# aleph-zero-foundation/sha2-on-cq-halo2

Measured on AMD Instinct MI355X. Metric: sha256_cq_create_proof_k18: MSM Mscalar/s over proof-generation wall-clock (ms_per_step), higher is better.
Workload: dtype u256-montgomery

## Files before the change

include/cq_halo2.h:

```cpp
#ifndef CQ_HALO2_H
#define CQ_HALO2_H

#include <stddef.h>
#include <stdint.h>

#ifdef __cplusplus
extern "C" {
#endif

#define CQ_OK 0
#define CQ_ERR_ARG (-1)
#define CQ_ERR_HIP (-2)
#define CQ_ERR_NO_DEVICE (-3)
#define CQ_ERR_LOOKUP (-4)
#define CQ_ERR_INTERNAL (-5)
#define CQ_ERR_TRANSCRIPT (-6)

typedef struct cq_ctx cq_ctx;
typedef struct cq_domain cq_domain;
typedef struct cq_params cq_params;
typedef struct cq_table_config cq_table_config;
typedef struct cq_static_table cq_static_table;
typedef struct cq_g2_srs cq_g2_srs;
typedef struct cq_pk cq_pk;
// ... 29 lines not shown
                    const uint64_t omega[4]);

int cq_best_multiexp(cq_ctx* ctx, const uint64_t* coeffs, const uint64_t* bases, size_t len,
                     uint64_t out_jac[12]);
int cq_best_multiexp_dev(cq_ctx* ctx, const uint64_t* coeffs_dev, const uint64_t* bases_dev, size_t len,
                         uint64_t out_jac[12]);
int cq_msm_batch_dev(cq_ctx* ctx, const uint64_t* const* coeffs_dev, const uint64_t* bases_dev, size_t len,
                     size_t count, uint64_t* out_jac);
int cq_g1_sum(const uint64_t* jac_points, size_t count, uint64_t out_jac[12]);
int cq_g1_to_affine(const uint64_t jac[12], uint64_t out_affine[8]);
int cq_best_multiexp_g2(cq_ctx* ctx, const uint64_t* coeffs, const uint64_t* bases, size_t len, uint64_t out_jac[24]);
int cq_best_multiexp_g2_dev(cq_ctx* ctx, const uint64_t* coeffs_dev, const uint64_t* bases_dev, size_t len,
                            uint64_t out_jac[24]);
int cq_g2_sum(const uint64_t* jac_points, size_t count, uint64_t out_jac[24]);
int cq_g2_to_affine(const uint64_t jac[24], uint64_t out_affine[16]);
int cq_msm_precompute_dev(cq_ctx* ctx, const uint64_t* bases_dev, size_t n);
int cq_msm_forget_dev(cq_ctx* ctx, const uint64_t* bases_dev);
int cq_msm_set_precompute(cq_ctx* ctx, int on);
int cq_msm_set_window(cq_ctx* ctx, uint32_t bits);
int cq_msm_set_table_window(cq_ctx* ctx, uint32_t bits);
int cq_msm_table_width_dev(cq_ctx* ctx, const uint64_t* bases_dev, size_t n, uint32_t preferred_bits, uint32_t* bits);

int cq_msm_bucket_sums_dev(cq_ctx* ctx, const uint64_t* const* bases_dev, size_t arrays, int packed, const uint32_t* index_dev, size_t n,
                           size_t buckets, uint64_t* out_dev);

int cq_eval_polynomial(cq_ctx* ctx, const uint64_t* poly, size_t n, const uint64_t point[4], uint64_t out[4]);
int cq_eval_polynomial_dev(cq_ctx* ctx, const uint64_t* poly_dev, size_t n, const uint64_t point[4], uint64_t out[4]);
int cq_kate_division(cq_ctx* ctx, const uint64_t* a, size_t n, const uint64_t b[4], uint64_t* q);
int cq_kate_division_dev(cq_ctx* ctx, const uint64_t* a_dev, size_t n, const uint64_t b[4], uint64_t* q_dev);
int cq_batch_invert(cq_ctx* ctx, uint64_t* a, size_t n);
int cq_batch_invert_dev(cq_ctx* ctx, uint64_t* a_dev, size_t n);

typedef struct {
  const uint64_t* num;
  const uint32_t* den_rows;
  const uint64_t* den;
  size_t den_count;
} cq_assigned_column;
int cq_batch_invert_assigned_dev(cq_ctx* ctx, const cq_assigned_column* cols, size_t ncols, size_t n, uint64_t* const* out_dev);
int cq_batch_invert_assigned(cq_ctx* ctx, const cq_assigned_column* cols, size_t ncols, size_t n, uint64_t* const* out);

int cq_domain_create(cq_ctx* ctx, uint32_t j, uint32_t k, cq_domain** out);
void cq_domain_destroy(cq_domain* domain);
uint32_t cq_domain_k(const cq_domain* domain);
uint32_t cq_domain_extended_k(const cq_domain* domain);
int cq_domain_constants(const cq_domain* domain, uint64_t omega[4], uint64_t omega_inv[4],
                        uint64_t extended_omega[4], uint64_t ifft_divisor[4]);
int cq_lagrange_to_coeff(cq_domain* domain, uint64_t* a);
int cq_coeff_to_extended(cq_domain* domain, const uint64_t* a, uint64_t* out);
int cq_extended_to_coeff(cq_domain* domain, const uint64_t* a, uint64_t* out);
int cq_lagrange_to_coeff_dev(cq_domain* domain, const uint64_t* in_dev, uint64_t* out_dev, uint32_t batch);
int cq_coeff_to_extended_dev(cq_domain* domain, const uint64_t* in_dev, uint64_t* out_dev, uint32_t batch);
int cq_extended_to_coeff_dev(cq_domain* domain, const uint64_t* in_dev, uint64_t* out_dev);

int cq_params_create(cq_ctx* ctx, uint32_t k, const uint64_t* g, const uint64_t* g_lagrange, cq_params** out);
int cq_params_setup_from_toxic_waste(cq_ctx* ctx, uint32_t k, const uint64_t s[4], cq_params** out);
int cq_fixed_base_mul_dev(cq_ctx* ctx, const uint64_t* scalars_dev, size_t n, uint64_t* out_affine_dev);
int cq_params_read_raw(cq_ctx* ctx, const uint8_t* buf, size_t len, int checked, cq_params** out);
int cq_params_write_raw(cq_params* params, uint8_t* buf, size_t cap, size_t* written);
#define CQ_SERDE_PROCESSED 0
#define CQ_SERDE_RAW_BYTES 1
#define CQ_SERDE_RAW_BYTES_UNCHECKED 2
int cq_g1_decompress_dev(cq_ctx* ctx, const uint8_t* bytes_dev, size_t n, uint64_t* out_affine_dev, size_t* first_bad);
int cq_g1_compress_dev(cq_ctx* ctx, const uint64_t* affine_dev, size_t n, uint8_t* bytes_dev);
int cq_fr_from_repr_dev(cq_ctx* ctx, const uint8_t* bytes_dev, size_t n, uint64_t* out_dev, size_t* first_bad);
int cq_fr_to_repr_dev(cq_ctx* ctx, const uint64_t* in_dev, size_t n, uint8_t* bytes_dev);
int cq_params_read(cq_ctx* ctx, const uint8_t* buf, size_t len, int format, cq_params** out);
int cq_params_write(cq_params* params, int format, uint8_t* buf, size_t cap, size_t* written);
size_t cq_params_serialized_size(const cq_params* params, int format);
int cq_g2_decompress_dev(cq_ctx* ctx, const uint8_t* bytes_dev, size_t n, uint64_t* out_affine_dev, size_t* first_bad);
int cq_g2_compress_dev(cq_ctx* ctx, const uint64_t* affine_dev, size_t n, uint8_t* bytes_dev);
int cq_params_set_g2(cq_params* params, const uint64_t g2[16], const uint64_t s_g2[16]);
int cq_params_g2(const cq_params* params, uint64_t g2[16], uint64_t s_g2[16]);
int cq_params_read_full(cq_ctx* ctx, const uint8_t* buf, size_t len, int format, cq_params** out);
int cq_params_write_full(cq_params* params, int format, uint8_t* buf, size_t cap, size_t* written);
size_t cq_params_serialized_size_full(const cq_params* params, int format);
int cq_g_to_lagrange_dev(cq_ctx* ctx, const uint64_t* g_dev, uint32_t k, uint64_t* g_lagrange_dev);
int cq_g_to_lagrange_windowed_dev(cq_ctx* ctx, const uint64_t* g_dev, uint32_t k, uint64_t* g_lagrange_dev);
int cq_params_from_powers(cq_ctx* ctx, uint32_t k, const uint64_t* g, int g_on_device, cq_params** out);
int cq_params_downsize(cq_params* params, uint32_t k, cq_params** out);
void cq_params_destroy(cq_params* params);
const uint64_t* cq_params_g_dev(const cq_params* params);
const uint64_t* cq_params_g_lagrange_dev(const cq_params* params);
int cq_commit(cq_params* params, const uint64_t* poly, size_t len, uint64_t out_jac[12]);
int cq_commit_lagrange(cq_params* params, const uint64_t* poly, size_t len, uint64_t out_jac[12]);
int cq_commit_dev(cq_params* params, const uint64_t* poly_dev, size_t len, uint64_t out_jac[12]);
int cq_commit_lagrange_dev(cq_params* params, const uint64_t* poly_dev, size_t len, uint64_t out_jac[12]);

int cq_table_config_create(cq_ctx* ctx, size_t size, const uint64_t* g1_lagrange,
                           const uint64_t* g_lagrange_opening_at_0, cq_table_config** out);
int cq_table_config_setup_from_toxic_waste(cq_ctx* ctx, size_t size, const uint64_t s[4], cq_table_config** out);
int cq_table_config_from_srs(cq_ctx* ctx, size_t size, const uint64_t* srs_g1, size_t srs_len, int on_device,
                             cq_table_config** out);
void cq_table_config_destroy(cq_table_config* cfg);
int cq_table_config_download(cq_table_config* cfg, uint64_t* g1_lagrange, uint64_t* g_lagrange_opening_at_0);
int cq_static_table_create(cq_ctx* ctx, size_t size, const uint64_t* values, const uint64_t* qs_affine,
                           cq_static_table** out);
int cq_static_table_setup_from_toxic_waste(cq_ctx* ctx, size_t size, const uint64_t* values, const uint64_t s[4],
                                           cq_static_table** out);
int cq_static_table_new(cq_ctx* ctx, size_t size, const uint64_t* values, const uint64_t* srs_g1, cq_static_table** out);
int cq_static_table_new_fk(cq_ctx* ctx, size_t size, const uint64_t* values, const uint64_t* srs_g1, cq_static_table** out);
int cq_static_table_new_fk_dev(cq_ctx* ctx, size_t size, const uint64_t* values, const uint64_t* srs_g1_dev,
                               cq_static_table** out);
void cq_static_table_destroy(cq_static_table* table);
int cq_static_table_download_qs(cq_static_table* table, uint64_t* qs_affine);
int cq_g2_srs_create(cq_ctx* ctx, size_t count, const uint64_t* points, int checked, cq_g2_srs** out);
// ... 37 lines not shown
  const uint32_t* gate_program_lens;
  const uint32_t* gate_programs;
  uint32_t num_constants;
  const uint64_t* constants;
  uint32_t num_perm_columns;
  const uint32_t* perm_column_kinds;
  const uint32_t* perm_column_indices;
  const uint32_t* perm_mapping;
  const uint32_t* lookup_input_program_lens;
  const uint32_t* lookup_input_programs;
  uint32_t num_legacy_lookups;
  const uint32_t* legacy_lookup_widths;
  const uint32_t* legacy_program_lens;
  const uint32_t* legacy_programs;
  const uint8_t* advice_column_phases;
  uint32_t num_challenges;
  const uint8_t* challenge_phases;
} cq_plonk;

typedef struct {
  uint32_t k;
  uint32_t num_advice;
  uint32_t num_lookups;
  const uint32_t* lookup_widths;
  const uint32_t* lookup_columns;
  cq_static_table* const* lookup_tables;
  uint64_t vk_repr[4];
  const cq_plonk* plonk;
} cq_circuit;

void cq_permutation_assembly_init(uint32_t columns, uint32_t n, uint32_t* mapping, uint32_t* aux, uint32_t* sizes);
int cq_permutation_assembly_copy(uint32_t columns, uint32_t n, uint32_t* mapping, uint32_t* aux, uint32_t* sizes,
                                 uint32_t left_column, uint32_t left_row, uint32_t right_column, uint32_t right_row);
int cq_pk_create(cq_ctx* ctx, cq_params* params, const cq_circuit* circuit, cq_table_config* cfg,
                 const uint64_t* b0_g1_bound, int b0_on_device, cq_pk** out);
int cq_pk_read_raw(cq_ctx* ctx, cq_params* params, const cq_circuit* circuit, cq_table_config* cfg,
                   const uint64_t* b0_g1_bound, int b0_on_device, const uint8_t* buf, size_t len, uint32_t num_selectors,
                   int checked, cq_pk** out);
size_t cq_pk_raw_size(const cq_pk* pk, uint32_t num_selectors);
int cq_pk_write_raw(cq_pk* pk, const uint8_t* selector_bits, uint32_t num_selectors, uint8_t* buf, size_t cap, size_t* written);
int cq_pk_read(cq_ctx* ctx, cq_params* params, const cq_circuit* circuit, cq_table_config* cfg, const uint64_t* b0_g1_bound,
               int b0_on_device, const uint8_t* buf, size_t len, uint32_t num_selectors, int format, cq_pk** out);
size_t cq_pk_serialized_size(const cq_pk* pk, int format, uint32_t num_selectors);
int cq_pk_write(cq_pk* pk, int format, const uint8_t* selector_bits, uint32_t num_selectors, uint8_t* buf, size_t cap, size_t* written);
int cq_pk_set_sharding(cq_pk* pk, uint32_t rank, uint32_t world, cq_allgather_fn fn, void* user);
int cq_pk_set_column_sharding(cq_pk* pk, int on, cq_bcast_fn fn, void* user);
int cq_pk_set_resident_sharding(cq_pk* pk, int on, cq_exchange_fn fn, void* user);
#define CQ_OPENER_GWC 0
#define CQ_OPENER_SHPLONK 1
int cq_pk_set_opener(cq_pk* pk, int opener);
int cq_pk_set_rng_fill(cq_pk* pk, cq_rng_fill_fn fill);
void cq_pk_destroy(cq_pk* pk);
uint32_t cq_pk_usable_rows(const cq_pk* pk);
const uint64_t* cq_pk_b_row_bases_dev(const cq_pk* pk, int which);
size_t cq_pk_proof_size(const cq_pk* pk);
int cq_create_proof(cq_pk* pk, const uint64_t* const* advice_dev, cq_rng_next_u64 rng, void* rng_state,
                    uint8_t* proof, size_t proof_cap, size_t* proof_len);
int cq_create_proof_batch(cq_pk* pk, size_t count, const uint64_t* const* const* advice_dev, cq_rng_next_u64 rng,
                          void* const* rng_states, uint8_t* const* proofs, size_t proof_cap, size_t* proof_lens, uint32_t lanes);
int cq_create_proof_host(cq_pk* pk, const uint64_t* const* advice, cq_rng_next_u64 rng, void* rng_state,
                         uint8_t* proof, size_t proof_cap, size_t* proof_len);
int cq_create_proof_assigned(cq_pk* pk, const cq_assigned_column* cols, const uint64_t* const* instances,
                             const size_t* instance_lens, cq_rng_next_u64 rng, void* rng_state, uint8_t* proof,
                             size_t proof_cap, size_t* proof_len);
int cq_create_proof_instances(cq_pk* pk, const uint64_t* const* advice, int advice_on_device,
                              const uint64_t* const* instances, const size_t* instance_lens, cq_rng_next_u64 rng,
                              void* rng_state, uint8_t* proof, size_t proof_cap, size_t* proof_len);
typedef int (*cq_phase_fn)(void* user, uint32_t phase, const uint64_t* challenges, uint64_t* const* advice_dev);
int cq_create_proof_phases(cq_pk* pk, uint64_t* const* advice_dev, const uint64_t* const* instances,
                           const size_t* instance_lens, cq_phase_fn phase_fn, void* phase_user, cq_rng_next_u64 rng,
                           void* rng_state, uint8_t* proof, size_t proof_cap, size_t* proof_len);
#define CQ_FAIL_GATE 1u
#define CQ_FAIL_GATE_POISONED 2u
#define CQ_FAIL_LOOKUP 3u
#define CQ_FAIL_STATIC_LOOKUP 4u
#define CQ_FAIL_PERMUTATION 5u
typedef struct { uint32_t kind; uint32_t index; uint32_t row; uint32_t detail; } cq_witness_failure;
int cq_pk_check_witness(cq_pk* pk, const uint64_t* const* advice, int advice_on_device, const uint64_t* const* instances,
                        const size_t* instance_lens, const uint64_t* challenges, cq_witness_failure* failures, size_t cap,
                        size_t* total);
int cq_cq_round1_dev(cq_pk* pk, const uint64_t* const* advice_dev, const uint64_t* const* instance_dev, const uint64_t* challenges,
                     const uint64_t theta[4], uint64_t* f_dev, uint32_t* m_dev, uint64_t* commitments);
int cq_cq_round2_dev(cq_pk* pk, const uint64_t* f_dev, const uint32_t* m_dev, const uint64_t theta[4], const uint64_t beta[4],
                     uint64_t* b_coeff_dev, uint64_t* f_coeff_dev, uint64_t* commitments, uint64_t* a_at_zero);
int cq_quotient_dev(cq_pk* pk, const uint64_t* b_coeff_dev, const uint64_t* f_coeff_dev, const uint64_t y[4], const uint64_t beta[4],
                    const uint64_t* h_in_dev, int divide_by_vanishing, uint64_t* h_out_dev);
int cq_permute_expression_pair_dev(cq_ctx* ctx, uint32_t k, uint32_t usable, const uint64_t* input_dev, const uint64_t* table_dev,
                                   uint64_t* permuted_input_dev, uint64_t* permuted_table_dev);
int cq_permutation_commit_dev(cq_pk* pk, const uint64_t* const* advice_dev, const uint64_t* const* instance_dev, const uint64_t beta[4],
                              const uint64_t gamma[4], cq_rng_next_u64 rng, void* rng_state, uint64_t* z_coeff_dev,
                              uint64_t* commitments);
int cq_lookup_commit_product_dev(cq_pk* pk, const uint64_t* const* input_dev, const uint64_t* const* table_dev,
                                 const uint64_t* const* permuted_input_dev, const uint64_t* const* permuted_table_dev,
                                 const uint64_t beta[4], const uint64_t gamma[4], cq_rng_next_u64 rng, void* rng_state,
                                 uint64_t* z_coeff_dev, uint64_t* commitments);
int cq_evaluate_h_dev(cq_pk* pk, const uint64_t* const* advice_coeff_dev, const uint64_t* const* instance_coeff_dev,
                      const uint64_t* perm_z_coeff_dev, const uint64_t* const* permuted_input_coeff_dev,
                      const uint64_t* const* permuted_table_coeff_dev, const uint64_t* lookup_z_coeff_dev, const uint64_t* challenges,
                      const uint64_t beta[4], const uint64_t gamma[4], const uint64_t theta[4], const uint64_t y[4], uint64_t* h_out_dev);
typedef struct { const uint64_t* poly_dev; size_t len; uint64_t point[4]; } cq_open_query;
typedef int (*cq_squeeze_challenge_fn)(void* user, uint64_t* out );
typedef int (*cq_write_point_fn)(void* user, const uint64_t* affine );
typedef struct { cq_squeeze_challenge_fn squeeze_challenge; cq_write_point_fn write_point; void* user; } cq_open_transcript;
int cq_multiopen_dev(cq_pk* pk, const cq_open_query* queries, size_t count, const cq_open_transcript* transcript);
uint32_t cq_pk_permutation_sets(const cq_pk* pk);
uint32_t cq_pk_legacy_lookups(const cq_pk* pk);
// ... 128 lines not shown
```

include/cq_halo2_sys.rs:

```rust
#![allow(non_camel_case_types, dead_code)]
use core::ffi::{c_char, c_int, c_void};

pub const CQ_OK: i32 = 0;
pub const CQ_ERR_ARG: i32 = -1;
pub const CQ_ERR_HIP: i32 = -2;
pub const CQ_ERR_NO_DEVICE: i32 = -3;
pub const CQ_ERR_LOOKUP: i32 = -4;
pub const CQ_ERR_INTERNAL: i32 = -5;
pub const CQ_ERR_TRANSCRIPT: i32 = -6;
pub const CQ_RCCL_UNIQUE_ID_BYTES: usize = 128;
pub const CQ_SERDE_PROCESSED: i32 = 0;
pub const CQ_SERDE_RAW_BYTES: i32 = 1;
pub const CQ_SERDE_RAW_BYTES_UNCHECKED: i32 = 2;
pub const CQ_GATE_CONST: u32 = 0;
pub const CQ_GATE_ADVICE: u32 = 1;
pub const CQ_GATE_FIXED: u32 = 2;
pub const CQ_GATE_INSTANCE: u32 = 3;
pub const CQ_GATE_NEG: u32 = 4;
pub const CQ_GATE_ADD: u32 = 5;
pub const CQ_GATE_MUL: u32 = 6;
pub const CQ_GATE_SCALE: u32 = 7;
pub const CQ_GATE_CHALLENGE: u32 = 8;
pub const CQ_COL_ADVICE: u32 = 0;
pub const CQ_COL_FIXED: u32 = 1;
// ... 190 lines not shown
    pub fn cq_ctx_create(device: c_int, hip_stream: *mut c_void, out: *mut *mut CqCtx) -> c_int;
    pub fn cq_ctx_destroy(ctx: *mut CqCtx);
    pub fn cq_last_error(ctx: *const CqCtx) -> *const c_char;
    pub fn cq_ctx_sync(ctx: *mut CqCtx) -> c_int;
    pub fn cq_ctx_set_hip_graphs(ctx: *mut CqCtx, on: c_int) -> c_int;
    pub fn cq_rccl_unique_id(id: *mut u8 ) -> c_int;
    pub fn cq_ctx_comm_init_rccl(ctx: *mut CqCtx, rank: u32, world: u32, id: *const u8 ) -> c_int;
    pub fn cq_ctx_comm_destroy(ctx: *mut CqCtx) -> c_int;
    pub fn cq_ctx_comm_selftest(ctx: *mut CqCtx) -> c_int;
    pub fn cq_ctx_stream(ctx: *mut CqCtx) -> *mut c_void;
    pub fn cq_version() -> *const c_char;
    pub fn cq_dev_alloc(ctx: *mut CqCtx, bytes: usize, dptr: *mut *mut c_void) -> c_int;
    pub fn cq_dev_free(ctx: *mut CqCtx, dptr: *mut c_void) -> c_int;
    pub fn cq_dev_upload(ctx: *mut CqCtx, dst_dev: *mut c_void, src_host: *const c_void, bytes: usize) -> c_int;
    pub fn cq_dev_download(ctx: *mut CqCtx, dst_host: *mut c_void, src_dev: *const c_void, bytes: usize) -> c_int;
    pub fn cq_dev_memset(ctx: *mut CqCtx, dptr: *mut c_void, value: c_int, bytes: usize) -> c_int;
    pub fn cq_best_fft(ctx: *mut CqCtx, a: *mut u64, log_n: u32, omega: *const u64 ) -> c_int;
    pub fn cq_best_fft_dev(ctx: *mut CqCtx, in_dev: *const u64, out_dev: *mut u64, log_n: u32, omega: *const u64 ) -> c_int;
    pub fn cq_best_multiexp(ctx: *mut CqCtx, coeffs: *const u64, bases: *const u64, len: usize, out_jac: *mut u64 ) -> c_int;
    pub fn cq_best_multiexp_dev(ctx: *mut CqCtx, coeffs_dev: *const u64, bases_dev: *const u64, len: usize, out_jac: *mut u64 ) -> c_int;
    pub fn cq_msm_batch_dev(ctx: *mut CqCtx, coeffs_dev: *const *const u64, bases_dev: *const u64, len: usize, count: usize, out_jac: *mut u64) -> c_int;
    pub fn cq_g1_sum(jac_points: *const u64, count: usize, out_jac: *mut u64 ) -> c_int;
    pub fn cq_g1_to_affine(jac: *const u64 , out_affine: *mut u64 ) -> c_int;
    pub fn cq_best_multiexp_g2(ctx: *mut CqCtx, coeffs: *const u64, bases: *const u64, len: usize, out_jac: *mut u64 ) -> c_int;
    pub fn cq_best_multiexp_g2_dev(ctx: *mut CqCtx, coeffs_dev: *const u64, bases_dev: *const u64, len: usize, out_jac: *mut u64 ) -> c_int;
    pub fn cq_g2_sum(jac_points: *const u64, count: usize, out_jac: *mut u64 ) -> c_int;
    pub fn cq_g2_to_affine(jac: *const u64 , out_affine: *mut u64 ) -> c_int;
    pub fn cq_msm_precompute_dev(ctx: *mut CqCtx, bases_dev: *const u64, n: usize) -> c_int;
    pub fn cq_msm_forget_dev(ctx: *mut CqCtx, bases_dev: *const u64) -> c_int;
    pub fn cq_msm_set_precompute(ctx: *mut CqCtx, on: c_int) -> c_int;
    pub fn cq_msm_set_window(ctx: *mut CqCtx, bits: u32) -> c_int;
    pub fn cq_msm_set_table_window(ctx: *mut CqCtx, bits: u32) -> c_int;
    pub fn cq_msm_table_width_dev(ctx: *mut CqCtx, bases_dev: *const u64, n: usize, preferred_bits: u32, bits: *mut u32) -> c_int;
    pub fn cq_msm_bucket_sums_dev(ctx: *mut CqCtx, bases_dev: *const *const u64, arrays: usize, packed: c_int, index_dev: *const u32, n: usize, buckets: usize, out_dev: *mut u64) -> c_int;
    pub fn cq_eval_polynomial(ctx: *mut CqCtx, poly: *const u64, n: usize, point: *const u64 , out: *mut u64 ) -> c_int;
    pub fn cq_eval_polynomial_dev(ctx: *mut CqCtx, poly_dev: *const u64, n: usize, point: *const u64 , out: *mut u64 ) -> c_int;
    pub fn cq_kate_division(ctx: *mut CqCtx, a: *const u64, n: usize, b: *const u64 , q: *mut u64) -> c_int;
    pub fn cq_kate_division_dev(ctx: *mut CqCtx, a_dev: *const u64, n: usize, b: *const u64 , q_dev: *mut u64) -> c_int;
    pub fn cq_batch_invert(ctx: *mut CqCtx, a: *mut u64, n: usize) -> c_int;
    pub fn cq_batch_invert_dev(ctx: *mut CqCtx, a_dev: *mut u64, n: usize) -> c_int;
    pub fn cq_batch_invert_assigned_dev(ctx: *mut CqCtx, cols: *const CqAssignedColumn, ncols: usize, n: usize, out_dev: *const *mut u64) -> c_int;
    pub fn cq_batch_invert_assigned(ctx: *mut CqCtx, cols: *const CqAssignedColumn, ncols: usize, n: usize, out: *const *mut u64) -> c_int;
    pub fn cq_domain_create(ctx: *mut CqCtx, j: u32, k: u32, out: *mut *mut CqDomain) -> c_int;
    pub fn cq_domain_destroy(domain: *mut CqDomain);
    pub fn cq_domain_k(domain: *const CqDomain) -> u32;
    pub fn cq_domain_extended_k(domain: *const CqDomain) -> u32;
    pub fn cq_domain_constants(domain: *const CqDomain, omega: *mut u64 , omega_inv: *mut u64 , extended_omega: *mut u64 , ifft_divisor: *mut u64 ) -> c_int;
    pub fn cq_lagrange_to_coeff(domain: *mut CqDomain, a: *mut u64) -> c_int;
    pub fn cq_coeff_to_extended(domain: *mut CqDomain, a: *const u64, out: *mut u64) -> c_int;
    pub fn cq_extended_to_coeff(domain: *mut CqDomain, a: *const u64, out: *mut u64) -> c_int;
    pub fn cq_lagrange_to_coeff_dev(domain: *mut CqDomain, in_dev: *const u64, out_dev: *mut u64, batch: u32) -> c_int;
    pub fn cq_coeff_to_extended_dev(domain: *mut CqDomain, in_dev: *const u64, out_dev: *mut u64, batch: u32) -> c_int;
    pub fn cq_extended_to_coeff_dev(domain: *mut CqDomain, in_dev: *const u64, out_dev: *mut u64) -> c_int;
    pub fn cq_params_create(ctx: *mut CqCtx, k: u32, g: *const u64, g_lagrange: *const u64, out: *mut *mut CqParams) -> c_int;
    pub fn cq_params_setup_from_toxic_waste(ctx: *mut CqCtx, k: u32, s: *const u64 , out: *mut *mut CqParams) -> c_int;
    pub fn cq_fixed_base_mul_dev(ctx: *mut CqCtx, scalars_dev: *const u64, n: usize, out_affine_dev: *mut u64) -> c_int;
    pub fn cq_params_read_raw(ctx: *mut CqCtx, buf: *const u8, len: usize, checked: c_int, out: *mut *mut CqParams) -> c_int;
    pub fn cq_params_write_raw(params: *mut CqParams, buf: *mut u8, cap: usize, written: *mut usize) -> c_int;
    pub fn cq_g1_decompress_dev(ctx: *mut CqCtx, bytes_dev: *const u8, n: usize, out_affine_dev: *mut u64, first_bad: *mut usize) -> c_int;
    pub fn cq_g1_compress_dev(ctx: *mut CqCtx, affine_dev: *const u64, n: usize, bytes_dev: *mut u8) -> c_int;
    pub fn cq_fr_from_repr_dev(ctx: *mut CqCtx, bytes_dev: *const u8, n: usize, out_dev: *mut u64, first_bad: *mut usize) -> c_int;
    pub fn cq_fr_to_repr_dev(ctx: *mut CqCtx, in_dev: *const u64, n: usize, bytes_dev: *mut u8) -> c_int;
    pub fn cq_params_read(ctx: *mut CqCtx, buf: *const u8, len: usize, format: c_int, out: *mut *mut CqParams) -> c_int;
    pub fn cq_params_write(params: *mut CqParams, format: c_int, buf: *mut u8, cap: usize, written: *mut usize) -> c_int;
    pub fn cq_params_serialized_size(params: *const CqParams, format: c_int) -> usize;
    pub fn cq_g2_decompress_dev(ctx: *mut CqCtx, bytes_dev: *const u8, n: usize, out_affine_dev: *mut u64, first_bad: *mut usize) -> c_int;
    pub fn cq_g2_compress_dev(ctx: *mut CqCtx, affine_dev: *const u64, n: usize, bytes_dev: *mut u8) -> c_int;
    pub fn cq_params_set_g2(params: *mut CqParams, g2: *const u64 , s_g2: *const u64 ) -> c_int;
    pub fn cq_params_g2(params: *const CqParams, g2: *mut u64 , s_g2: *mut u64 ) -> c_int;
    pub fn cq_params_read_full(ctx: *mut CqCtx, buf: *const u8, len: usize, format: c_int, out: *mut *mut CqParams) -> c_int;
    pub fn cq_params_write_full(params: *mut CqParams, format: c_int, buf: *mut u8, cap: usize, written: *mut usize) -> c_int;
    pub fn cq_params_serialized_size_full(params: *const CqParams, format: c_int) -> usize;
    pub fn cq_g_to_lagrange_dev(ctx: *mut CqCtx, g_dev: *const u64, k: u32, g_lagrange_dev: *mut u64) -> c_int;
    pub fn cq_g_to_lagrange_windowed_dev(ctx: *mut CqCtx, g_dev: *const u64, k: u32, g_lagrange_dev: *mut u64) -> c_int;
    pub fn cq_params_from_powers(ctx: *mut CqCtx, k: u32, g: *const u64, g_on_device: c_int, out: *mut *mut CqParams) -> c_int;
    pub fn cq_params_downsize(params: *mut CqParams, k: u32, out: *mut *mut CqParams) -> c_int;
    pub fn cq_params_destroy(params: *mut CqParams);
    pub fn cq_params_g_dev(params: *const CqParams) -> *const u64;
    pub fn cq_params_g_lagrange_dev(params: *const CqParams) -> *const u64;
    pub fn cq_commit(params: *mut CqParams, poly: *const u64, len: usize, out_jac: *mut u64 ) -> c_int;
    pub fn cq_commit_lagrange(params: *mut CqParams, poly: *const u64, len: usize, out_jac: *mut u64 ) -> c_int;
    pub fn cq_commit_dev(params: *mut CqParams, poly_dev: *const u64, len: usize, out_jac: *mut u64 ) -> c_int;
    pub fn cq_commit_lagrange_dev(params: *mut CqParams, poly_dev: *const u64, len: usize, out_jac: *mut u64 ) -> c_int;
    pub fn cq_table_config_create(ctx: *mut CqCtx, size: usize, g1_lagrange: *const u64, g_lagrange_opening_at_0: *const u64, out: *mut *mut CqTableConfig) -> c_int;
    pub fn cq_table_config_setup_from_toxic_waste(ctx: *mut CqCtx, size: usize, s: *const u64 , out: *mut *mut CqTableConfig) -> c_int;
    pub fn cq_table_config_from_srs(ctx: *mut CqCtx, size: usize, srs_g1: *const u64, srs_len: usize, on_device: c_int, out: *mut *mut CqTableConfig) -> c_int;
    pub fn cq_table_config_destroy(cfg: *mut CqTableConfig);
    pub fn cq_table_config_download(cfg: *mut CqTableConfig, g1_lagrange: *mut u64, g_lagrange_opening_at_0: *mut u64) -> c_int;
    pub fn cq_static_table_create(ctx: *mut CqCtx, size: usize, values: *const u64, qs_affine: *const u64, out: *mut *mut CqStaticTable) -> c_int;
    pub fn cq_static_table_setup_from_toxic_waste(ctx: *mut CqCtx, size: usize, values: *const u64, s: *const u64 , out: *mut *mut CqStaticTable) -> c_int;
    pub fn cq_static_table_new(ctx: *mut CqCtx, size: usize, values: *const u64, srs_g1: *const u64, out: *mut *mut CqStaticTable) -> c_int;
    pub fn cq_static_table_new_fk(ctx: *mut CqCtx, size: usize, values: *const u64, srs_g1: *const u64, out: *mut *mut CqStaticTable) -> c_int;
    pub fn cq_static_table_new_fk_dev(ctx: *mut CqCtx, size: usize, values: *const u64, srs_g1_dev: *const u64, out: *mut *mut CqStaticTable) -> c_int;
    pub fn cq_static_table_destroy(table: *mut CqStaticTable);
    pub fn cq_static_table_download_qs(table: *mut CqStaticTable, qs_affine: *mut u64) -> c_int;
    pub fn cq_g2_srs_create(ctx: *mut CqCtx, count: usize, points: *const u64, checked: c_int, out: *mut *mut CqG2Srs) -> c_int;
    pub fn cq_g2_srs_setup_from_toxic_waste(ctx: *mut CqCtx, count: usize, s: *const u64 , out: *mut *mut CqG2Srs) -> c_int;
    pub fn cq_g2_srs_download(srs: *mut CqG2Srs, points: *mut u64) -> c_int;
    pub fn cq_g2_srs_len(srs: *const CqG2Srs) -> usize;
    pub fn cq_g2_srs_dev(srs: *const CqG2Srs) -> *const u64;
    pub fn cq_g2_srs_destroy(srs: *mut CqG2Srs);
    pub fn cq_g2_srs_read(ctx: *mut CqCtx, buf: *const u8, len: usize, format: c_int, out: *mut *mut CqG2Srs) -> c_int;
    pub fn cq_g2_srs_write(srs: *mut CqG2Srs, format: c_int, buf: *mut u8, cap: usize, written: *mut usize) -> c_int;
    pub fn cq_g2_srs_serialized_size(srs: *const CqG2Srs, format: c_int) -> usize;
    pub fn cq_static_table_commit(table: *mut CqStaticTable, srs_g2: *mut CqG2Srs, srs_g1_len: usize, circuit_n: usize, zv: *mut u64 , t: *mut u64 , x_b0_bound: *mut u64 ) -> c_int;
    pub fn cq_permutation_assembly_init(columns: u32, n: u32, mapping: *mut u32, aux: *mut u32, sizes: *mut u32);
    pub fn cq_permutation_assembly_copy(columns: u32, n: u32, mapping: *mut u32, aux: *mut u32, sizes: *mut u32, left_column: u32, left_row: u32, right_column: u32, right_row: u32) -> c_int;
    pub fn cq_pk_create(ctx: *mut CqCtx, params: *mut CqParams, circuit: *const CqCircuit, cfg: *mut CqTableConfig, b0_g1_bound: *const u64, b0_on_device: c_int, out: *mut *mut CqPk) -> c_int;
    pub fn cq_pk_read_raw(ctx: *mut CqCtx, params: *mut CqParams, circuit: *const CqCircuit, cfg: *mut CqTableConfig, b0_g1_bound: *const u64, b0_on_device: c_int, buf: *const u8, len: usize, num_selectors: u32, checked: c_int, out: *mut *mut CqPk) -> c_int;
    pub fn cq_pk_raw_size(pk: *const CqPk, num_selectors: u32) -> usize;
    pub fn cq_pk_write_raw(pk: *mut CqPk, selector_bits: *const u8, num_selectors: u32, buf: *mut u8, cap: usize, written: *mut usize) -> c_int;
    pub fn cq_pk_read(ctx: *mut CqCtx, params: *mut CqParams, circuit: *const CqCircuit, cfg: *mut CqTableConfig, b0_g1_bound: *const u64, b0_on_device: c_int, buf: *const u8, len: usize, num_selectors: u32, format: c_int, out: *mut *mut CqPk) -> c_int;
    pub fn cq_pk_serialized_size(pk: *const CqPk, format: c_int, num_selectors: u32) -> usize;
    pub fn cq_pk_write(pk: *mut CqPk, format: c_int, selector_bits: *const u8, num_selectors: u32, buf: *mut u8, cap: usize, written: *mut usize) -> c_int;
    pub fn cq_pk_set_sharding(pk: *mut CqPk, rank: u32, world: u32, fn_: CqAllgatherFn, user: *mut c_void) -> c_int;
    pub fn cq_pk_set_column_sharding(pk: *mut CqPk, on: c_int, fn_: CqBcastFn, user: *mut c_void) -> c_int;
    pub fn cq_pk_set_resident_sharding(pk: *mut CqPk, on: c_int, fn_: CqExchangeFn, user: *mut c_void) -> c_int;
    pub fn cq_pk_set_opener(pk: *mut CqPk, opener: c_int) -> c_int;
    pub fn cq_pk_set_rng_fill(pk: *mut CqPk, fill: CqRngFillFn) -> c_int;
    pub fn cq_pk_destroy(pk: *mut CqPk);
    pub fn cq_pk_usable_rows(pk: *const CqPk) -> u32;
    pub fn cq_pk_b_row_bases_dev(pk: *const CqPk, which: c_int) -> *const u64;
    pub fn cq_pk_proof_size(pk: *const CqPk) -> usize;
    pub fn cq_create_proof(pk: *mut CqPk, advice_dev: *const *const u64, rng: CqRngNextU64, rng_state: *mut c_void, proof: *mut u8, proof_cap: usize, proof_len: *mut usize) -> c_int;
    pub fn cq_create_proof_batch(pk: *mut CqPk, count: usize, advice_dev: *const *const *const u64, rng: CqRngNextU64, rng_states: *const *mut c_void, proofs: *const *mut u8, proof_cap: usize, proof_lens: *mut usize, lanes: u32) -> c_int;
    pub fn cq_create_proof_host(pk: *mut CqPk, advice: *const *const u64, rng: CqRngNextU64, rng_state: *mut c_void, proof: *mut u8, proof_cap: usize, proof_len: *mut usize) -> c_int;
    pub fn cq_create_proof_assigned(pk: *mut CqPk, cols: *const CqAssignedColumn, instances: *const *const u64, instance_lens: *const usize, rng: CqRngNextU64, rng_state: *mut c_void, proof: *mut u8, proof_cap: usize, proof_len: *mut usize) -> c_int;
    pub fn cq_create_proof_instances(pk: *mut CqPk, advice: *const *const u64, advice_on_device: c_int, instances: *const *const u64, instance_lens: *const usize, rng: CqRngNextU64, rng_state: *mut c_void, proof: *mut u8, proof_cap: usize, proof_len: *mut usize) -> c_int;
    pub fn cq_create_proof_phases(pk: *mut CqPk, advice_dev: *const *mut u64, instances: *const *const u64, instance_lens: *const usize, phase_fn: CqPhaseFn, phase_user: *mut c_void, rng: CqRngNextU64, rng_state: *mut c_void, proof: *mut u8, proof_cap: usize, proof_len: *mut usize) -> c_int;
    pub fn cq_pk_check_witness(pk: *mut CqPk, advice: *const *const u64, advice_on_device: c_int, instances: *const *const u64, instance_lens: *const usize, challenges: *const u64, failures: *mut CqWitnessFailure, cap: usize, total: *mut usize) -> c_int;
    pub fn cq_cq_round1_dev(pk: *mut CqPk, advice_dev: *const *const u64, instance_dev: *const *const u64, challenges: *const u64, theta: *const u64 , f_dev: *mut u64, m_dev: *mut u32, commitments: *mut u64) -> c_int;
    pub fn cq_cq_round2_dev(pk: *mut CqPk, f_dev: *const u64, m_dev: *const u32, theta: *const u64 , beta: *const u64 , b_coeff_dev: *mut u64, f_coeff_dev: *mut u64, commitments: *mut u64, a_at_zero: *mut u64) -> c_int;
    pub fn cq_quotient_dev(pk: *mut CqPk, b_coeff_dev: *const u64, f_coeff_dev: *const u64, y: *const u64 , beta: *const u64 , h_in_dev: *const u64, divide_by_vanishing: c_int, h_out_dev: *mut u64) -> c_int;
    pub fn cq_permute_expression_pair_dev(ctx: *mut CqCtx, k: u32, usable: u32, input_dev: *const u64, table_dev: *const u64, permuted_input_dev: *mut u64, permuted_table_dev: *mut u64) -> c_int;
    pub fn cq_permutation_commit_dev(pk: *mut CqPk, advice_dev: *const *const u64, instance_dev: *const *const u64, beta: *const u64 , gamma: *const u64 , rng: CqRngNextU64, rng_state: *mut c_void, z_coeff_dev: *mut u64, commitments: *mut u64) -> c_int;
    pub fn cq_lookup_commit_product_dev(pk: *mut CqPk, input_dev: *const *const u64, table_dev: *const *const u64, permuted_input_dev: *const *const u64, permuted_table_dev: *const *const u64, beta: *const u64 , gamma: *const u64 , rng: CqRngNextU64, rng_state: *mut c_void, z_coeff_dev: *mut u64, commitments: *mut u64) -> c_int;
    pub fn cq_evaluate_h_dev(pk: *mut CqPk, advice_coeff_dev: *const *const u64, instance_coeff_dev: *const *const u64, perm_z_coeff_dev: *const u64, permuted_input_coeff_dev: *const *const u64, permuted_table_coeff_dev: *const *const u64, lookup_z_coeff_dev: *const u64, challenges: *const u64, beta: *const u64 , gamma: *const u64 , theta: *const u64 , y: *const u64 , h_out_dev: *mut u64) -> c_int;
    pub fn cq_multiopen_dev(pk: *mut CqPk, queries: *const CqOpenQuery, count: usize, transcript: *const CqOpenTranscript) -> c_int;
    pub fn cq_pk_permutation_sets(pk: *const CqPk) -> u32;
    pub fn cq_pk_legacy_lookups(pk: *const CqPk) -> u32;
    pub fn cq_pk_vk_commitments(pk: *mut CqPk, fixed_commitments: *mut u64, permutation_commitments: *mut u64) -> c_int;
    pub fn cq_sha_witness_fill_dev(ctx: *mut CqCtx, words_dev: *const u32, nwords: usize, pairs: u32, n: usize, cols_dev: *const *mut u64) -> c_int;
    pub fn cq_sha_synthesis_table_dev(ctx: *mut CqCtx, kind: c_int, first_limb_len: u32, second_limb_len: u32, out_dev: *mut u64) -> c_int;
    pub fn cq_sha_decomposition_table_dev(ctx: *mut CqCtx, first_limb_len: u32, second_limb_len: u32, k_bits: u32, out_dev: *mut u64) -> c_int;
    pub fn cq_sha_spread_table_dev(ctx: *mut CqCtx, size: usize, dense_dev: *mut u64, spread_dev: *mut u64) -> c_int;
    pub fn cq_sha256_layout(cells: *mut u32, cap: usize, count: *mut usize) -> c_int;
    pub fn cq_sha256_synthesize_dev(ctx: *mut CqCtx, table_bits: u32, msg_words: *const u32, blocks: usize, n: usize, cols_dev: *const *mut u64, digest: *mut u32 ) -> c_int;
    pub fn cq_sha256_synthesize_segments_dev(ctx: *mut CqCtx, table_bits: u32, seg_blocks: *const u32, segments: usize, sources: *const u32, words_dev: *const u32, words_len: usize, n: usize, cols_dev: *const *mut u64, digests_dev: *mut u32) -> c_int;
    pub fn cq_sha256_synthesize_choices_dev(ctx: *mut CqCtx, table_bits: u32, seg_blocks: *const u32, segments: usize, sources: *const u32, choices: *const u32, n_choices: usize, words_dev: *const u32, words_len: usize, n: usize, cols_dev: *const *mut u64, digests_dev: *mut u32) -> c_int;
    pub fn cq_sha256_synthesize_states_dev(ctx: *mut CqCtx, table_bits: u32, seg_blocks: *const u32, segments: usize, sources: *const u32, choices: *const u32, n_choices: usize, init_sources: *const u32, words_dev: *const u32, words_len: usize, n: usize, cols_dev: *const *mut u64, digests_dev: *mut u32) -> c_int;
    pub fn cq_sha256_synthesize_xors_dev(ctx: *mut CqCtx, table_bits: u32, seg_blocks: *const u32, segments: usize, sources: *const u32, choices: *const u32, n_choices: usize, init_sources: *const u32, xors: *const u32, n_xors: usize, words_dev: *const u32, words_len: usize, n: usize, cols_dev: *const *mut u64, digests_dev: *mut u32) -> c_int;
    pub fn cq_sha256_synthesize_varlen_dev(ctx: *mut CqCtx, table_bits: u32, seg_max_blocks: *const u32, segments: usize, msg_bytes_dev: *const u8, msg_bytes_len: usize, msg_offsets: *const u64, msg_lens: *const u64, n: usize, cols_dev: *const *mut u64, digests_dev: *mut u32) -> c_int;
    pub fn cq_sha256_synthesize_varlen_from_dev(ctx: *mut CqCtx, table_bits: u32, seg_max_blocks: *const u32, segments: usize, msg_bytes_dev: *const u8, msg_bytes_len: usize, msg_offsets: *const u64, msg_lens: *const u64, init_states_dev: *const u32, base_lens: *const u64, n: usize, cols_dev: *const *mut u64, digests_dev: *mut u32) -> c_int;
    pub fn cq_sha512_layout(cells: *mut u32, cap: usize, count: *mut usize) -> c_int;
    pub fn cq_sha512_synthesize_dev(ctx: *mut CqCtx, table_bits: u32, seg_blocks: *const u32, segments: usize, seg_variant: *const u32, msg_words: *const u64, n: usize, cols_dev: *const *mut u64, digests_out: *mut u64) -> c_int;
    pub fn cq_xoshiro256ss_seed(seed: u64, state: *mut u64 );
    pub fn cq_xoshiro256ss_next_u64(state: *mut c_void) -> u64;
    pub fn cq_xoshiro256ss_fill(state: *mut u64 , dst: *mut u64, count: usize, threads: u32);
    pub fn cq_buffer_rng_next_u64(state: *mut c_void) -> u64;
    pub fn cq_opaque_rng_next_u64(state: *mut c_void) -> u64;
    pub fn cq_opaque_rng_fill(state: *mut c_void, dst: *mut u64, count: usize);
    pub fn cq_profile_enable(ctx: *mut CqCtx, on: c_int) -> c_int;
    pub fn cq_profile_read(ctx: *mut CqCtx, id: c_int, total_ms: *mut f64, calls: *mut u64) -> c_int;
    pub fn cq_bench_modmul_dev(ctx: *mut CqCtx, out_dev: *mut u64, lanes: u32, iters: u32, which: c_int) -> c_int;
}
```

sha2_on_cq_halo2_amd/csrc/capi_cq.hip:

```cpp
#include <algorithm>
#include <atomic>
#include <cstring>
#include <mutex>
#include <string>
#include <thread>
#include <vector>
#include "assigned_host.hpp"
#include "building.hpp"
#include "cq.hpp"
#include "xoshiro.hpp"
#include "ctx.hpp"
#include "g1fft.hpp"
#include "plonk.hpp"
#include "poly.hpp"
#include "prover.hpp"
#include "setup.hpp"
#include "msm.hpp"
#include "comm.hpp"
#include "serde.hpp"

using namespace cq;

static bool is_pow2(size_t x) { return x && !(x & (x - 1)); }
static uint32_t log2u(size_t x) {
// ... 132 lines not shown
  if ((rc = domain_lagrange_to_coeff(dom, t->values, coeffs, 1, size, size)) != CQ_OK) return rc;
  if ((rc = poly_eval(c, coeffs, (uint32_t)size, sf, &ts)) != CQ_OK) return rc;
  if ((rc = cq_qs_scalars(c, t->values, (uint32_t)size, ts, sf, dom->omega, dom->ifft_divisor, sc)) != CQ_OK) return rc;
  if ((rc = fixed_base_mul(c, sc, (uint32_t)size, t->qs)) != CQ_OK) return rc;
  return guard.finish(out);
}

void cq_static_table_destroy(cq_static_table* t) {
  if (!t) return;
  hipStreamSynchronize(t->ctx->stream);
  if (t->values) hipFree(t->values);
  if (t->qs) hipFree(t->qs);
  if (t->slots) hipFree(t->slots);
  delete t;
}

int cq_static_table_download_qs(cq_static_table* t, uint64_t* qs_affine) {
  if (!t || !qs_affine) return CQ_ERR_ARG;
  cq_ctx* c = t->ctx;
  CQ_HIP(c, hipMemcpyAsync(qs_affine, t->qs, t->N * sizeof(G1Affine), hipMemcpyDeviceToHost, c->stream));
  CQ_HIP(c, hipStreamSynchronize(c->stream));
  return CQ_OK;
}

int cq_pk_set_opener(cq_pk* pk, int opener) {
  if (!pk || (opener != CQ_OPENER_GWC && opener != CQ_OPENER_SHPLONK)) return CQ_ERR_ARG;
  pk->opener = opener;
  return CQ_OK;
}

int cq_pk_set_rng_fill(cq_pk* pk, cq_rng_fill_fn fill) {
  if (!pk) return CQ_ERR_ARG;
  pk->rng_fill = fill;
  return CQ_OK;
}

int cq_pk_set_column_sharding(cq_pk* pk, int on, cq_bcast_fn fn, void* user) {
  if (!pk) return CQ_ERR_ARG;
  pk->shard_columns = on != 0;
  pk->bcast = fn;
  pk->bcast_user = user;
  return CQ_OK;
}

int cq_pk_set_resident_sharding(cq_pk* pk, int on, cq_exchange_fn fn, void* user) {
  if (!pk) return CQ_ERR_ARG;
  pk->shard_resident = on != 0;
  pk->exchange = fn;
  pk->exchange_user = user;
  return CQ_OK;
}

uint32_t cq_pk_usable_rows(const cq_pk* pk) { return pk ? pk->u : 0; }
const uint64_t* cq_pk_b_row_bases_dev(const cq_pk* pk, int which) {
  return pk && (which == 0 || which == 1) ? (const uint64_t*)pk->b_row_bases[which] : nullptr;
}

size_t cq_pk_proof_size(const cq_pk* pk) {
  if (!pk) return 0;
  const size_t L = pk->lookups.size(), S = pk->perm_sets();
  const size_t PL = pk->legacy.size();
  const size_t openings = pk->opener == CQ_OPENER_SHPLONK ? 2 : pk->opening_rotations().size();
  const size_t points = pk->num_advice + 2 * L + 3 * PL + S + 5 * L + 1 + pk->domain->quotient_poly_degree + openings;
  const size_t scalars = pk->advice_queries.size() + pk->fixed_queries.size() + 1 + pk->perm_columns.size() + (S ? 3 * S - 1 : 0) + 3 * L + 5 * PL;
  return 32 * (points + scalars);
}

static int create_proof_any(cq_pk* pk, const uint64_t* const* advice_dev, const uint64_t* const* instances,
                            const size_t* instance_lens, cq_rng_next_u64 rng, void* rng_state, uint8_t* proof,
                            size_t proof_cap, size_t* proof_len, cq_phase_fn phase_fn = nullptr, void* phase_user = nullptr) {
  if (!pk || (!advice_dev && pk->num_advice) || !rng || !proof || !proof_len) return CQ_ERR_ARG;
  cq_ctx* c = pk->ctx;
  if (pk->num_instance && (!instances || !instance_lens)) return c->fail(CQ_ERR_ARG, "create_proof: instance columns missing");
  CQ_HIP(c, hipSetDevice(c->device));
  std::vector<uint8_t> out;
  if (pk->num_phases > 1 && !phase_fn) return c->fail(CQ_ERR_ARG, "create_proof: a multi-phase circuit needs cq_create_proof_phases");
  if (rng == cq_buffer_rng_next_u64) ((cq_buffer_rng*)rng_state)->overrun = 0;
  int rc = create_proof_dev(pk, advice_dev, instances, instance_lens, phase_fn, phase_user, rng, rng_state, out);
  const bool rank_local = rc == CQ_ERR_HIP || rc == CQ_ERR_INTERNAL || rc == CQ_ERR_NO_DEVICE;
  if (rank_local && pk->sharded() && !pk->allgather && c->rccl_comm && !pk->shard_single) {
    const std::string keep = c->err;
    cq::comm_rccl_abort(c);
    c->err = keep + " (sharded proof: this rank's RCCL communicator was aborted so that its peers do not hang)";
  }
  if (rng == cq_buffer_rng_next_u64 && ((cq_buffer_rng*)rng_state)->overrun && (rc == CQ_OK || rc == CQ_ERR_TRANSCRIPT))
    return c->fail(CQ_ERR_ARG, "create_proof: the pre-drawn RNG stream ran out (blinding would be zero)");
  if (rc != CQ_OK) return rc;
  if (out.size() > proof_cap) return c->fail(CQ_ERR_ARG, "proof buffer too small");
  memcpy(proof, out.data(), out.size());
  *proof_len = out.size();
  return CQ_OK;
}

int cq_create_proof(cq_pk* pk, const uint64_t* const* advice_dev, cq_rng_next_u64 rng, void* rng_state, uint8_t* proof,
                    size_t proof_cap, size_t* proof_len) {
  return create_proof_any(pk, advice_dev, nullptr, nullptr, rng, rng_state, proof, proof_cap, proof_len);
}

static int create_proof_host_any(cq_pk* pk, const uint64_t* const* advice, const uint64_t* const* instances,
                                 const size_t* instance_lens, cq_rng_next_u64 rng, void* rng_state, uint8_t* proof,
                                 size_t proof_cap, size_t* proof_len) {
  if (!pk || (!advice && pk->num_advice)) return CQ_ERR_ARG;
  cq_ctx* c = pk->ctx;
  CQ_HIP(c, hipSetDevice(c->device));
  const size_t n = (size_t)1 << pk->k;
  void* stage;
// ... 334 lines not shown
```

sha2_on_cq_halo2_amd/csrc/capi_poly.hip:

```cpp
#include <cstring>
#include <string>
#include <vector>
#include "assigned_host.hpp"
#include "ctx.hpp"
#include "poly.hpp"

using namespace cq;

namespace {
struct HostStage {
  cq_ctx* c;
  void* din = nullptr;
  void* dout = nullptr;
  int rc = CQ_OK;
  HostStage(cq_ctx* c_, size_t in_bytes, size_t out_bytes) : c(c_) {
    if ((rc = c->ensure_scratch(Scratch::EntryA, in_bytes ? in_bytes : 32, &din)) != CQ_OK) return;
    rc = c->ensure_scratch(Scratch::EntryB, out_bytes ? out_bytes : 32, &dout);
  }
};

int assigned_offsets(cq_ctx* c, const cq_assigned_column* cols, size_t ncols, size_t n, std::vector<uint32_t>& off) {
  if (n > 0x7fffffffull) return c->fail(CQ_ERR_ARG, "batch_invert_assigned: n too large");
  off.assign(ncols + 1, 0);
  for (size_t a = 0; a < ncols; a++) {
    const cq_assigned_column& col = cols[a];
    if ((n && !col.num) || (col.den_count && (!col.den_rows || !col.den)))
      return c->fail(CQ_ERR_ARG, "batch_invert_assigned: column " + std::to_string(a) + ": null array");
    if (col.den_count > n)
      return c->fail(CQ_ERR_ARG, "batch_invert_assigned: column " + std::to_string(a) + ", entry " + std::to_string(n) +
                                     ": more entries than rows");
    if ((uint64_t)off[a] + col.den_count > 0x7fffffffull) return c->fail(CQ_ERR_ARG, "batch_invert_assigned: too many rational cells");
    off[a + 1] = off[a] + (uint32_t)col.den_count;
  }
  return CQ_OK;
}
inline size_t round32(size_t b) { return (b + 31) & ~(size_t)31; }
}

extern "C" {

int cq_domain_create(cq_ctx* c, uint32_t j, uint32_t k, cq_domain** out) {
  if (!c || !out || j < 1) return CQ_ERR_ARG;
  CQ_HIP(c, hipSetDevice(c->device));
  return domain_create(c, j, k, out);
}
void cq_domain_destroy(cq_domain* d) { domain_destroy(d); }
uint32_t cq_domain_k(const cq_domain* d) { return d ? d->k : 0; }
uint32_t cq_domain_extended_k(const cq_domain* d) { return d ? d->extended_k : 0; }

int cq_domain_constants(const cq_domain* d, uint64_t omega[4], uint64_t omega_inv[4], uint64_t extended_omega[4],
                        uint64_t ifft_divisor[4]) {
  if (!d) return CQ_ERR_ARG;
  if (omega) d->omega.to_limbs64(omega);
  if (omega_inv) d->omega_inv.to_limbs64(omega_inv);
  if (extended_omega) d->extended_omega.to_limbs64(extended_omega);
  if (ifft_divisor) d->ifft_divisor.to_limbs64(ifft_divisor);
  return CQ_OK;
}

int cq_lagrange_to_coeff_dev(cq_domain* d, const uint64_t* in_dev, uint64_t* out_dev, uint32_t batch) {
  if (!d || !in_dev || !out_dev || !batch) return CQ_ERR_ARG;
  CQ_HIP(d->ctx, hipSetDevice(d->ctx->device));
  return domain_lagrange_to_coeff(d, (const Fr*)in_dev, (Fr*)out_dev, batch, d->n(), d->n());
}
int cq_coeff_to_extended_dev(cq_domain* d, const uint64_t* in_dev, uint64_t* out_dev, uint32_t batch) {
  if (!d || !in_dev || !out_dev || !batch) return CQ_ERR_ARG;
  if ((const void*)in_dev == (const void*)out_dev) return d->ctx->fail(CQ_ERR_ARG, "coeff_to_extended: in == out");
  CQ_HIP(d->ctx, hipSetDevice(d->ctx->device));
  return domain_coeff_to_extended(d, (const Fr*)in_dev, (Fr*)out_dev, batch, d->n(), d->ext());
}
int cq_extended_to_coeff_dev(cq_domain* d, const uint64_t* in_dev, uint64_t* out_dev) {
  if (!d || !in_dev || !out_dev) return CQ_ERR_ARG;
  CQ_HIP(d->ctx, hipSetDevice(d->ctx->device));
  return domain_extended_to_coeff(d, (const Fr*)in_dev, (Fr*)out_dev);
}

int cq_lagrange_to_coeff(cq_domain* d, uint64_t* a) {
  if (!d || !a) return CQ_ERR_ARG;
  cq_ctx* c = d->ctx;
  CQ_HIP(c, hipSetDevice(c->device));
  const size_t bytes = d->n() * sizeof(Fr);
  HostStage st(c, bytes, bytes);
  if (st.rc != CQ_OK) return st.rc;
  CQ_HIP(c, hipMemcpyAsync(st.din, a, bytes, hipMemcpyHostToDevice, c->stream));
  int rc = domain_lagrange_to_coeff(d, (const Fr*)st.din, (Fr*)st.dout, 1, d->n(), d->n());
  if (rc != CQ_OK) return rc;
  CQ_HIP(c, hipMemcpyAsync(a, st.dout, bytes, hipMemcpyDeviceToHost, c->stream));
  CQ_HIP(c, hipStreamSynchronize(c->stream));
  return CQ_OK;
}
int cq_coeff_to_extended(cq_domain* d, const uint64_t* a, uint64_t* out) {
  if (!d || !a || !out) return CQ_ERR_ARG;
  cq_ctx* c = d->ctx;
  CQ_HIP(c, hipSetDevice(c->device));
  HostStage st(c, d->n() * sizeof(Fr), d->ext() * sizeof(Fr));
  if (st.rc != CQ_OK) return st.rc;
  CQ_HIP(c, hipMemcpyAsync(st.din, a, d->n() * sizeof(Fr), hipMemcpyHostToDevice, c->stream));
  int rc = domain_coeff_to_extended(d, (const Fr*)st.din, (Fr*)st.dout, 1, d->n(), d->ext());
  if (rc != CQ_OK) return rc;
  CQ_HIP(c, hipMemcpyAsync(out, st.dout, d->ext() * sizeof(Fr), hipMemcpyDeviceToHost, c->stream));
  CQ_HIP(c, hipStreamSynchronize(c->stream));
  return CQ_OK;
}
int cq_extended_to_coeff(cq_domain* d, const uint64_t* a, uint64_t* out) {
  if (!d || !a || !out) return CQ_ERR_ARG;
  cq_ctx* c = d->ctx;
  CQ_HIP(c, hipSetDevice(c->device));
  const size_t out_bytes = d->n() * d->quotient_poly_degree * sizeof(Fr);
  HostStage st(c, d->ext() * sizeof(Fr), out_bytes);
  if (st.rc != CQ_OK) return st.rc;
  CQ_HIP(c, hipMemcpyAsync(st.din, a, d->ext() * sizeof(Fr), hipMemcpyHostToDevice, c->stream));
  int rc = domain_extended_to_coeff(d, (const Fr*)st.din, (Fr*)st.dout);
  if (rc != CQ_OK) return rc;
  if (out_bytes) CQ_HIP(c, hipMemcpyAsync(out, st.dout, out_bytes, hipMemcpyDeviceToHost, c->stream));
  CQ_HIP(c, hipStreamSynchronize(c->stream));
  return CQ_OK;
}

int cq_eval_polynomial_dev(cq_ctx* c, const uint64_t* poly_dev, size_t n, const uint64_t point[4], uint64_t out[4]) {
  if (!c || !point || !out || (n && !poly_dev) || n > 0x7fffffffull) return CQ_ERR_ARG;
  CQ_HIP(c, hipSetDevice(c->device));
  Fr r;
  int rc = poly_eval(c, (const Fr*)poly_dev, (uint32_t)n, Fr::from_limbs64(point), &r);
  if (rc != CQ_OK) return rc;
  r.to_limbs64(out);
  return CQ_OK;
}
int cq_eval_polynomial(cq_ctx* c, const uint64_t* poly, size_t n, const uint64_t point[4], uint64_t out[4]) {
  if (!c || !point || !out || (n && !poly) || n > 0x7fffffffull) return CQ_ERR_ARG;
// ... 122 lines not shown
```

sha2_on_cq_halo2_amd/csrc/cq.hpp:

```cpp
#pragma once
#include <hip/hip_runtime.h>
#include <vector>
#include "../../include/cq_halo2.h"
#include "curve.hpp"
#include "pk.hpp"
#include "poly.hpp"

struct cq_ctx;
struct cq_params;

namespace cq {

constexpr uint32_t CQ_MAX_WIDTH = 8;

struct CqRound1Args {
  const Fr* cols[CQ_MAX_WIDTH];
  const Fr* values[CQ_MAX_WIDTH];
  const uint32_t* slots[CQ_MAX_WIDTH];
  uint32_t nslots[CQ_MAX_WIDTH];
  uint32_t width;
};
constexpr uint32_t CQ_ROUND1_BATCH = 8;
struct CqRound1Batch {
  CqRound1Args a[CQ_ROUND1_BATCH];
// ... 52 lines not shown
int g1_validate(cq_ctx* c, const G1Affine* pts, uint32_t n, uint32_t* bad_dev);
int fr_validate(cq_ctx* c, const Fr* v, size_t n, uint32_t* bad_dev);

}

namespace cq {
inline void shard_range(size_t n, uint32_t rank, uint32_t world, size_t& lo, size_t& hi) {
  const size_t base = n / world, rem = n % world;
  lo = rank * base + (rank < rem ? rank : rem);
  hi = lo + base + (rank < rem ? 1 : 0);
}
}

struct cq_params {
  cq_ctx* ctx;
  uint32_t k;
  size_t n;
  cq::G1Affine* g;
  cq::G1Affine* g_lagrange;
  uint32_t key_users = 0;
  bool owner_released = false;
  bool has_g2 = false;
  uint64_t g2[16] = {}, s_g2[16] = {};
};

struct cq_table_config {
  cq_ctx* ctx;
  uint32_t log_n;
  size_t N;
  cq::G1Affine* g1_lagrange = nullptr;
  cq::G1Affine* g_lagrange_opening_at_0 = nullptr;
  uint32_t key_users = 0;
  bool owner_released = false;
};

struct cq_static_table {
  cq_ctx* ctx;
  size_t N;
  cq::Fr* values = nullptr;
  cq::G1Affine* qs = nullptr;
  uint32_t* slots = nullptr;
  uint32_t nslots = 0;
};

struct cq_pk : cq_pk_desc {
  cq_ctx* ctx;
  cq_params* params;
  cq_domain* domain = nullptr;
  cq_table_config* table_cfg;
  cq::G1Affine* b0_g1_bound = nullptr;
  bool own_b0 = false;
  cq::G1Affine* b_row_bases[2] = {nullptr, nullptr};
  cq::Fr* l_active_row = nullptr;
  cq::Fr* fixed_values = nullptr;
  cq::Fr* fixed_polys = nullptr;
  cq::Fr* fixed_cosets = nullptr;
  cq::Fr* l0 = nullptr;
  cq::Fr* l_last = nullptr;
  uint32_t* gate_prog = nullptr;
  cq::Fr* constants = nullptr;
  uint32_t* lookup_prog = nullptr;
  uint32_t* legacy_prog = nullptr;
  cq::Fr* perm_values = nullptr;
  cq::Fr* perm_polys = nullptr;
  cq::Fr* perm_cosets = nullptr;
  cq::Fr* omega_powers = nullptr;
  cq::Fr* ext_pow_lo = nullptr;
  cq::Fr* ext_pow_hi = nullptr;
  int opener = CQ_OPENER_GWC;
  cq_rng_fill_fn rng_fill = nullptr;
  cq::Fr vk_repr;
  std::vector<cq::G1Affine*> qs_concat;
  uint32_t shard_rank = 0, shard_world = 1;
  bool shard_single = false;
  bool sharded() const { return shard_world > 1 || shard_single; }
  cq_allgather_fn allgather = nullptr;
  void* allgather_user = nullptr;
  bool shard_columns = true;
  cq_bcast_fn bcast = nullptr;
  void* bcast_user = nullptr;
  bool shard_resident = false;
  cq_exchange_fn exchange = nullptr;
  void* exchange_user = nullptr;
  uint32_t table_c = 0;
  struct TableRef { const void* bases; size_t n; uint32_t c; };
  std::vector<TableRef> held_tables, shard_tables;
  bool dropped_params_tables = false, dropped_cfg_tables = false;
  bool counted_users = false;
};
```

sha2_on_cq_halo2_amd/csrc/domain.hip:

```cpp
#include "ctx.hpp"
#include "poly.hpp"

namespace cq {

int domain_create(cq_ctx* c, uint32_t j, uint32_t k, cq_domain** out) {
  if (j < 2 && j != 1) return c->fail(CQ_ERR_ARG, "domain: j must be >= 1");
  if (k > FR_S) return c->fail(CQ_ERR_ARG, "domain: k too large");
  cq_domain* d = new cq_domain();
  d->ctx = c;
  d->j = j;
  d->k = k;
  d->quotient_poly_degree = j - 1;
  const uint64_t n = 1ull << k;
  uint32_t ek = k;
  while ((1ull << ek) < n * d->quotient_poly_degree) ek++;
  if (ek > FR_S) {
    delete d;
    return c->fail(CQ_ERR_ARG, "domain: extended_k exceeds the field's 2-adicity");
  }
  d->extended_k = ek;
  Fr w = fr_from_raw(FR_ROOT_OF_UNITY_RAW);
  for (uint32_t i = ek; i < FR_S; i++) w = w.sqr();
  d->extended_omega = w;
  for (uint32_t i = k; i < ek; i++) w = w.sqr();
  d->omega = w;
  d->omega_inv = d->omega.inv();
  d->extended_omega_inv = d->extended_omega.inv();
  d->g_coset = fr_from_raw(FR_ZETA_RAW);
  d->g_coset_inv = d->g_coset.sqr();
  const Fr orig = d->g_coset.pow_u64(n);
  const Fr step = d->extended_omega.pow_u64(n);
  Fr cur = orig;
  const size_t tl = (size_t)1 << (ek - k);
  for (size_t i = 0; i < tl; i++) {
    d->t_evaluations.push_back((cur - Fr::one()).inv());
    cur = cur * step;
  }
  d->ifft_divisor = Fr::from_u64(n).inv();
  d->extended_ifft_divisor = Fr::from_u64(1ull << ek).inv();
  d->barycentric_weight = d->ifft_divisor;
  if (hipMalloc(&d->t_evaluations_dev, tl * sizeof(Fr)) != hipSuccess ||
      hipMemcpy(d->t_evaluations_dev, d->t_evaluations.data(), tl * sizeof(Fr), hipMemcpyHostToDevice) != hipSuccess) {
    delete d;
    return c->fail(CQ_ERR_HIP, "domain: t_evaluations upload failed");
  }
  *out = d;
  return CQ_OK;
}

void domain_destroy(cq_domain* d) {
  if (!d) return;
  hipStreamSynchronize(d->ctx->stream);
  if (d->t_evaluations_dev) hipFree(d->t_evaluations_dev);
  delete d;
}

static int run(cq_ctx* c, uint32_t log_n, const Fr& omega, const Fr* in, Fr* out, NttIo& io) {
  int rc = CQ_OK;
  const NttTables* tb = c->tables_for(log_n, omega, &rc);
  if (!tb) return rc;
  const size_t n = (size_t)1 << log_n;
  const bool aux = c->aux_stream && c->stream == c->aux_stream;
  void* scr;
  if ((rc = c->ensure_scratch(aux ? Scratch::NttAux : Scratch::Ntt, (size_t)2 * io.batch * n * sizeof(Fr), &scr)) != CQ_OK) return rc;
  io.prof = c;
  io.critical = !aux;
  if (ntt_run(*tb, in, out, (Fr*)scr, io, c->stream) != 0) return c->fail(CQ_ERR_HIP, "ntt launch failed");
  return CQ_OK;
}

int domain_fft(cq_ctx* c, const Fr* in, Fr* out, uint32_t log_n, const Fr& omega, uint32_t batch, size_t in_stride,
               size_t out_stride) {
  NttIo io;
  io.batch = batch;
  io.in_stride = in_stride;
  io.out_stride = out_stride;
  io.in_len = io.out_len = 1u << log_n;
  return run(c, log_n, omega, in, out, io);
}

int domain_lagrange_to_coeff(cq_domain* d, const Fr* in, Fr* out, uint32_t batch, size_t in_stride, size_t out_stride) {
  NttIo io;
  io.batch = batch;
  io.in_stride = in_stride;
  io.out_stride = out_stride;
  io.in_len = io.out_len = (uint32_t)d->n();
  io.out_mul = true;
  io.out_mul_v[0] = d->ifft_divisor;
  return run(d->ctx, d->k, d->omega_inv, in, out, io);
}

int domain_coeff_to_extended(cq_domain* d, const Fr* in, Fr* out, uint32_t batch, size_t in_stride, size_t out_stride) {
  NttIo io;
  io.batch = batch;
  io.in_stride = in_stride;
  io.out_stride = out_stride;
  io.in_len = (uint32_t)d->n();
  io.out_len = (uint32_t)d->ext();
  io.in_coset = true;
  io.in_coset_mul[0] = d->g_coset;
  io.in_coset_mul[1] = d->g_coset_inv;
  return run(d->ctx, d->extended_k, d->extended_omega, in, out, io);
}

int domain_extended_to_coeff(cq_domain* d, const Fr* in, Fr* out) {
  NttIo io;
  io.batch = 1;
  io.in_stride = d->ext();
  io.out_stride = d->n() * d->quotient_poly_degree;
  io.in_len = (uint32_t)d->ext();
  io.out_len = (uint32_t)(d->n() * d->quotient_poly_degree);
  io.out_mul = true;
  io.out_coset = true;
  io.out_mul_v[0] = d->extended_ifft_divisor;
  io.out_mul_v[1] = d->extended_ifft_divisor * d->g_coset_inv;
  io.out_mul_v[2] = d->extended_ifft_divisor * d->g_coset;
  return run(d->ctx, d->extended_k, d->extended_omega_inv, in, out, io);
}

}
```

sha2_on_cq_halo2_amd/csrc/ntt.hip:

```cpp
#include <cstdlib>
#include "ntt.hpp"
#include "ctx.hpp"

namespace cq {

__global__ void fr_powers_kernel(Fr* out, Fr base, uint64_t step, uint32_t count) {
  uint32_t j = blockIdx.x * blockDim.x + threadIdx.x;
  if (j >= count) return;
  out[j] = base.pow_u64((uint64_t)j * step);
}

static __device__ __forceinline__ Fr29 lds_load29(const uint32_t* sm, uint32_t E, uint32_t i) {
  Fr29 r;
  CQ_UNROLL for (int l = 0; l < 9; l++) r.a[l] = sm[l * E + i];
  return r;
}
static __device__ __forceinline__ void lds_store29(uint32_t* sm, uint32_t E, uint32_t i, const Fr29& r) {
  CQ_UNROLL for (int l = 0; l < 9; l++) sm[l * E + i] = r.a[l];
}
static __device__ __forceinline__ Fr29 g_load29(const Fr* p) {
  const uint4* q = reinterpret_cast<const uint4*>(p);
  const uint4 a = q[0], b = q[1];
  const uint32_t w[8] = {a.x, a.y, a.z, a.w, b.x, b.y, b.z, b.w};
  return Fr29::unpack(w);
}
static __device__ __forceinline__ void g_store29(Fr* p, const Fr29& x, bool canonical) {
  uint32_t w[8];
  x.pack(w);
  if (canonical) Fr::cond_sub_p(w, 0);
  uint4* q = reinterpret_cast<uint4*>(p);
  q[0] = make_uint4(w[0], w[1], w[2], w[3]);
  q[1] = make_uint4(w[4], w[5], w[6], w[7]);
}
static __device__ __forceinline__ Fr29 const29(const uint32_t* c) {
  Fr29 r;
  CQ_UNROLL for (int l = 0; l < 9; l++) r.a[l] = c[l];
  return r;
}
static __device__ __forceinline__ Fr29 canon29(const Fr29& x) {
  uint32_t w[8];
  x.pack(w);
  Fr::cond_sub_p(w, 0);
  return Fr29::unpack(w);
}
static __device__ __forceinline__ Fr29 sub_level(const Fr29& u, const Fr29& v, uint32_t rnd) {
  switch (rnd) {
    case 0: return Fr29::sub<2>(u, v);
    case 1: return Fr29::sub<4>(u, v);
    case 2: return Fr29::sub<8>(u, v);
    case 3: return Fr29::sub<16>(u, v);
    case 4: return Fr29::sub<32>(u, v);
    default: return Fr29::sub<64>(u, v);
  }
}

__global__ void ntt_table_to29_kernel(Fr* t, uint32_t count) {
  const uint32_t j = blockIdx.x * blockDim.x + threadIdx.x;
  if (j >= count) return;
  g_store29(t + j, Fr29::mul(g_load29(t + j), const29(CONSTS29<FrP>.from256)), true);
}

#ifdef CQ_NTT_TRACE
__device__ uint64_t g_ntt_trace[4 * 65536];
__device__ uint32_t g_ntt_trace_n;
static __device__ __forceinline__ uint32_t ntt_trace_begin() {
  uint32_t slot = 0;
  if (threadIdx.x == 0) {
    slot = atomicAdd(&g_ntt_trace_n, 1u) & 65535u;
    uint32_t hw, xcc;
    asm volatile("s_getreg_b32 %0, hwreg(HW_REG_HW_ID)" : "=s"(hw));
    asm volatile("s_getreg_b32 %0, hwreg(HW_REG_XCC_ID)" : "=s"(xcc));
    g_ntt_trace[4 * slot] = wall_clock64();
    g_ntt_trace[4 * slot + 2] = ((uint64_t)xcc << 32) | hw;
    g_ntt_trace[4 * slot + 3] = ((uint64_t)blockIdx.y << 32) | blockIdx.x;
  }
  return slot;
}
static __device__ __forceinline__ void ntt_trace_end(uint32_t slot) {
  __syncthreads();
  if (threadIdx.x == 0) g_ntt_trace[4 * slot + 1] = wall_clock64();
}
extern "C" int cq_debug_ntt_trace(uint64_t* out, uint32_t cap) {
  uint32_t n = 0;
  if (hipDeviceSynchronize() != hipSuccess) return -1;
  if (hipMemcpyFromSymbol(&n, HIP_SYMBOL(g_ntt_trace_n), 4) != hipSuccess) return -1;
  if (n > cap) n = cap;
  if (n > 65536) n = 65536;
  if (n && hipMemcpyFromSymbol(out, HIP_SYMBOL(g_ntt_trace), (size_t)n * 32) != hipSuccess) return -1;
  const uint32_t z = 0;
  if (hipMemcpyToSymbol(HIP_SYMBOL(g_ntt_trace_n), &z, 4) != hipSuccess) return -1;
  return (int)n;
}
#endif

static_assert(NTT_MAX_DEG <= 6, "sub_level: B_r = 2^(r+1) <= 64");
static __device__ __forceinline__ uint32_t bitrev(uint32_t x, uint32_t bits) {
  return bits ? (__brev(x) >> (32 - bits)) : 0;
}

template <uint32_t DEG, uint32_t LOG_T>
__global__ __launch_bounds__(NTT_THREADS) void ntt_pass_kernel(NttPassArgs a) {
  extern __shared__ uint32_t smem29[];
#ifdef CQ_NTT_TRACE
  const uint32_t trace_slot = ntt_trace_begin();
#endif
  if (a.flags & NTT_CRITICAL) CQ_CRITICAL_WAVES();
  constexpr bool DYN = DEG == 0;
  const uint32_t deg = DYN ? a.deg : DEG, log_t = DYN ? a.log_t : LOG_T;
  const uint32_t D = 1u << deg;
  const uint32_t T = 1u << log_t;
  const uint32_t E = D * T;
  uint32_t* const tw29 = smem29 + 9 * E;
  uint32_t* const cl29 = tw29 + 9 * (D / 2 + 1);
  uint32_t* const cs29 = cl29 + 27;
  const uint32_t n = 1u << a.log_n;
  const uint32_t t = n >> deg;
  const uint32_t p = 1u << a.lgp;
  const uint32_t tile = blockIdx.x;
  const uint32_t batch = blockIdx.y;
  const Fr* in = a.in + (size_t)batch * a.in_stride;
  Fr* out = a.out + (size_t)batch * a.out_stride;
  const uint32_t index0 = tile * T;
  const bool first = a.lgp == 0, last = a.next_deg == 0;
  constexpr bool SWZ = !DYN && LOG_T == 4;
  auto at = [&](uint32_t row, uint32_t c) { return SWZ ? (((row ^ (((row >> 2) ^ (row >> 4)) & 3u)) << 4) + c) : row * T + c; };

  const bool load_mul = first && (a.flags & NTT_IN_COSET);
  if (load_mul && threadIdx.x < 3) {
    Fr29 cl = const29(CONSTS29<FrP>.from256);
    if (threadIdx.x) cl = Fr29::mul(Fr29::unpack(a.in_coset[threadIdx.x - 1].v.l), const29(CONSTS29<FrP>.c271));
    CQ_UNROLL for (int l = 0; l < 9; l++) cl29[threadIdx.x * 9 + l] = cl.a[l];
  }
  if (last && threadIdx.x >= 64 && threadIdx.x < 67) {
    const uint32_t m = threadIdx.x - 64;
    const Fr one = Fr::one();
    const uint32_t* src = (a.flags & NTT_OUT_MUL) ? ((a.flags & NTT_OUT_COSET) ? a.out_mul[m].v.l : a.out_mul[0].v.l) : one.v.l;
    const Fr29 cm = Fr29::unpack(src);
    CQ_UNROLL for (int l = 0; l < 9; l++) cs29[m * 9 + l] = cm.a[l];
  }
  if (load_mul) __syncthreads();
  const uint32_t half = D >> 1;
  for (uint32_t j = threadIdx.x; j < half; j += NTT_THREADS) {
    const Fr29 w = g_load29(a.pq + ((size_t)j << a.pq_shift));
    CQ_UNROLL for (int l = 0; l < 9; l++) tw29[l * half + j] = w.a[l];
  }
  for (uint32_t e = threadIdx.x; e < E; e += NTT_THREADS) {
    const uint32_t c = e & (T - 1);
    const uint32_t i = e >> log_t;
    const uint32_t g = index0 + c + i * t;
    Fr29 x = Fr29::zero();
    if (g < a.in_len) {
      x = g_load29(in + g);
      if (load_mul) x = Fr29::mul(x, lds_load29(cl29 + (g % 3) * 9, 1, 0));
    }
    lds_store29(smem29, E, at(i, c), x);
  }
  __syncthreads();

  constexpr uint32_t R4 = DEG / 2, LEVELS = DEG;
  Fr29::static_for<0, (int)R4>([&](auto ST) {
    constexpr uint32_t st = (uint32_t) decltype(ST)::value;
    constexpr uint32_t rnd = 2 * st;
    const uint32_t bit = half >> rnd;
    const uint32_t hb = bit >> 1;
    for (uint32_t w = threadIdx.x; w < (half >> 1) * T; w += NTT_THREADS) {
      const uint32_t c = w & (T - 1);
      const uint32_t wg = w >> log_t;
      const uint32_t dj = wg >> rnd;
      const uint32_t r0 = (((wg & ((1u << rnd) - 1u)) * bit) << 1) + dj;
      const uint32_t o0 = at(r0, c), o1 = at(r0 + hb, c), o2 = at(r0 + bit, c), o3 = at(r0 + bit + hb, c);
      const Fr29 x0 = lds_load29(smem29, E, o0), x1 = lds_load29(smem29, E, o1);
      const Fr29 x2 = lds_load29(smem29, E, o2), x3 = lds_load29(smem29, E, o3);
      const Fr29 s02 = x0 + x2, s13 = x1 + x3;
      Fr29 d02 = sub_level(x0, x2, rnd);
      Fr29 d13 = sub_level(x1, x3, rnd);
      if (dj) Fr29::mul_pair(d02, lds_load29(tw29, half, dj << rnd), d13, lds_load29(tw29, half, (dj + hb) << rnd), d02, d13);
      else d13 = Fr29::mul(d13, lds_load29(tw29, half, (dj + hb) << rnd));
      Fr29 y0 = s02 + s13;
      y0.normalise();
      Fr29 y1 = sub_level(s02, s13, rnd + 1);
      Fr29 y2 = d02 + d13;
      y2.normalise();
      Fr29 y3 = sub_level(d02, d13, rnd + 1);
      if (dj) {
        const Fr29 w2 = lds_load29(tw29, half, dj << (rnd + 1));
        Fr29::mul_pair(y1, w2, y3, w2, y1, y3);
      }
      lds_store29(smem29, E, o0, y0);
      lds_store29(smem29, E, o1, y1);
      lds_store29(smem29, E, o2, y2);
      lds_store29(smem29, E, o3, y3);
    }
    __syncthreads();
  });
#pragma unroll
  for (uint32_t rnd = 2 * R4; rnd < (DYN ? 6u : LEVELS); rnd++) {
    if (DYN && rnd >= deg) break;
    const uint32_t bit = half >> rnd;
    const uint32_t lg_rest = rnd;
    for (uint32_t w = threadIdx.x; w < half * T; w += NTT_THREADS) {
      const uint32_t c = w & (T - 1);
      const uint32_t wb = w >> log_t;
      const uint32_t di = wb >> lg_rest;
      const uint32_t b = ((wb & ((1u << lg_rest) - 1u)) * bit) | di;
      const uint32_t i0 = (b << 1) - di;
      const uint32_t i1 = i0 + bit;
// ... 61 lines not shown

int NttTables::build(uint32_t log_n_, const Fr& omega_, hipStream_t stream) {
  log_n = log_n_;
  omega = omega_;
  tw_l = (log_n + 1) / 2;
  const uint32_t lo_cnt = 1u << tw_l;
  const uint32_t hi_cnt = 1u << (log_n - tw_l);
  pq_log = log_n < NTT_MAX_DEG ? log_n : NTT_MAX_DEG;
  const uint32_t pq_cnt = pq_log ? (1u << (pq_log - 1)) : 1;
  if (hipMalloc(&tw_lo, sizeof(Fr) * lo_cnt) != hipSuccess) return -1;
  if (hipMalloc(&tw_hi, sizeof(Fr) * hi_cnt) != hipSuccess) return -1;
  if (hipMalloc(&pq, sizeof(Fr) * pq_cnt) != hipSuccess) return -1;
  fr_powers_kernel<<<(lo_cnt + 255) / 256, 256, 0, stream>>>(tw_lo, omega, 1, lo_cnt);
  fr_powers_kernel<<<(hi_cnt + 255) / 256, 256, 0, stream>>>(tw_hi, omega, (uint64_t)lo_cnt, hi_cnt);
  if (log_n >= 8 && log_n <= 24 && !getenv("CQ_NTT_NO_FULL_TABLE") && hipMalloc(&tw_full, sizeof(Fr) << log_n) == hipSuccess)
    fr_powers_kernel<<<((1u << log_n) + 255) / 256, 256, 0, stream>>>(tw_full, omega, 1, 1u << log_n);
  else
    (void)hipGetLastError();
  fr_powers_kernel<<<(pq_cnt + 255) / 256, 256, 0, stream>>>(pq, omega, (uint64_t)1 << (log_n - pq_log), pq_cnt);
  ntt_table_to29_kernel<<<(lo_cnt + 255) / 256, 256, 0, stream>>>(tw_lo, lo_cnt);
  ntt_table_to29_kernel<<<(hi_cnt + 255) / 256, 256, 0, stream>>>(tw_hi, hi_cnt);
  if (tw_full) ntt_table_to29_kernel<<<((1u << log_n) + 255) / 256, 256, 0, stream>>>(tw_full, 1u << log_n);
  ntt_table_to29_kernel<<<(pq_cnt + 255) / 256, 256, 0, stream>>>(pq, pq_cnt);
  return hipGetLastError() == hipSuccess ? 0 : -1;
}

int ntt_run(const NttTables& tb, const Fr* in, Fr* out, Fr* scratch, const NttIo& io, hipStream_t stream) {
  const uint32_t log_n = tb.log_n;
  const uint32_t n = 1u << log_n;
  const uint32_t npass = log_n == 0 ? 1 : (log_n + NTT_MAX_DEG - 1) / NTT_MAX_DEG;
  uint32_t degs[8];
  uint32_t rem = log_n;
  for (uint32_t i = 0; i < npass; i++) {
    uint32_t d = (rem + (npass - i) - 1) / (npass - i);
    degs[i] = d;
    rem -= d;
  }
  if (NTT_MAX_DEG == 6 && log_n >= 12) {
    for (uint32_t c5 = 0; c5 <= npass; c5++) {
      bool found = false;
      for (uint32_t a6 = 0; a6 + c5 <= npass; a6++) {
        const uint32_t b4 = npass - c5 - a6;
        if (6 * a6 + 5 * c5 + 4 * b4 != log_n) continue;
        uint32_t i = 0;
        for (uint32_t q = 0; q < a6; q++) degs[i++] = 6;
        for (uint32_t q = 0; q < c5; q++) degs[i++] = 5;
        for (uint32_t q = 0; q < b4; q++) degs[i++] = 4;
        found = true;
        break;
      }
      if (found) break;
    }
  }
  Fr* sbuf[2] = {scratch, scratch + (size_t)io.batch * n};
  const Fr* src = in;
  uint32_t lgp = 0;
  for (uint32_t ps = 0; ps < npass; ps++) {
    const bool last = (ps + 1 == npass);
    Fr* dst = last ? out : sbuf[ps & 1];
    NttPassArgs a;
    a.in = src;
    a.out = dst;
    a.in_stride = (ps == 0) ? io.in_stride : (size_t)n;
    a.out_stride = last ? io.out_stride : (size_t)n;
    a.log_n = log_n;
    a.lgp = lgp;
    a.deg = degs[ps];
    a.next_deg = last ? 0 : degs[ps + 1];
    const uint32_t t = n >> degs[ps];
    uint32_t log_t = 0;
    while ((1u << (log_t + 1)) <= t && ((1u << (log_t + 1)) << degs[ps]) <= NTT_TILE_ELEMS) log_t++;
    a.log_t = log_t;
    a.tw_lo = tb.tw_lo;
    a.tw_hi = tb.tw_hi;
    a.tw_full = tb.tw_full;
    a.tw_l = tb.tw_l;
    a.pq = tb.pq;
    a.pq_shift = tb.pq_log - degs[ps];
    a.flags = io.critical ? NTT_CRITICAL : 0;
    a.in_len = n;
    a.out_len = n;
    if (ps == 0) {
      a.in_len = io.in_len;
      if (io.in_coset) {
        a.flags |= NTT_IN_COSET;
        a.in_coset[0] = io.in_coset_mul[0];
        a.in_coset[1] = io.in_coset_mul[1];
      }
    }
    if (last) {
      a.out_len = io.out_len;
      const Fr fix = io.in_coset ? Fr::one() : Fr::from_u64(32);
      if (io.out_mul || !io.in_coset) {
        a.flags |= NTT_OUT_MUL;
        a.out_mul[0] = (io.out_mul ? io.out_mul_v[0] : Fr::one()) * fix;
        if (io.out_mul && io.out_coset) {
          a.flags |= NTT_OUT_COSET;
          a.out_mul[1] = io.out_mul_v[1] * fix;
          a.out_mul[2] = io.out_mul_v[2] * fix;
        }
      }
    }
    const uint32_t T = 1u << log_t;
    dim3 grid(t / T, io.batch);
    const size_t lds = ((size_t)(T << degs[ps]) + ((size_t)1 << degs[ps]) / 2 + 1) * 36 + 54 * 4;
    hipEvent_t pe = io.prof ? io.prof->prof_begin(CQ_PROF_NTT_PASS) : nullptr;
    constexpr uint32_t LT = NTT_TILE_ELEMS == 512 ? 9 : NTT_TILE_ELEMS == 2048 ? 11 : 10;
    static_assert(NTT_TILE_ELEMS == (1u << LT), "NTT_TILE_ELEMS: 512, 1024 or 2048");
    if (degs[ps] == 6 && log_t == LT - 6) ntt_pass_kernel<6, LT - 6><<<grid, NTT_THREADS, lds, stream>>>(a);
    else if (degs[ps] == 5 && log_t == LT - 5) ntt_pass_kernel<5, LT - 5><<<grid, NTT_THREADS, lds, stream>>>(a);
    else if (degs[ps] == 4 && log_t == LT - 4) ntt_pass_kernel<4, LT - 4><<<grid, NTT_THREADS, lds, stream>>>(a);
    else ntt_pass_kernel<0, 0><<<grid, NTT_THREADS, lds, stream>>>(a);
    if (io.prof) io.prof->prof_end(pe);
    src = dst;
    lgp += degs[ps];
  }
  return hipGetLastError() == hipSuccess ? 0 : -1;
}

}
```

sha2_on_cq_halo2_amd/csrc/ntt.hpp:

```cpp
#pragma once
#include <hip/hip_runtime.h>
#include "field.hpp"
#include "field29.hpp"

struct cq_ctx;

namespace cq {

#ifndef CQ_NTT_THREADS
#define CQ_NTT_THREADS 256
#endif
constexpr uint32_t NTT_THREADS = CQ_NTT_THREADS;
#ifndef CQ_NTT_MAX_DEG
#define CQ_NTT_MAX_DEG 6
#endif
#ifndef CQ_NTT_TILE_ELEMS
#define CQ_NTT_TILE_ELEMS 1024
#endif
constexpr uint32_t NTT_MAX_DEG = CQ_NTT_MAX_DEG;
constexpr uint32_t NTT_TILE_ELEMS = CQ_NTT_TILE_ELEMS;

enum : uint32_t { NTT_IN_COSET = 1, NTT_OUT_MUL = 2, NTT_OUT_COSET = 4, NTT_CRITICAL = 8 };

struct NttPassArgs {
  const Fr* in;
  Fr* out;
  size_t in_stride, out_stride;
  uint32_t log_n, lgp, deg, log_t;
  uint32_t next_deg;
  const Fr* tw_lo;
  const Fr* tw_hi;
  const Fr* tw_full;
  uint32_t tw_l;
  const Fr* pq;
  uint32_t pq_shift;
  uint32_t flags;
  uint32_t in_len;
  uint32_t out_len;
  Fr in_coset[2];
  Fr out_mul[3];
};

struct NttTables {
  uint32_t log_n = 0;
  Fr omega;
  Fr* tw_lo = nullptr;
  Fr* tw_hi = nullptr;
  Fr* tw_full = nullptr;
  Fr* pq = nullptr;
  uint32_t tw_l = 0, pq_log = 0;
  NttTables() = default;
  NttTables(const NttTables&) = delete;
  NttTables& operator=(const NttTables&) = delete;
  ~NttTables();
  int build(uint32_t log_n, const Fr& omega, hipStream_t stream);
};

struct NttIo {
  uint32_t batch = 1;
  size_t in_stride = 0, out_stride = 0;
  uint32_t in_len = 0, out_len = 0;
  bool in_coset = false;
  Fr in_coset_mul[2];
  bool out_mul = false, out_coset = false;
  Fr out_mul_v[3];
  cq_ctx* prof = nullptr;
  bool critical = false;
};

int ntt_run(const NttTables& tb, const Fr* in, Fr* out, Fr* scratch, const NttIo& io, hipStream_t stream);

}
```

sha2_on_cq_halo2_amd/csrc/pk.hip:

```cpp
#include <algorithm>
#include <cstring>
#include <string>
#include <vector>
#include "building.hpp"
#include "cq.hpp"
#include "ctx.hpp"
#include "g1fft.hpp"
#include "msm.hpp"
#include "plonk.hpp"
#include "poly.hpp"
#include "serde.hpp"

using namespace cq;

size_t cq::static_table_rows(const cq_static_table* t) { return t->N; }

namespace {
void put_be32(uint8_t*& o, uint32_t v) {
  o[0] = (uint8_t)(v >> 24); o[1] = (uint8_t)(v >> 16); o[2] = (uint8_t)(v >> 8); o[3] = (uint8_t)v;
  o += 4;
}
int unit_coset(cq_pk* pk, size_t row, Fr* tmp, Fr* dst) {
  cq_ctx* c = pk->ctx;
  const size_t n = (size_t)1 << pk->k, ext = pk->domain->ext();
// ... 246 lines not shown
  if (b0_g1_bound && b0_on_device) {
    pk->b0_g1_bound = (G1Affine*)b0_g1_bound;
  } else if (b0_g1_bound) {
    if ((rc = c->dev_alloc(&pk->b0_g1_bound, n - 1, "b0 bound")) != CQ_OK) return rc;
    pk->own_b0 = true;
    CQ_HIP(c, hipMemcpyAsync(pk->b0_g1_bound, b0_g1_bound, (n - 1) * sizeof(G1Affine), hipMemcpyHostToDevice, c->stream));
  }
  for (auto& lk : pk->lookups) {
    G1Affine* cat = nullptr;
    const size_t N = cfg->N;
    if ((rc = c->dev_alloc(&cat, lk.tables.size() * N, "qs")) != CQ_OK) return rc;
    pk->qs_concat.push_back(cat);
    for (size_t j = 0; j < lk.tables.size(); j++)
      CQ_HIP(c, hipMemcpyAsync(cat + j * N, lk.tables[j]->qs, N * sizeof(G1Affine), hipMemcpyDeviceToDevice, c->stream));
  }
  if ((rc = pk_small_tables(pk)) != CQ_OK) return rc;
  CQ_HIP(c, hipStreamSynchronize(c->stream));
  if (!pk->lookups.empty() && pk->b0_g1_bound && cfg->N + 1 <= ((size_t)1 << (MSM_TABLE_C - 1)) && n >= 2) {
    const G1Affine* src[2] = {pk->params->g, pk->b0_g1_bound};
    for (int q = 0; q < 2; q++) {
      if ((rc = c->dev_alloc(&pk->b_row_bases[q], n, "b row bases")) != CQ_OK) return rc;
      if ((rc = g1_to_lagrange_shifted(c, src[q], (uint32_t)(n - 1), 1, pk->k, pk->b_row_bases[q])) != CQ_OK) return rc;
      if (msm_bases29(c, pk->b_row_bases[q], (uint32_t)n, pk->b_row_bases[q]) != 0) return c->fail(CQ_ERR_HIP, "b row bases");
    }
    CQ_HIP(c, hipStreamSynchronize(c->stream));
  }
  return CQ_OK;
}

static int pk_create_impl(cq_ctx* c, cq_params* params, const cq_circuit* cs, cq_table_config* cfg, const uint64_t* b0_g1_bound,
                          int b0_on_device, PkStreamReader* in, cq_pk** out) {
  if (!c || !params || !cs || !out) return CQ_ERR_ARG;
  *out = nullptr;
  cq_pk_desc desc;
  std::string why;
  int rc = pk_describe(cs, params->k, cfg ? &cfg->N : nullptr, b0_g1_bound != nullptr, in != nullptr,
                       PkLimits{CQ_MAX_LOOKUPS, CQ_MAX_WIDTH, PERM_MAX_COLUMNS, PERM_MAX_CHUNK}, &desc, &why);
  if (rc != CQ_OK) return c->fail(rc, why);
  CQ_HIP(c, hipSetDevice(c->device));
  cq_pk* pk = new cq_pk();
  Building<cq_pk> guard(pk, cq_pk_destroy, c);
  static_cast<cq_pk_desc&>(*pk) = std::move(desc);
  pk->ctx = c;
  pk->params = params;
  pk->table_cfg = cfg;
  pk->vk_repr = Fr::from_limbs64(cs->vk_repr);
  params->key_users++;
  if (cfg) cfg->key_users++;
  pk->counted_users = true;
  if ((rc = pk_upload_programs(pk, cs->plonk)) != CQ_OK) return rc;
  if ((rc = domain_create(c, pk->cs_degree, pk->k, &pk->domain)) != CQ_OK) return rc;
  if ((rc = pk_alloc_polys(pk)) != CQ_OK) return rc;
  if ((rc = in ? pk_read_polys(pk, *in) : pk_keygen_polys(pk, cs->plonk)) != CQ_OK) return rc;
  if ((rc = pk_attach_bases(pk, b0_g1_bound, b0_on_device)) != CQ_OK) return rc;
  *out = guard.release();
  return CQ_OK;
}

extern "C" {

int cq_pk_create(cq_ctx* c, cq_params* params, const cq_circuit* cs, cq_table_config* cfg, const uint64_t* b0_g1_bound,
                 int b0_on_device, cq_pk** out) {
  return pk_create_impl(c, params, cs, cfg, b0_g1_bound, b0_on_device, nullptr, out);
}

int cq_pk_read_raw(cq_ctx* c, cq_params* params, const cq_circuit* cs, cq_table_config* cfg, const uint64_t* b0_g1_bound,
                   int b0_on_device, const uint8_t* buf, size_t len, uint32_t num_selectors, int checked, cq_pk** out) {
  if (!buf) return CQ_ERR_ARG;
  PkStreamReader in{buf, len, num_selectors, checked != 0, false};
  return pk_create_impl(c, params, cs, cfg, b0_g1_bound, b0_on_device, &in, out);
}

int cq_pk_read(cq_ctx* c, cq_params* params, const cq_circuit* cs, cq_table_config* cfg, const uint64_t* b0_g1_bound, int b0_on_device,
               const uint8_t* buf, size_t len, uint32_t num_selectors, int format, cq_pk** out) {
  if (!buf) return CQ_ERR_ARG;
  if (format != CQ_SERDE_PROCESSED && format != CQ_SERDE_RAW_BYTES && format != CQ_SERDE_RAW_BYTES_UNCHECKED)
    return c ? c->fail(CQ_ERR_ARG, "pk: unknown serde format") : CQ_ERR_ARG;
  PkStreamReader in{buf, len, num_selectors, format == CQ_SERDE_RAW_BYTES, format == CQ_SERDE_PROCESSED};
  return pk_create_impl(c, params, cs, cfg, b0_g1_bound, b0_on_device, &in, out);
}

static size_t pk_stream_size(const cq_pk* pk, uint32_t num_selectors, size_t point_bytes) {
  if (!pk) return 0;
  const size_t n = (size_t)1 << pk->k, ext = pk->domain->ext(), F = pk->num_fixed, PC = pk->perm_columns.size();
  const size_t poly_n = 4 + n * sizeof(Fr), poly_e = 4 + ext * sizeof(Fr);
  return 8 + (F + PC) * point_bytes + (size_t)num_selectors * ((n + 7) / 8) + 3 * poly_e + 3 * 4 + F * (2 * poly_n + poly_e) + 3 * 4 +
         PC * (2 * poly_n + poly_e);
}
size_t cq_pk_raw_size(const cq_pk* pk, uint32_t num_selectors) { return pk_stream_size(pk, num_selectors, sizeof(G1Affine)); }
size_t cq_pk_serialized_size(const cq_pk* pk, int format, uint32_t num_selectors) {
  if (format == CQ_SERDE_PROCESSED) return pk_stream_size(pk, num_selectors, 32);
  if (format == CQ_SERDE_RAW_BYTES || format == CQ_SERDE_RAW_BYTES_UNCHECKED) return pk_stream_size(pk, num_selectors, sizeof(G1Affine));
  return 0;
}

static int pk_write_impl(cq_pk* pk, bool processed, const uint8_t* selector_bits, uint32_t num_selectors, uint8_t* buf, size_t cap,
                         size_t* written) {
  if (!pk || !buf || !written || (num_selectors && !selector_bits)) return CQ_ERR_ARG;
  cq_ctx* c = pk->ctx;
  CQ_HIP(c, hipSetDevice(c->device));
  const size_t n = (size_t)1 << pk->k, ext = pk->domain->ext(), F = pk->num_fixed, PC = pk->perm_columns.size();
  const size_t total = pk_stream_size(pk, num_selectors, processed ? 32 : sizeof(G1Affine));
  if (cap < total) return c->fail(CQ_ERR_ARG, "pk: output buffer too small");
  uint8_t* o = buf;
  put_be32(o, pk->k);
  put_be32(o, (uint32_t)F);
// ... 101 lines not shown
    pk->dropped_cfg_tables = true;
  }
  struct Use { const G1Affine* b; size_t len; };
  std::vector<Use> uses{{pk->params->g_lagrange, n}, {pk->params->g, n}, {pk->params->g, n - 1}};
  if (has_cfg) {
    uses.push_back({pk->table_cfg->g1_lagrange, N});
    uses.push_back({pk->table_cfg->g_lagrange_opening_at_0, N});
  }
  if (pk->b0_g1_bound) uses.push_back({pk->b0_g1_bound, n - 1});
  std::vector<std::pair<const G1Affine*, const G1Affine*>> iv;
  for (auto& u : uses) {
    size_t lo, hi;
    shard_range(u.len, pk->shard_rank, pk->shard_world, lo, hi);
    if (hi > lo) iv.push_back({u.b + lo, u.b + hi});
  }
  std::sort(iv.begin(), iv.end());
  std::vector<std::pair<const G1Affine*, const G1Affine*>> merged;
  for (auto& x : iv) {
    if (!merged.empty() && x.first <= merged.back().second) merged.back().second = std::max(merged.back().second, x.second);
    else merged.push_back(x);
  }
  for (auto& m : merged) {
    bool held = false;
    const size_t len = (size_t)(m.second - m.first);
    if ((rc = msm_register_tables(c, m.first, len, pk->table_c, &held)) != CQ_OK) return rc;
    if (held) pk->shard_tables.push_back({m.first, len, pk->table_c});
  }
  return CQ_OK;
}

int cq_pk_set_sharding(cq_pk* pk, uint32_t rank, uint32_t world, cq_allgather_fn fn, void* user) {
  if (!pk || world == 0 || rank >= world) return CQ_ERR_ARG;
  cq_ctx* c = pk->ctx;
  if (world > 1 && !fn && (!c->rccl_comm || c->rccl_world != world || c->rccl_rank != rank))
    return c->fail(CQ_ERR_ARG, "set_sharding: no all-gather callback and no matching RCCL communicator on the context");
  CQ_HIP(c, hipSetDevice(c->device));
  CQ_HIP(c, hipStreamSynchronize(c->stream));
  pk->shard_rank = rank;
  pk->shard_world = world;
  pk->shard_single = world == 1 && !fn && c->rccl_comm && c->rccl_world == 1;
  pk->allgather = world > 1 ? fn : nullptr;
  pk->allgather_user = user;
  int rc = pk_shard_tables(pk);
  if (rc != CQ_OK) return rc;
  CQ_HIP(c, hipStreamSynchronize(c->stream));
  return CQ_OK;
}

void cq_pk_destroy(cq_pk* pk) {
  if (!pk) return;
  hipStreamSynchronize(pk->ctx->stream);
  if (pk->domain) domain_destroy(pk->domain);
  if (pk->l_active_row) hipFree(pk->l_active_row);
  for (void* p : {(void*)pk->fixed_values, (void*)pk->fixed_polys, (void*)pk->fixed_cosets, (void*)pk->l0, (void*)pk->l_last,
                  (void*)pk->gate_prog, (void*)pk->constants, (void*)pk->lookup_prog, (void*)pk->legacy_prog, (void*)pk->perm_values, (void*)pk->perm_polys, (void*)pk->perm_cosets,
                  (void*)pk->omega_powers, (void*)pk->ext_pow_lo, (void*)pk->ext_pow_hi})
    if (p) hipFree(p);
  if (pk->shard_world > 1 || pk->dropped_params_tables || pk->dropped_cfg_tables) {
    pk->shard_world = 1;
    (void)pk_shard_tables(pk);
  }
  for (auto& t : pk->held_tables) msm_release_table(pk->ctx, t.bases, t.n, t.c);
  for (int q = 0; q < 2; q++)
    if (pk->b_row_bases[q]) hipFree(pk->b_row_bases[q]);
  if (pk->own_b0 && pk->b0_g1_bound) {
    msm_unregister_tables(pk->ctx, pk->b0_g1_bound);
    hipFree(pk->b0_g1_bound);
  }
  for (auto p : pk->qs_concat) {
    msm_unregister_tables(pk->ctx, p);
    hipFree(p);
  }
  if (pk->counted_users) {
    cq_params* params = pk->params;
    cq_table_config* cfg = pk->table_cfg;
    if (--params->key_users == 0 && params->owner_released) cq_params_destroy(params);
    if (cfg && --cfg->key_users == 0 && cfg->owner_released) cq_table_config_destroy(cfg);
  }
  delete pk;
}

}
```

sha2_on_cq_halo2_amd/csrc/pk.hpp:

```cpp
#pragma once
#include <algorithm>
#include <cstdint>
#include <string>
#include <utility>
#include <vector>
#include "../../include/cq_halo2.h"

namespace cq {
size_t static_table_rows(const cq_static_table* t);
bool gate_program_check(const uint32_t* lens, const uint32_t* words, uint32_t num_polys, uint32_t num_constants,
                        uint32_t num_advice, uint32_t num_fixed, uint32_t num_instance, uint32_t num_challenges,
                        const char** why, size_t* total_words);
}

struct cq_lookup_desc {
  std::vector<uint32_t> cols;
  std::vector<int64_t> prog;
  std::vector<cq_static_table*> tables;
};

struct cq_pk_desc {
  uint32_t k = 0, num_advice = 0, bf = 0, u = 0;
  std::vector<cq_lookup_desc> lookups;
  std::vector<std::pair<uint32_t, int32_t>> advice_queries;
  uint32_t num_fixed = 0, num_instance = 0, cs_degree = 3;
  std::vector<std::pair<uint32_t, int32_t>> fixed_queries;
  uint32_t num_gate_polys = 0;
  bool lookup_exprs = false;
  struct LegacyLookup { uint32_t width; size_t in_off, tab_off; };
  std::vector<LegacyLookup> legacy;
  std::vector<std::pair<uint32_t, uint32_t>> perm_columns;
  std::vector<uint8_t> advice_phase;
  std::vector<uint8_t> challenge_phase;
  uint32_t num_phases = 1;
  bool general() const { return num_gate_polys || !perm_columns.empty() || !legacy.empty(); }
  size_t perm_sets() const {
    const size_t chunk = cs_degree - 2;
    return (perm_columns.size() + chunk - 1) / chunk;
  }
  int32_t point_rotation(int32_t rot) const {
    const int64_t n = (int64_t)1 << k, r = (((int64_t)rot % n) + n) % n;
    return (int32_t)(r >= (n + 1) / 2 ? r - n : r);
  }
  std::vector<int32_t> opening_rotations() const {
    std::vector<int32_t> rots{0};
    auto seen = [&](int32_t rot) {
      const int32_t r = point_rotation(rot);
      if (std::find(rots.begin(), rots.end(), r) == rots.end()) rots.push_back(r);
    };
    for (auto& q : advice_queries) seen(q.second);
    for (auto& q : fixed_queries) seen(q.second);
    if (perm_sets() || !legacy.empty()) seen(1);
    if (!legacy.empty()) seen(-1);
    if (perm_sets() > 1) seen(-(int32_t)(bf + 1));
    return rots;
  }
};

namespace cq {

struct PkLimits {
  uint32_t lookups, width, perm_columns, perm_chunk;
};

inline std::vector<uint32_t> pack_programs(const uint32_t* lens, const uint32_t* words, size_t count, std::vector<size_t>* offsets = nullptr) {
  std::vector<uint32_t> blob;
  for (size_t i = 0; i < count; i++) {
    if (offsets) offsets->push_back(blob.size());
    blob.push_back(lens[i]);
    blob.insert(blob.end(), words, words + lens[i]);
    words += lens[i];
// ... 146 lines not shown
```

sha2_on_cq_halo2_amd/csrc/poly.hip:

```cpp
#include "poly.hpp"
#include "field29.hpp"
#include <algorithm>
#include <cstring>
#include "ctx.hpp"

namespace cq {

static __device__ __forceinline__ Fr ld(const Fr* p) {
  const uint4* q = reinterpret_cast<const uint4*>(p);
  uint4 a = q[0], b = q[1];
  Fr r;
  r.v.l[0] = a.x; r.v.l[1] = a.y; r.v.l[2] = a.z; r.v.l[3] = a.w;
  r.v.l[4] = b.x; r.v.l[5] = b.y; r.v.l[6] = b.z; r.v.l[7] = b.w;
  return r;
}
static __device__ __forceinline__ void ld8w(const Fr* p, uint32_t* w) {
  const uint4* q = reinterpret_cast<const uint4*>(p);
  const uint4 a = q[0], b = q[1];
  w[0] = a.x; w[1] = a.y; w[2] = a.z; w[3] = a.w;
  w[4] = b.x; w[5] = b.y; w[6] = b.z; w[7] = b.w;
}
static __device__ __forceinline__ void st(Fr* p, const Fr& r) {
  uint4* q = reinterpret_cast<uint4*>(p);
  q[0] = make_uint4(r.v.l[0], r.v.l[1], r.v.l[2], r.v.l[3]);
// ... 229 lines not shown
    __syncthreads();
    Fr29::mul_pair(below, inc, suf, above, inc, suf);
  }
  bi_put29(lo, hi, t, inc);
  bi_put29(lo2, hi2, t, suf);
  __syncthreads();
  Fr29 exc = t ? bi_get29(lo, hi, t - 1) : Fr29::one();
  const Fr29 total = bi_get29(lo, hi, 255);
  const Fr29 after = t < 255 ? bi_get29(lo2, hi2, t + 1) : Fr29::one();
  __syncthreads();
  if (t == 0) {
    Fr tc;
    total.pack(tc.v.l);
    Fr::cond_sub_p(tc.v.l, 0);
    bi_put(lo, hi, 0, tc.inv_safegcd_var());
  }
  if constexpr (IO::kNumerator) exc = IO::scaled_for_numerator(exc);
  const Fr29 exc_b = Fr29::mul(exc, total_a);
  __syncthreads();
  const Fr29 total_inv = bi_get29(lo, hi, 0);
  Fr29 r = Fr29::mul(total_inv, after);
  auto prefix = [&](int k) {
    uint32_t w[8] = {0, 0, 0, 0, 0, 0, 0, 0};
    if (nz[k]) ld8w(io.slot(base + k * 256 + t), w);
    return Fr29::unpack(w);
  };
  auto emit = [&](int k, const Fr29& out) {
    if constexpr (!IO::kNumerator) io.emit(base + k * 256 + t, nz[k], out);
  };
  Fr29::static_for<0, H>([&](auto K) {
    constexpr int k1 = BI_PER_LANE - 1 - 2 * decltype(K)::value, k0 = k1 - 1;
    Fr29 b1, b0, o1, o0;
    Fr29::mul_pair(k1 >= H ? exc_b : exc, prefix(k1), k0 >= H ? exc_b : exc, prefix(k0), b1, b0);
    Fr29::mul_pair(b1, r, r, elem(k1), o1, r);
    Fr29::mul_pair(b0, r, r, elem(k0), o0, r);
    if constexpr (IO::kNumerator) {
      const auto c1 = io.cell(base + k1 * 256 + t, n), c0 = io.cell(base + k0 * 256 + t, n);
      IO::times_numerators(c1, o1, c0, o0);
      c1.emit(nz[k1], o1);
      c0.emit(nz[k0], o0);
    } else {
      emit(k1, o1);
      emit(k0, o0);
    }
  });
}
template <int BI_PER_LANE>
__global__ __launch_bounds__(256) void batch_invert_kernel(Fr* __restrict__ a, uint32_t n) {
  CQ_CRITICAL_WAVES();
  batch_invert_block<BI_PER_LANE>(BiInPlace{a}, n);
}

#include "assigned_kernels.hpp"

__global__ __launch_bounds__(256) void lincomb_kernel(LincombArgs args, uint32_t n, Fr* __restrict__ out) {
  __shared__ uint32_t cf[LINCOMB_MAX][9];
  for (uint32_t j = threadIdx.x; j < args.count; j += blockDim.x) {
    const Fr29 c = Fr29::unpack(args.coeff[j].v.l);
    CQ_UNROLL for (int l = 0; l < 9; l++) cf[j][l] = c.a[l];
  }
  __syncthreads();
  const uint32_t i = blockIdx.x * blockDim.x + threadIdx.x;
  if (i >= n) return;
  Fr29 acc = Fr29::zero();
  uint64_t col[18];
  for (uint32_t j0 = 0; j0 < args.count; j0 += 6) {
    CQ_UNROLL for (int k = 0; k < 18; k++) col[k] = 0;
    const uint32_t j1 = min(args.count, j0 + 6);
    for (uint32_t j = j0; j < j1; j++) {
      if (i >= args.len[j]) continue;
      uint32_t w[8];
      ld8w(args.p[j] + i, w);
      Fr29 c;
      CQ_UNROLL for (int l = 0; l < 9; l++) c.a[l] = cf[j][l];
      Fr29::mac(col, Fr29::unpack(w), c);
    }
    acc = acc + Fr29::redc(col);
    acc.normalise();
  }
  uint32_t w[8];
  acc.to_canonical_words(w);
  Fr r;
  CQ_UNROLL for (int k = 0; k < 8; k++) r.v.l[k] = w[k];
  if (i == 0) r = r - args.sub_const;
  st(out + i, r);
}

__global__ __launch_bounds__(256) void from_u512_kernel(const uint64_t* __restrict__ words, uint32_t n, Fr* __restrict__ out) {
  CQ_CRITICAL_WAVES();
  const uint32_t i = blockIdx.x * blockDim.x + threadIdx.x;
  if (i >= n) return;
  uint64_t w[8];
  for (int k = 0; k < 8; k++) w[k] = words[(size_t)i * 8 + k];
  st(out + i, Fr::from_u512(w));
}

__global__ __launch_bounds__(256) void cq_b_denominators_kernel(const Fr* __restrict__ f, uint32_t n, uint32_t u, Fr beta,
                                                                Fr* __restrict__ out) {
  const uint32_t i = blockIdx.x * blockDim.x + threadIdx.x;
  if (i >= n) return;
  st(out + i, i < u ? ld(f + i) + beta : beta);
}

struct CqQuotientConsts {
  Fr y261;
  Fr beta_32;
  Fr one_1024;
  Fr c_1024;
  Fr scale261;
};
__global__ __launch_bounds__(256) void cq_quotient_kernel(CqQuotientArgs args, CqQuotientConsts k, uint32_t ext, Fr* h) {
  const uint32_t i = blockIdx.x * blockDim.x + threadIdx.x;
  if (i >= ext) return;
  uint32_t w8[8];
  auto load29 = [&](const Fr* p) {
    ld8w(p, w8);
    return Fr29::unpack(w8);
  };
  const Fr29 la = load29(args.l_active + i);
  const Fr29 y = Fr29::unpack(k.y261.v.l), beta = Fr29::unpack(k.beta_32.v.l), one = Fr29::unpack(k.one_1024.v.l);
  Fr29 acc = Fr29::zero();
  if (args.h_in) acc = Fr29::mul(load29(args.h_in + i), Fr29::unpack(k.c_1024.v.l));
  for (uint32_t l = 0; l < args.count; l++) {
    const Fr29 b = load29(args.b[l] + i), f = load29(args.f[l] + i);
    Fr29 w = Fr29::mul(f, la) + beta;
    w.normalise();
    uint64_t col[18];
    CQ_UNROLL for (int q = 0; q < 18; q++) col[q] = 0;
    Fr29::mac(col, acc, y);
    Fr29::mac(col, b, w);
    acc = Fr29::sub<2>(Fr29::redc(col), one);
  }
  acc = Fr29::mul(acc, Fr29::unpack(k.scale261.v.l));
  if (args.t_len) acc = Fr29::mul(acc, load29(args.t_evals + (i & (args.t_len - 1))));
  acc.pack(w8);
  Fr::cond_sub_p(w8, 0);
  Fr r;
  CQ_UNROLL for (int q = 0; q < 8; q++) r.v.l[q] = w8[q];
  st(h + i, r);
}

__global__ void fill_usable_rows_kernel(Fr* out, uint32_t n, uint32_t u) {
  const uint32_t i = blockIdx.x * blockDim.x + threadIdx.x;
  if (i >= n) return;
  st(out + i, i < u ? Fr::one() : Fr::zero());
}

__global__ __launch_bounds__(256) void advice_fill_kernel(AdviceFillArgs a, const Fr* __restrict__ tails, uint32_t n, uint32_t u) {
  const uint32_t col = blockIdx.y;
  const uint32_t h = blockIdx.x * blockDim.x + threadIdx.x;
  if (h >= 2 * n) return;
  const uint32_t i = h >> 1;
  const uint4* src = i < u ? reinterpret_cast<const uint4*>(a.src[col]) + h
                           : reinterpret_cast<const uint4*>(tails + (size_t)col * (n - u)) + (h - 2 * u);
  reinterpret_cast<uint4*>(a.dst[col])[h] = *src;
}
__global__ void gather_scalars_kernel(GatherArgs a, Fr* out) {
  CQ_CRITICAL_WAVES();
  const uint32_t i = threadIdx.x;
  if (i < a.count) st(out + i, ld(a.src[i]));
}

static inline uint32_t blocks_for(uint32_t n) { return (n + 255) / 256; }

int poly_eval_batch(cq_ctx* c, const Fr* const* p, const uint32_t* len, uint32_t count, const Fr& z, Fr* out_host) {
  if (count == 0) return CQ_OK;
  if (count > EVAL_MAX_BATCH) return c->fail(CQ_ERR_ARG, "eval: batch too large");
  EvalBatchArgs args;
  uint32_t maxlen = 0;
  for (uint32_t i = 0; i < count; i++) {
    args.p[i] = p[i];
    args.len[i] = len[i];
    args.cur_len[i] = len[i];
    maxlen = std::max(maxlen, len[i]);
  }
  if (maxlen == 0) {
    for (uint32_t i = 0; i < count; i++) out_host[i] = Fr::zero();
    return CQ_OK;
  }
  const uint32_t nb0 = (maxlen + EVAL_TILE - 1) / EVAL_TILE;
  void* scr;
  int rc;
  if ((rc = c->ensure_scratch(Scratch::PolyTmp, ((size_t)count * (nb0 + 8) * 2) * sizeof(Fr), &scr)) != CQ_OK) return rc;
  Fr* buf[2] = {(Fr*)scr, (Fr*)scr + (size_t)count * (nb0 + 8)};
  const uint32_t stride = nb0 + 8;
  Fr x = z;
  const Fr* level_in = nullptr;
// ... 96 lines not shown
  if (per == 4) batch_invert_kernel<4><<<(n + 256 * 4 - 1) / (256 * 4), 256, 0, c->stream>>>(a, n);
  else if (per == 8) batch_invert_kernel<8><<<(n + 256 * 8 - 1) / (256 * 8), 256, 0, c->stream>>>(a, n);
  else batch_invert_kernel<16><<<(n + 256 * 16 - 1) / (256 * 16), 256, 0, c->stream>>>(a, n);
  return hipGetLastError() == hipSuccess ? CQ_OK : c->fail(CQ_ERR_HIP, "batch_invert launch failed");
}

int poly_validate_assigned(cq_ctx* c, const uint32_t* off, uint32_t ncols, const uint32_t* rows_dev, uint32_t nrows, uint32_t* verdict_dev) {
  if (hipMemsetAsync(verdict_dev, 0xff, sizeof(uint32_t), c->stream) != hipSuccess) return c->fail(CQ_ERR_HIP, "assigned: verdict reset failed");
  for (uint32_t c0 = 0; c0 < ncols; c0 += ASSIGNED_MAX_COLS) {
    AssignedCols cols{};
    cols.count = std::min(ASSIGNED_MAX_COLS, ncols - c0);
    for (uint32_t j = 0; j <= cols.count; j++) cols.off[j] = off[c0 + j] - off[c0];
    const uint32_t total = cols.off[cols.count];
    if (total) assigned_validate_kernel<<<blocks_for(total), 256, 0, c->stream>>>(cols, rows_dev + off[c0], nrows, off[c0], verdict_dev);
  }
  return hipGetLastError() == hipSuccess ? CQ_OK : c->fail(CQ_ERR_HIP, "assigned validate launch failed");
}

int poly_resolve_assigned(cq_ctx* c, const Fr* const* num, Fr* const* out, const uint32_t* off, uint32_t ncols, const uint32_t* rows_dev,
                          const Fr* den_dev, uint32_t nrows, Fr* work_dev, const uint32_t* verdict_dev) {
  for (uint32_t c0 = 0; c0 < ncols; c0 += ASSIGNED_MAX_COLS) {
    AssignedCols cols{};
    cols.count = std::min(ASSIGNED_MAX_COLS, ncols - c0);
    bool copies = false;
    for (uint32_t j = 0; j < cols.count; j++) {
      cols.num[j] = num[c0 + j];
      cols.out[j] = out[c0 + j];
      copies |= cols.out[j] != cols.num[j];
    }
    for (uint32_t j = 0; j <= cols.count; j++) cols.off[j] = off[c0 + j] - off[c0];
    const uint32_t total = cols.off[cols.count];
    const uint32_t* rows = rows_dev + off[c0];
    const Fr* den = den_dev + off[c0];
    Fr* work = work_dev + off[c0];
    if (copies && nrows) assigned_copy_kernel<<<dim3(blocks_for(2 * nrows), cols.count), 256, 0, c->stream>>>(cols, nrows, verdict_dev);
    if (!total) continue;
    const int per = batch_invert_per_lane(total);
    const uint32_t blocks = (total + 256 * per - 1) / (256 * per);
    if (per == 4) assigned_resolve_kernel<4><<<blocks, 256, 0, c->stream>>>(cols, rows, den, work, nrows, verdict_dev);
    else if (per == 8) assigned_resolve_kernel<8><<<blocks, 256, 0, c->stream>>>(cols, rows, den, work, nrows, verdict_dev);
    else assigned_resolve_kernel<16><<<blocks, 256, 0, c->stream>>>(cols, rows, den, work, nrows, verdict_dev);
  }
  return hipGetLastError() == hipSuccess ? CQ_OK : c->fail(CQ_ERR_HIP, "assigned resolve launch failed");
}

int poly_lincomb(cq_ctx* c, const LincombArgs& args_in, uint32_t n, Fr* out) {
  if (!n) return CQ_OK;
  LincombArgs args = args_in;
  for (uint32_t j = 0; j < args.count; j++) args.coeff[j] = fr_to_r261(args_in.coeff[j]);
  lincomb_kernel<<<blocks_for(n), 256, 0, c->stream>>>(args, n, out);
  return hipGetLastError() == hipSuccess ? CQ_OK : c->fail(CQ_ERR_HIP, "lincomb launch failed");
}

int poly_from_u512(cq_ctx* c, const uint64_t* words_dev, uint32_t n, Fr* out) {
  if (!n) return CQ_OK;
  from_u512_kernel<<<blocks_for(n), 256, 0, c->stream>>>(words_dev, n, out);
  return hipGetLastError() == hipSuccess ? CQ_OK : c->fail(CQ_ERR_HIP, "from_u512 launch failed");
}

int poly_cq_b_denominators(cq_ctx* c, const Fr* f, uint32_t n, uint32_t u, const Fr& beta, Fr* out) {
  cq_b_denominators_kernel<<<blocks_for(n), 256, 0, c->stream>>>(f, n, u, beta, out);
  return hipGetLastError() == hipSuccess ? CQ_OK : c->fail(CQ_ERR_HIP, "cq_b launch failed");
}

int poly_cq_quotient(cq_ctx* c, const CqQuotientArgs& args, uint32_t ext, Fr* h) {
  CqQuotientConsts k;
  const Fr inv32 = Fr::from_u64(32).inv(), inv1024 = inv32 * inv32;
  k.y261 = fr_to_r261(args.y);
  k.beta_32 = args.beta * inv32;
  k.one_1024 = inv1024;
  k.c_1024 = fr_to_r261(inv1024);
  k.scale261 = fr_to_r261((args.has_scale ? args.scale : Fr::one()) * Fr::from_u64(args.t_len ? 32768 : 1024));
  cq_quotient_kernel<<<blocks_for(ext), 256, 0, c->stream>>>(args, k, ext, h);
  return hipGetLastError() == hipSuccess ? CQ_OK : c->fail(CQ_ERR_HIP, "cq_quotient launch failed");
}

int poly_fill_usable_rows(cq_ctx* c, Fr* out, uint32_t n, uint32_t u) {
  fill_usable_rows_kernel<<<blocks_for(n), 256, 0, c->stream>>>(out, n, u);
  return hipGetLastError() == hipSuccess ? CQ_OK : c->fail(CQ_ERR_HIP, "fill launch failed");
}

int poly_advice_fill(cq_ctx* c, const AdviceFillArgs& a, const Fr* tails_dev, uint32_t n, uint32_t u) {
  if (!a.count) return CQ_OK;
  advice_fill_kernel<<<dim3(blocks_for(2 * n), a.count), 256, 0, c->stream>>>(a, tails_dev, n, u);
  return hipGetLastError() == hipSuccess ? CQ_OK : c->fail(CQ_ERR_HIP, "advice fill launch failed");
}

int poly_gather_scalars(cq_ctx* c, const GatherArgs& a, Fr* out_dev) {
  if (!a.count) return CQ_OK;
  gather_scalars_kernel<<<1, GATHER_MAX, 0, c->stream>>>(a, out_dev);
  return hipGetLastError() == hipSuccess ? CQ_OK : c->fail(CQ_ERR_HIP, "gather launch failed");
}

}
```

sha2_on_cq_halo2_amd/csrc/poly.hpp:

```cpp
#pragma once
#include <hip/hip_runtime.h>
#include <vector>
#include "field.hpp"
#include "ntt.hpp"

struct cq_ctx;

namespace cq {

constexpr uint32_t POLY_CHUNK = 16;
constexpr uint32_t LINCOMB_MAX = 40;
constexpr uint32_t CQ_MAX_LOOKUPS = 16;

struct LincombArgs {
  const Fr* p[LINCOMB_MAX];
  uint32_t len[LINCOMB_MAX];
  Fr coeff[LINCOMB_MAX];
  uint32_t count;
  Fr sub_const;
};
inline Fr fr_to_r261(const Fr& x) { return Fr::from_u64(32) * x; }

#ifndef CQ_EVAL_TILE
#define CQ_EVAL_TILE 4096
#endif
constexpr uint32_t EVAL_TILE = CQ_EVAL_TILE;
constexpr uint32_t EVAL_MAX_BATCH = 40;
struct EvalBatchArgs {
  const Fr* p[EVAL_MAX_BATCH];
  uint32_t len[EVAL_MAX_BATCH];
  uint32_t cur_len[EVAL_MAX_BATCH];
};
struct EvalPowers {
  Fr sq[8];
  Fr x256;
};

struct CqQuotientArgs {
  const Fr* b[CQ_MAX_LOOKUPS];
  const Fr* f[CQ_MAX_LOOKUPS];
  uint32_t count;
  const Fr* h_in;
  const Fr* l_active;
  const Fr* t_evals;
  uint32_t t_len;
  Fr y, beta;
  Fr scale;
  uint32_t has_scale = 0;
};

int poly_eval(cq_ctx* c, const Fr* a_dev, uint32_t n, const Fr& z, Fr* out_host);
int poly_eval_batch(cq_ctx* c, const Fr* const* p_dev, const uint32_t* len, uint32_t count, const Fr& z, Fr* out_host);
int poly_kate_division(cq_ctx* c, const Fr* a_dev, uint32_t n, const Fr& z, Fr* q_dev);
int poly_batch_invert(cq_ctx* c, Fr* a_dev, uint32_t n);
constexpr uint32_t ASSIGNED_MAX_COLS = 32;
struct AssignedCols {
  const Fr* num[ASSIGNED_MAX_COLS];
  Fr* out[ASSIGNED_MAX_COLS];
  uint32_t off[ASSIGNED_MAX_COLS + 1];
  uint32_t count;
};
int poly_validate_assigned(cq_ctx* c, const uint32_t* off, uint32_t ncols, const uint32_t* rows_dev, uint32_t nrows, uint32_t* verdict_dev);
int poly_resolve_assigned(cq_ctx* c, const Fr* const* num_dev, Fr* const* out_dev, const uint32_t* off, uint32_t ncols,
                          const uint32_t* rows_dev, const Fr* den_dev, uint32_t nrows, Fr* work_dev, const uint32_t* verdict_dev);
int poly_lincomb(cq_ctx* c, const LincombArgs& args, uint32_t n, Fr* out_dev);
int poly_from_u512(cq_ctx* c, const uint64_t* words_dev, uint32_t n, Fr* out_dev);
int poly_cq_b_denominators(cq_ctx* c, const Fr* f, uint32_t n, uint32_t u, const Fr& beta, Fr* out);
int poly_cq_quotient(cq_ctx* c, const CqQuotientArgs& args, uint32_t ext, Fr* h);
int poly_fill_usable_rows(cq_ctx* c, Fr* out, uint32_t n, uint32_t u);
constexpr uint32_t ADVICE_FILL_MAX = 32;
struct AdviceFillArgs {
  const Fr* src[ADVICE_FILL_MAX];
  Fr* dst[ADVICE_FILL_MAX];
  uint32_t count;
};
int poly_advice_fill(cq_ctx* c, const AdviceFillArgs& a, const Fr* tails_dev, uint32_t n, uint32_t u);
constexpr uint32_t GATHER_MAX = 64;
struct GatherArgs {
  const Fr* src[GATHER_MAX];
  uint32_t count;
};
int poly_gather_scalars(cq_ctx* c, const GatherArgs& a, Fr* out_dev);

}

struct cq_domain {
  cq_ctx* ctx;
  uint32_t j, k, extended_k, quotient_poly_degree;
  cq::Fr omega, omega_inv, extended_omega, extended_omega_inv, g_coset, g_coset_inv, ifft_divisor,
      extended_ifft_divisor, barycentric_weight;
  std::vector<cq::Fr> t_evaluations;
  cq::Fr* t_evaluations_dev = nullptr;
  size_t n() const { return (size_t)1 << k; }
  size_t ext() const { return (size_t)1 << extended_k; }
};

namespace cq {
int domain_create(cq_ctx* c, uint32_t j, uint32_t k, cq_domain** out);
void domain_destroy(cq_domain* d);
int domain_lagrange_to_coeff(cq_domain* d, const Fr* in, Fr* out, uint32_t batch, size_t in_stride, size_t out_stride);
int domain_coeff_to_extended(cq_domain* d, const Fr* in, Fr* out, uint32_t batch, size_t in_stride, size_t out_stride);
int domain_extended_to_coeff(cq_domain* d, const Fr* in, Fr* out );
int domain_fft(cq_ctx* c, const Fr* in, Fr* out, uint32_t log_n, const Fr& omega, uint32_t batch, size_t in_stride,
               size_t out_stride);
}
```

sha2_on_cq_halo2_amd/csrc/prover_lookup.hip:

```cpp
#include "prover_run.hpp"

namespace cq {
namespace prover {

GateEvalArgs ProofRun::lagrange_eval_args(const uint32_t* prog, uint32_t num_polys, const Fr& fold) const {
  GateEvalArgs ga;
  ga.prog = prog;
  ga.num_polys = num_polys;
  ga.constants = pk->constants;
  ga.challenges = B.challenges;
  ga.advice = B.adv;
  ga.fixed = pk->fixed_values;
  ga.instance = B.inst_lag;
  ga.stride = n;
  ga.size = (uint32_t)n;
  ga.rot_scale = 1;
  ga.y = fold;
  return ga;
}
int ProofRun::lagrange_compress(const uint32_t* prog, uint32_t width, const Fr& chal, Fr* dst) {
  return gate_eval(c, lagrange_eval_args(prog, width, chal), dst);
}

int ProofRun::count_multiplicities() {
// ... 96 lines not shown
    for (uint32_t j = 0; j < CQ_MAX_WIDTH; j++) fb.theta_pow[j] = theta_pow[j];
    for (uint32_t q = 0; q < fb.count; q++) {
      const size_t l = l0 + q;
      const uint32_t w = (uint32_t)pk->lookups[l].cols.size();
      fb.width[q] = w;
      for (uint32_t j = 0; j < w; j++) fb.src[q][j] = lk_input[l][j];
      fb.out[q] = owns_lookup(l) ? B.f_lag + l * n : nullptr;
    }
    CQ_TRY(cq_fold_inputs(c, fb, (uint32_t)n));
  }
  if (L || PL) {
    std::vector<const Fr*> sc;
    std::vector<const G1Affine*> bs;
    std::vector<size_t> ln;
    for (size_t l = 0; l < PL; l++)
      for (int which = 2; which <= 3; which++) { sc.push_back(plk_buf(l, which)); bs.push_back(pk->params->g_lagrange); ln.push_back(n); }
    std::vector<int> f_linear(L, 0);
    std::vector<G1Jac> f_host(L);
    for (size_t l = 0; l < L; l++) {
      f_linear[l] = 1;
      for (int64_t pj : pk->lookups[l].prog) f_linear[l] &= pj < 0;
    }
    std::vector<size_t> f_slot(L, 0);
    for (size_t l = 0; l < L; l++)
      if (!f_linear[l]) { f_slot[l] = sc.size(); sc.push_back(B.f_lag + l * n); bs.push_back(pk->params->g_lagrange); ln.push_back(n); }
    const size_t m_first = sc.size();
    if (!early_m)
      for (size_t l = 0; l < L; l++) { sc.push_back(B.m_fr + l * N); bs.push_back(pk->table_cfg->g1_lagrange); ln.push_back(N); }
    std::vector<G1Affine> cm;
    Commit r1;
    const uint64_t seq = c->msm_tail_seq;
    if (!sc.empty()) CQ_TRY(r1.begin(pk, sc, bs, ln));
    if (L && !early_m) CQ_TRY(fork_bucket_sums(seq));
    std::vector<size_t> f_lin;
    for (size_t l = 0; l < L; l++)
      if (f_linear[l]) f_lin.push_back(l);
    struct PoolJoin {
      HostPool& pool;
      HostPool::Ticket t;
      ~PoolJoin() { pool.wait(t); }
    } f_job{c->pool(), nullptr};
    f_job.t = c->pool().submit(f_lin.size(), [&](size_t i) {
      const size_t l = f_lin[i];
      const auto& lcols = pk->lookups[l].cols;
      G1Jac acc = jac_from_affine(advice_commitments[lcols[0]]);
      for (size_t j = 1; j < lcols.size(); j++) acc = jac_add(host_scalar_mul(acc, theta), jac_from_affine(advice_commitments[lcols[j]]));
      f_host[l] = acc;
    });
    {
      AuxFork fork(c);
      CQ_TRY(fork.begin(seq));
      if (resident) {
        CQ_TRY(resident_round1_transforms());
      } else {
        if (L) {
          CQ_TRY(lagrange_to_coeff_cols(B.f_lag, B.f_coeff, L));
          CQ_TRY(coeff_to_extended_cols(B.f_coeff, B.cosets + L * ext, L));
        }
        if (general && I) CQ_TRY(coeff_to_extended_cols(B.inst_coeff, B.inst_cosets, I));
        if (A && S == 0 && !adv_is_coeff) {
          CQ_TRY(lagrange_to_coeff_cols(B.adv, B.adv, A));
          adv_is_coeff = true;
        }
      }
      CQ_TRY(fork.end());
    }
    if (!sc.empty()) CQ_TRY(r1.end(cm));
    c->pool().wait(f_job.t);
    for (size_t q = 0; q < 2 * PL; q++)
      if (!tr.write_point(cm[q])) return c->fail(CQ_ERR_TRANSCRIPT, "permuted lookup commitment is the identity");
    for (size_t l = 0; l < L; l++) {
      const G1Affine f_cm = f_linear[l] ? jac_to_affine(f_host[l]) : cm[f_slot[l]];
      if (!tr.write_point(f_cm)) return c->fail(CQ_ERR_TRANSCRIPT, "f commitment is the identity");
      if (!tr.write_point(early_m ? m_commitments[l] : cm[m_first + l])) return c->fail(CQ_ERR_TRANSCRIPT, "m commitment is the identity");
    }
  }
  return CQ_OK;
}

int ProofRun::legacy_commit_product() {
  for (size_t l = 0; l < PL; l++)
    CQ_TRY(lookup_product(c, plk_buf(l, 0), plk_buf(l, 1), plk_buf(l, 2), plk_buf(l, 3), beta, gamma, plkz_tails.data() + l * bf, (uint32_t)n, bf,
                          plk_buf(l, 4)));
  return CQ_OK;
}

int ProofRun::cq_round2() {
  bool random_late = false;
  CQ_TRY(round2_prepare());
  CQ_TRY(round2_random_late(random_late));
  return round2_commit(random_late);
}
int ProofRun::round2_prepare() {
  for (size_t l0 = 0; l0 < L; l0 += CQ_FOLD_BATCH) {
    CqFoldBatch fb;
    fb.count = (uint32_t)std::min<size_t>(CQ_FOLD_BATCH, L - l0);
    for (uint32_t j = 0; j < CQ_MAX_WIDTH; j++) fb.theta_pow[j] = theta_pow[j];
    for (uint32_t q = 0; q < fb.count; q++) {
      const size_t l = l0 + q;
      const cq_lookup_desc& lk = pk->lookups[l];
      fb.width[q] = (uint32_t)lk.cols.size();
      for (uint32_t j = 0; j < fb.width[q]; j++) fb.src[q][j] = lk.tables[j]->values;
      fb.out[q] = nullptr;
      fb.f[q] = owns_lookup(l) ? B.f_lag + l * n : nullptr;
      fb.b[q] = B.bpoly + l * n;
      fb.m[q] = B.m_counts + l * N;
// ... 38 lines not shown
}
int ProofRun::round2_random_late(bool& random_late) {
  const char* force = getenv("CQ_RANDOM_LATE");
  const auto t0 = std::chrono::steady_clock::now();
  while (!drawer.done.load()) {
    if (force && force[0] == '1') break;
    const double waited = std::chrono::duration<double, std::micro>(std::chrono::steady_clock::now() - t0).count();
    if (!(force && force[0] == '0') && waited > 100.0 && drawer.remaining_us() > 700.0) break;
    std::this_thread::yield();
  }
  CQ_TRY(shard_any(pk, (force && force[0] == '1') || !drawer.done.load(), random_late));
  return CQ_OK;
}
int ProofRun::round2_commit(bool random_late) {
  if (!random_late) CQ_TRY(finish_random_poly());
  std::vector<G1Affine> r2;
  {
    std::vector<const Fr*> sc;
    std::vector<const G1Affine*> bs;
    std::vector<size_t> ln;
    std::vector<size_t> at;
    for (size_t l = 0; b_by_rows && l < L; l++)
      for (size_t q = 0; q < 2; q++) { sc.push_back(B.b_values + l * (N + 1)); bs.push_back(B.b_sums + (2 * l + q) * (N + 1)); ln.push_back(N + 1); }
    for (size_t st = 0; st < S; st++) { at.push_back(sc.size()); sc.push_back(B.z + st * n); bs.push_back(pk->params->g_lagrange); ln.push_back(n); }
    for (size_t l = 0; l < PL; l++) { at.push_back(sc.size()); sc.push_back(plk_buf(l, 4)); bs.push_back(pk->params->g_lagrange); ln.push_back(n); }
    size_t woff = 0;
    for (size_t l = 0; l < L; l++) {
      const uint32_t w = (uint32_t)pk->lookups[l].cols.size();
      at.push_back(sc.size()); sc.push_back(B.a_val + l * N); bs.push_back(pk->table_cfg->g1_lagrange); ln.push_back(N);
      at.push_back(sc.size()); sc.push_back(B.a_scaled + woff * N); bs.push_back(pk->qs_concat[l]); ln.push_back((size_t)w * N);
      at.push_back(sc.size()); sc.push_back(B.a_val + l * N); bs.push_back(pk->table_cfg->g_lagrange_opening_at_0); ln.push_back(N);
      if (b_by_rows) {
        at.push_back(2 * l);
        at.push_back(2 * l + 1);
      } else {
        at.push_back(sc.size()); sc.push_back(B.bpoly + l * n + 1); bs.push_back(pk->params->g); ln.push_back(n - 1);
        at.push_back(sc.size()); sc.push_back(B.bpoly + l * n + 1); bs.push_back(pk->b0_g1_bound); ln.push_back(n - 1);
      }
      woff += w;
    }
    if (!random_late) { at.push_back(sc.size()); sc.push_back(B.random_poly); bs.push_back(pk->params->g); ln.push_back(n); }
    Commit r2cm;
    const uint64_t seq = c->msm_tail_seq;
    if (sums_pending) {
      CQ_HIP(c, hipStreamWaitEvent(s, c->b_sums_done, 0));
      sums_pending = false;
    }
    CQ_TRY(r2cm.begin(pk, sc, bs, ln));
    {
      AuxFork fork(c);
      CQ_TRY(fork.begin(seq));
      if (A && !adv_is_coeff) CQ_TRY(lagrange_to_coeff_cols(B.adv, B.adv, A));
      if (resident) CQ_TRY(resident_b_to_coset());
      else if (L) CQ_TRY(coeff_to_extended_cols(B.bpoly, B.cosets, L));
      if (general && A) CQ_TRY(coeff_to_extended_cols(B.adv, B.adv_cosets, A));
      CQ_TRY(fork.end());
    }
    if (random_late) CQ_TRY(finish_random_poly());
    mark("round 2 queued");
    {
      std::vector<G1Affine> in_launch_order;
      CQ_TRY(r2cm.end(in_launch_order));
      for (size_t i : at) r2.push_back(in_launch_order[i]);
    }
    mark("round 2 commitments on the host");
    if (random_late) {
      std::vector<G1Affine> rc;
      CQ_TRY(commit_batch(pk, {B.random_poly}, {pk->params->g}, n, rc));
      r2.push_back(rc[0]);
    }
  }
  for (size_t st = 0; st < S; st++)
    if (!tr.write_point(r2[st])) return c->fail(CQ_ERR_TRANSCRIPT, "permutation product commitment is the identity");
  if (S) CQ_TRY(lagrange_to_coeff_cols(B.z, B.z, S));
  for (size_t l = 0; l < PL; l++) {
    if (!tr.write_point(r2[S + l])) return c->fail(CQ_ERR_TRANSCRIPT, "lookup product commitment is the identity");
    CQ_TRY(domain_lagrange_to_coeff(dom, plk_buf(l, 2), plk_buf(l, 2), 3, n, n));
  }
  for (size_t l = 0; l < L; l++) {
    for (size_t q = 0; q < 5; q++)
      if (!tr.write_point(r2[S + PL + 5 * l + q])) return c->fail(CQ_ERR_TRANSCRIPT, "a CQ round-2 commitment is the identity");
  }
  random_cm = r2[S + PL + 5 * L];
  if (L) {
    if (resident) CQ_TRY(resident_sum_b_at_zero());
    const Fr n_table_inv = Fr::from_u64(N).inv();
    for (size_t l = 0; l < L; l++)
      a_at_zero[l] = (small_fr[l] * Fr::from_u64(n) - Fr::from_u64(bf + 1) * beta_inv) * n_table_inv;
  }
  return CQ_OK;
}

}
}
```

sha2_on_cq_halo2_amd/csrc/prover_quotient.hip:

```cpp
#include "prover_run.hpp"

namespace cq {
namespace prover {

int perm_products(const cq_pk* pk, const Fr* const* cols, const Fr& beta, const Fr& gamma, const Fr* z_tails, Fr* mv, Fr* z) {
  cq_ctx* c = pk->ctx;
  const hipStream_t s = c->stream;
  const size_t n = (size_t)1 << pk->k, S = pk->perm_sets(), PC = pk->perm_columns.size(), chunk_len = pk->cs_degree - 2;
  const uint32_t bf = pk->bf, u = pk->u;
  const Fr delta = fr_from_raw(FR_DELTA_RAW);
  std::vector<PermProductArgs> pa(S);
  Fr deltaomega = Fr::one();
  for (size_t st = 0; st < S; st++) {
    PermProductArgs& a = pa[st];
    a.count = (uint32_t)std::min(chunk_len, PC - st * chunk_len);
    a.beta = beta;
    a.gamma = gamma;
    a.omega_powers = pk->omega_powers;
    for (uint32_t j = 0; j < a.count; j++) {
      const size_t ci = st * chunk_len + j;
      a.col[j] = cols[ci];
      a.sigma[j] = pk->perm_values + ci * n;
      a.delta_beta[j] = deltaomega * beta;
      deltaomega = deltaomega * delta;
// ... 93 lines not shown
    }
    LookupHArgs la;
    la.a = co;
    la.s = co + ext;
    la.z = co + 2 * ext;
    la.cin = co + 3 * ext;
    la.ctab = co + 4 * ext;
    la.l0 = pk->l0;
    la.l_last = pk->l_last;
    la.l_active = pk->l_active_row;
    la.beta = t.beta;
    la.gamma = t.gamma;
    la.y = t.y;
    la.ext = (uint32_t)ext;
    la.rot_scale = rot_scale;
    CQ_TRY(lookup_h_terms(c, la, h_ext));
  }
  return CQ_OK;
}

int ProofRun::permutation_commit() {
  if (!S) return CQ_OK;
  std::vector<const Fr*> cols(PC);
  for (size_t ci = 0; ci < PC; ci++) {
    const auto& col = pk->perm_columns[ci];
    cols[ci] = col.first == CQ_COL_ADVICE ? B.adv + (size_t)col.second * n
             : col.first == CQ_COL_FIXED  ? pk->fixed_values + (size_t)col.second * n
                                          : B.inst_lag + (size_t)col.second * n;
  }
  return perm_products(pk, cols.data(), beta, gamma, z_tails.data(), B.mv, B.z);
}

int ProofRun::evaluate_h() {
  if (general) {
    if (I && !(L || PL)) CQ_TRY(coeff_to_extended_cols(B.inst_coeff, B.inst_cosets, I));
    if (S) CQ_TRY(coeff_to_extended_cols(B.z, B.z_cosets, S));
    std::vector<const Fr*> plk_polys(PL);
    for (size_t l = 0; l < PL; l++) plk_polys[l] = plk_buf(l, 2);
    HTermsArgs ht;
    ht.adv_cosets = B.adv_cosets;
    ht.inst_cosets = B.inst_cosets;
    ht.z_cosets = B.z_cosets;
    ht.challenges = B.challenges;
    ht.plk_polys = plk_polys.data();
    ht.plk_cosets = B.plk_cosets;
    ht.beta = beta;
    ht.gamma = gamma;
    ht.theta = theta;
    ht.y = y;
    CQ_TRY(h_terms(pk, ht, B.h_ext));
  }
  CqQuotientArgs qa;
  qa.h_in = general ? B.h_ext : nullptr;
  qa.l_active = pk->l_active_row;
  qa.t_evals = dom->t_evaluations_dev;
  qa.t_len = (uint32_t)dom->t_evaluations.size();
  qa.y = y;
  qa.beta = beta;
  if (resident) return resident_quotient(qa);
  qa.count = (uint32_t)L;
  for (size_t l = 0; l < L; l++) {
    qa.b[l] = B.cosets + l * ext;
    qa.f[l] = B.cosets + (L + l) * ext;
  }
  return poly_cq_quotient(c, qa, (uint32_t)ext, B.h_ext);
}

int ProofRun::construct_h() {
  if (resident) CQ_TRY(resident_collect_h());
  else CQ_TRY(domain_extended_to_coeff(dom, B.h_ext, B.h_coeff));
  for (size_t i = 0; i < pieces; i++) (void)rng.fr();
  {
    std::vector<const Fr*> sc(pieces);
    std::vector<const G1Affine*> bs(pieces, pk->params->g);
    for (size_t i = 0; i < pieces; i++) sc[i] = B.h_coeff + i * n;
    std::vector<G1Affine> o;
    CQ_TRY(commit_batch(pk, sc, bs, n, o));
    for (auto& p : o)
      if (!tr.write_point(p)) return c->fail(CQ_ERR_TRANSCRIPT, "h piece commitment is the identity");
  }
  return CQ_OK;
}

}
}
```

sha2_on_cq_halo2_amd/csrc/prover_run.hpp:

```cpp
#pragma once
#include <algorithm>
#include <array>
#include <atomic>
#include <chrono>
#include <cstdio>
#include <cstdlib>
#include <cstring>
#include <functional>
#include <thread>
#include <vector>
#include "blake2b.hpp"
#include "comm.hpp"
#include "cq.hpp"
#include "ctx.hpp"
#include "msm.hpp"
#include "plonk.hpp"
#include "prover.hpp"
#include "glv.hpp"
#include "xoshiro.hpp"

namespace cq {
namespace prover {

struct Transcript {
// ... 166 lines not shown

struct OpenTranscript {
  std::function<int(Fr&)> squeeze;
  std::function<int(const G1Affine&, const char* what)> write_point;
};
struct OpenJob {
  const cq_pk* pk;
  const std::vector<Query>* qs;
  const std::vector<Fr>* points;
  const std::vector<size_t>* q_h;
  Fr xn;
  Fr *gwc_batch, *gwc_wit;
  Fr* shplonk;
  OpenTranscript tr;
  std::function<int(size_t g, const std::vector<Term>& terms, const Fr& eval_batch, Fr* batch, Fr* wit)> witness;
};
int open_gwc_queries(OpenJob& j);
int open_shplonk_queries(OpenJob& j);

struct RandomPolyDrawer {
  std::thread th;
  bool running = false;
  std::atomic<bool> done{false};
  std::atomic<uint32_t> chunks_done{0};
  uint32_t chunks_total = 1;
  std::chrono::steady_clock::time_point t_start;
  hipError_t err = hipSuccess;
  double remaining_us() const {
    if (done.load()) return 0.0;
    const double el = std::chrono::duration<double, std::micro>(std::chrono::steady_clock::now() - t_start).count();
    const uint32_t d = chunks_done.load();
    return d ? el * (double)(chunks_total - d + 1) / d : 1e9;
  }
  void start(cq_ctx* c, Rng* rng, uint64_t* pin, uint64_t* dev, size_t words);
  int join();
  ~RandomPolyDrawer() {
    if (running) th.join();
  }
};

struct ProofRun {
  cq_pk* const pk;
  cq_ctx* const c = pk->ctx;
  cq_domain* const dom = pk->domain;
  const hipStream_t s = c->stream;
  const uint32_t k = pk->k;
  const size_t n = (size_t)1 << k, ext = dom->ext();
  const uint32_t bf = pk->bf, u = pk->u;
  const size_t L = pk->lookups.size(), A = pk->num_advice, I = pk->num_instance;
  const size_t N = pk->table_cfg ? pk->table_cfg->N : 0;
  const size_t S = pk->perm_sets(), PC = pk->perm_columns.size(), chunk_len = pk->cs_degree - 2;
  const size_t PL = pk->legacy.size(), NC = pk->challenge_phase.size(), pieces = dom->quotient_poly_degree;
  const bool general = pk->general();
  const bool early_m = L > 0 && pk->num_phases == 1 && pk->challenge_phase.empty();
  const bool early_adv = early_advice_polys(pk);
  const bool b_by_rows = L > 0 && !pk->sharded() && pk->b_row_bases[0] != nullptr &&
                         msm_bucket_sums_fit((uint32_t)n, (uint32_t)std::min<size_t>(2 * L, MSM_MAX_BATCH));
  const bool sums_side = b_by_rows && side_switch();
  bool sums_pending = false;
  static bool side_switch() {
    const char* e = getenv("CQ_BUCKET_SUMS_SIDE");
    return !(e && e[0] == '0');
  }

  bool resident = false;
  const uint32_t SW = pk->shard_world, me = pk->shard_rank;
  size_t lk_lo = 0, lk_hi = L, adv_lo = 0, adv_hi = A;
  size_t lk_cnt = L;
  const size_t res_slice_max = (n + pk->shard_world - 1) / pk->shard_world + 1;
  const size_t res_stage_elems = (size_t)pk->shard_world * res_slice_max * (pk->cs_degree > 2 ? pk->cs_degree - 1 : 1) + res_slice_max + 64;
  void* res_stage_v = nullptr;

  Rng rng;
  Transcript tr;
  Buffers B;
  void *pin = nullptr, *small_v = nullptr;
  volatile uint32_t* herr = nullptr;
  Fr* small_fr = nullptr;
  const std::chrono::steady_clock::time_point t_start = std::chrono::steady_clock::now();

  std::vector<Fr> z_tails = std::vector<Fr>(S * bf), plk_tails = std::vector<Fr>(PL * 2 * (bf + 1)), plkz_tails = std::vector<Fr>(PL * bf);
  std::vector<std::array<const Fr*, CQ_MAX_WIDTH>> lk_input = std::vector<std::array<const Fr*, CQ_MAX_WIDTH>>(L);
  std::vector<G1Affine> m_commitments = std::vector<G1Affine>(L, G1Affine::identity());
  std::vector<G1Affine> advice_commitments = std::vector<G1Affine>(A, G1Affine::identity());
  std::vector<Fr> user_challenges = std::vector<Fr>(NC, Fr::zero());
  Fr* adv_poly = nullptr;
  bool adv_is_coeff = false;
  Fr theta, beta, gamma, beta_inv, y, x, xn;
  Fr theta_pow[CQ_MAX_WIDTH];
  std::vector<Fr> a_at_zero = std::vector<Fr>(L);
  G1Affine random_cm = G1Affine::identity();
  std::vector<Query> qs;
  std::vector<size_t> q_h;
  std::vector<int32_t> rots;
  std::vector<Fr> points;
  std::vector<int> qowner;
  size_t my_lo = 0, my_hi = n;
  RandomPolyDrawer drawer;

  ProofRun(cq_pk* pk_, cq_rng_next_u64 rng_next, void* rng_state);
  ~ProofRun();

  void mark(const char* what) const {
    if (host_trace_enabled()) fprintf(stderr, "[cq host] %8.1f us  %s\n", std::chrono::duration<double, std::micro>(std::chrono::steady_clock::now() - t_start).count(), what);
  }
  uint32_t phase_of(size_t a) const { return pk->advice_phase.empty() ? 0u : pk->advice_phase[a]; }
// ... 54 lines not shown
```

sha2_on_cq_halo2_amd/params.py:

```python
from __future__ import annotations

import numpy as np

from ._lib import CqError
from ._marshal import SERDE_PROCESSED, _fr, _g1, _g2, _limbs4, _written
from .context import Context, DevBuf, _Handle, _host_or_device_points


class ParamsKZG(_Handle):

    _destroy = "cq_params_destroy"

    def _open_k(self, k: int, ctx: Context, create, *args) -> "ParamsKZG":
        self.k, self.n = k, 1 << k
        return self._open(ctx, create, *args)

    def __init__(self, ctx: Context, k: int, g: np.ndarray, g_lagrange: np.ndarray):
        g = _g1(g)
        g_lagrange = _g1(g_lagrange)
        assert g.shape[0] == 1 << k and g_lagrange.shape[0] == 1 << k
        self._open_k(k, ctx, ctx.lib.cq_params_create, ctx.h, k, g.ctypes.data, g_lagrange.ctypes.data)

    @classmethod
    def setup_from_toxic_waste(cls, ctx: Context, k: int, s: np.ndarray) -> "ParamsKZG":
# ... 212 lines not shown


class EvaluationDomain(_Handle):

    _destroy = "cq_domain_destroy"

    def __init__(self, ctx: Context, j: int, k: int):
        self._open(ctx, ctx.lib.cq_domain_create, ctx.h, j, k)
        self.j = j
        self.k = k
        self.extended_k = ctx.lib.cq_domain_extended_k(self.h)
        self.n = 1 << k

    @property
    def extended_len(self) -> int:
        return 1 << self.extended_k

    def constants(self):
        arrs = [np.zeros(4, dtype=np.uint64) for _ in range(4)]
        self.ctx._chk(self.ctx.lib.cq_domain_constants(self.h, *[a.ctypes.data for a in arrs]))
        return dict(zip(("omega", "omega_inv", "extended_omega", "ifft_divisor"), arrs))

    def lagrange_to_coeff(self, a: np.ndarray) -> np.ndarray:
        a = _fr(a).copy()
        if a.shape[0] != self.n:
            raise CqError(-1, "lagrange_to_coeff: wrong length")
        self.ctx._chk(self.ctx.lib.cq_lagrange_to_coeff(self.h, a.ctypes.data))
        return a

    def coeff_to_extended(self, a: np.ndarray) -> np.ndarray:
        a = _fr(a)
        if a.shape[0] != self.n:
            raise CqError(-1, "coeff_to_extended: wrong length")
        out = np.zeros((self.extended_len, 4), dtype=np.uint64)
        self.ctx._chk(self.ctx.lib.cq_coeff_to_extended(self.h, a.ctypes.data, out.ctypes.data))
        return out

    def extended_to_coeff(self, a: np.ndarray) -> np.ndarray:
        a = _fr(a)
        if a.shape[0] != self.extended_len:
            raise CqError(-1, "extended_to_coeff: wrong length")
        out = np.zeros((self.n * (self.j - 1), 4), dtype=np.uint64)
        self.ctx._chk(self.ctx.lib.cq_extended_to_coeff(self.h, a.ctypes.data, out.ctypes.data))
        return out

    def lagrange_to_coeff_dev(self, src: DevBuf, dst: DevBuf, batch: int = 1):
        self.ctx._chk(self.ctx.lib.cq_lagrange_to_coeff_dev(self.h, src.ptr, dst.ptr, batch))

    def coeff_to_extended_dev(self, src: DevBuf, dst: DevBuf, batch: int = 1):
        self.ctx._chk(self.ctx.lib.cq_coeff_to_extended_dev(self.h, src.ptr, dst.ptr, batch))

    def extended_to_coeff_dev(self, src: DevBuf, dst: DevBuf):
        self.ctx._chk(self.ctx.lib.cq_extended_to_coeff_dev(self.h, src.ptr, dst.ptr))
```

sha2_on_cq_halo2_amd/proving_key.py:

```python
from __future__ import annotations

import ctypes as C
from typing import NamedTuple

import numpy as np

from ._lib import CqError
from ._marshal import (FAIL_GATE, FAIL_GATE_POISONED, FAIL_LOOKUP, FAIL_PERMUTATION, FAIL_STATIC_LOOKUP, SERDE_PROCESSED,
                       _ALLGATHER_T, _BCAST_T, _EXCHANGE_T, _OPENERS, _PHASE_T, _SQUEEZE_T, _WRITE_POINT_T, _BufferRng, _CqCircuit,
                       _CqOpenQuery, _CqOpenTranscript, _CqPlonk, _ProofBuffer, _assigned_structs, _fr, _g1, _instance_columns,
                       _limbs4, _ptr_array, _struct_of, _written, fr_from_mont, fr_to_mont)
from .context import Context, DevBuf, _Handle
from .params import ParamsKZG, TableConfig


def _lower_plonk(cs, fixed, mapping, keep: list, from_raw: bool = False) -> _CqPlonk:
    pl = _CqPlonk()
    n_fixed = cs.num_fixed_columns
    fixed = [_fr(f) for f in (fixed or [])]
    pl.num_fixed, pl.num_instance = n_fixed, cs.num_instance_columns
    if not from_raw:
        assert len(fixed) == n_fixed, "one value column per fixed column (pk.fixed_values)"
        fptrs = _ptr_array([f.ctypes.data for f in fixed], False)
        keep += [fixed, fptrs]
# ... 114 lines not shown
            self._b0 = b0
            b0_ptr, on_dev = b0.ctypes.data, 0
        shape = (ctx.h, params.h, C.byref(cs_), table_cfg.h if table_cfg is not None else None, b0_ptr, on_dev)
        if raw is None:
            self._open(ctx, ctx.lib.cq_pk_create, *shape)
        else:
            rb = np.frombuffer(raw, dtype=np.uint8)
            if format is not None:
                if checked is not None:
                    raise CqError(-1, "ProvingKey: give `format` or `checked`, not both")
                self._open(ctx, ctx.lib.cq_pk_read, *shape, rb.ctypes.data, rb.shape[0], num_selectors, format)
            else:
                checked = True if checked is None else checked
                self._open(ctx, ctx.lib.cq_pk_read_raw, *shape, rb.ctypes.data, rb.shape[0], num_selectors, 1 if checked else 0)
        self.num_advice = num_advice
        self._num_lookups = len(lookups)
        self._table_size = table_cfg.size if table_cfg is not None else 0
        self.usable_rows = ctx.lib.cq_pk_usable_rows(self.h)
        self.proof_size = ctx.lib.cq_pk_proof_size(self.h)

    @classmethod
    def read(cls, ctx: Context, params: ParamsKZG, k: int, num_advice: int, lookups, table_cfg, b0_g1_bound, vk_repr, data: bytes,
             format: int = SERDE_PROCESSED, cs=None, num_selectors: int = 0) -> "ProvingKey":
        return cls(ctx, params, k, num_advice, lookups, table_cfg, b0_g1_bound, vk_repr, cs=cs, raw=data, num_selectors=num_selectors,
                   format=format)

    def _write(self, size: int, fn, *fmt, selector_bits: bytes, num_selectors: int) -> bytes:
        sel = np.frombuffer(selector_bits, dtype=np.uint8) if num_selectors else None
        return _written(size, lambda buf, size, w: self.ctx._chk(fn(self.h, *fmt, sel.ctypes.data if sel is not None else None,
                                                                    num_selectors, buf, size, w)))

    def write(self, format: int = SERDE_PROCESSED, selector_bits: bytes = b"", num_selectors: int = 0) -> bytes:
        return self._write(self.serialized_size(format, num_selectors), self.ctx.lib.cq_pk_write, format, selector_bits=selector_bits,
                           num_selectors=num_selectors)

    def to_bytes(self, selector_bits: bytes = b"", num_selectors: int = 0) -> bytes:
        return self._write(self.ctx.lib.cq_pk_raw_size(self.h, num_selectors), self.ctx.lib.cq_pk_write_raw, selector_bits=selector_bits,
                           num_selectors=num_selectors)

    def serialized_size(self, format: int = SERDE_PROCESSED, num_selectors: int = 0) -> int:
        return self.ctx.lib.cq_pk_serialized_size(self.h, format, num_selectors)

    def vk_commitments(self):
        nf = self.cs.num_fixed_columns if self.cs is not None else 0
        npc = len(self.cs.permutation_columns) if self.cs is not None else 0
        f = np.zeros((max(nf, 1), 8), dtype=np.uint64)
        p = np.zeros((max(npc, 1), 8), dtype=np.uint64)
        self.ctx._chk(self.ctx.lib.cq_pk_vk_commitments(self.h, f.ctypes.data, p.ctypes.data))
        return f[:nf], p[:npc]

    def b_row_bases(self, which):
        return self.ctx.lib.cq_pk_b_row_bases_dev(self.h, which)

    def set_opener(self, name: str):
        self.ctx._chk(self.ctx.lib.cq_pk_set_opener(self.h, _OPENERS[name]))
        self.proof_size = self.ctx.lib.cq_pk_proof_size(self.h)

    def set_rng_fill(self, name):
        fn = C.cast(self.ctx.lib.cq_opaque_rng_fill, C.c_void_p) if name == "opaque" else None
        self.ctx._chk(self.ctx.lib.cq_pk_set_rng_fill(self.h, fn))

    def _rng(self, rng_words=None, seed=None, opaque=False):
        lib = self.ctx.lib
        if rng_words is not None:
            w = np.ascontiguousarray(rng_words, dtype=np.uint64)
            st = _BufferRng(w.ctypes.data_as(C.POINTER(C.c_uint64)), 0, w.shape[0], 0)
            self._rng_keep = (w, st)
            return C.cast(lib.cq_buffer_rng_next_u64, C.c_void_p), C.cast(C.byref(st), C.c_void_p)
        st = (C.c_uint64 * 4)()
        lib.cq_xoshiro256ss_seed(seed, st)
        self._rng_keep = st
        return C.cast(lib.cq_opaque_rng_next_u64 if opaque else lib.cq_xoshiro256ss_next_u64, C.c_void_p), C.cast(st, C.c_void_p)

    def _run(self, fn, ptrs, rng_fn, rng_state, instances=None, on_device=False) -> bytes:
        arr, out = _ptr_array(ptrs, False), _ProofBuffer(self.proof_size)
        if instances is None:
            self.ctx._chk(fn(self.h, arr, rng_fn, rng_state, *out.args))
        else:
            iptr, ilen, keep = _instance_columns(instances)
            self.ctx._chk(self.ctx.lib.cq_create_proof_instances(self.h, arr, 1 if on_device else 0, iptr, ilen, rng_fn, rng_state,
                                                                 *out.args))
            del keep
        return out.bytes()

    def create_proof(self, advice, rng_words=None, seed=None, instances=None) -> bytes:
        cols = [np.ascontiguousarray(a, dtype=np.uint64) for a in advice]
        assert len(cols) == self.num_advice and all(c.shape == (1 << self.k, 4) for c in cols)
        fn, st = self._rng(rng_words, seed)
        return self._run(self.ctx.lib.cq_create_proof_host, [c.ctypes.data for c in cols], fn, st, instances)

    def create_proof_dev(self, advice_ptrs, rng_words=None, seed=None, instances=None, opaque_rng=False) -> bytes:
        fn, st = self._rng(rng_words, seed, opaque_rng)
        return self._run(self.ctx.lib.cq_create_proof, list(advice_ptrs), fn, st, instances, on_device=True)

    def create_proof_assigned(self, columns, rng_words=None, seed=None, instances=None) -> bytes:
        columns = list(columns)
        assert len(columns) == self.num_advice and all(c.n == 1 << self.k for c in columns)
        fn, st = self._rng(rng_words, seed)
        iptr, ilen, keep = _instance_columns(instances)
        out = _ProofBuffer(self.proof_size)
        self.ctx._chk(self.ctx.lib.cq_create_proof_assigned(self.h, _assigned_structs(columns), iptr, ilen, fn, st, *out.args))
        del keep
        return out.bytes()

    def create_proof_phases(self, advice_bufs, phase_fn, rng_words=None, seed=None, instances=None) -> bytes:
        fn, st = self._rng(rng_words, seed)
# ... 245 lines not shown
```

Before: 1439.

## Compute quotient over coset-major layout with size-n NTTs instead of extended NTT

For non-general circuits with a 2n extended domain, polynomials are moved to the extended evaluation domain as two size-n coset NTTs, with per-coset twiddle scaling applied at load time. The quotient comes back via a batched size-n inverse NTT plus a coset-solve kernel that recombines the halves. Lookup inputs are folded in coefficient form by a new fold kernel, so each lookup needs one transform instead of per-column ones. This should cut extended-NTT cost and transforms, at the price of extra twiddle loads, a new coset-major l_active buffer and more complex NTT indexing.

```diff
diff --git a/include/cq_halo2.h b/include/cq_halo2.h
--- a/include/cq_halo2.h
+++ b/include/cq_halo2.h
@@ -105,6 +105,10 @@
 int cq_lagrange_to_coeff_dev(cq_domain* domain, const uint64_t* in_dev, uint64_t* out_dev, uint32_t batch);
 int cq_coeff_to_extended_dev(cq_domain* domain, const uint64_t* in_dev, uint64_t* out_dev, uint32_t batch);
 int cq_extended_to_coeff_dev(cq_domain* domain, const uint64_t* in_dev, uint64_t* out_dev);
+int cq_coeff_to_cosets_dev(cq_domain* domain, const uint64_t* in_dev, uint64_t* out_dev, uint32_t batch);
+int cq_cosets_to_coeff_dev(cq_domain* domain, const uint64_t* in_dev, uint64_t* out_dev);
+int cq_fold_columns_dev(cq_ctx* ctx, const uint64_t* const* cols_dev, uint32_t width, const uint64_t theta[4], size_t n,
+                        uint64_t* out_dev);
 
 int cq_params_create(cq_ctx* ctx, uint32_t k, const uint64_t* g, const uint64_t* g_lagrange, cq_params** out);
 int cq_params_setup_from_toxic_waste(cq_ctx* ctx, uint32_t k, const uint64_t s[4], cq_params** out);
@@ -248,6 +252,7 @@
 int cq_pk_set_rng_fill(cq_pk* pk, cq_rng_fill_fn fill);
 void cq_pk_destroy(cq_pk* pk);
 uint32_t cq_pk_usable_rows(const cq_pk* pk);
+int cq_pk_coset_quotient(const cq_pk* pk);
 const uint64_t* cq_pk_b_row_bases_dev(const cq_pk* pk, int which);
 size_t cq_pk_proof_size(const cq_pk* pk);
 int cq_create_proof(cq_pk* pk, const uint64_t* const* advice_dev, cq_rng_next_u64 rng, void* rng_state,
diff --git a/include/cq_halo2_sys.rs b/include/cq_halo2_sys.rs
--- a/include/cq_halo2_sys.rs
+++ b/include/cq_halo2_sys.rs
@@ -266,6 +266,9 @@
     pub fn cq_lagrange_to_coeff_dev(domain: *mut CqDomain, in_dev: *const u64, out_dev: *mut u64, batch: u32) -> c_int;
     pub fn cq_coeff_to_extended_dev(domain: *mut CqDomain, in_dev: *const u64, out_dev: *mut u64, batch: u32) -> c_int;
     pub fn cq_extended_to_coeff_dev(domain: *mut CqDomain, in_dev: *const u64, out_dev: *mut u64) -> c_int;
+    pub fn cq_coeff_to_cosets_dev(domain: *mut CqDomain, in_dev: *const u64, out_dev: *mut u64, batch: u32) -> c_int;
+    pub fn cq_cosets_to_coeff_dev(domain: *mut CqDomain, in_dev: *const u64, out_dev: *mut u64) -> c_int;
+    pub fn cq_fold_columns_dev(ctx: *mut CqCtx, cols_dev: *const *const u64, width: u32, theta: *const u64 , n: usize, out_dev: *mut u64) -> c_int;
     pub fn cq_params_create(ctx: *mut CqCtx, k: u32, g: *const u64, g_lagrange: *const u64, out: *mut *mut CqParams) -> c_int;
     pub fn cq_params_setup_from_toxic_waste(ctx: *mut CqCtx, k: u32, s: *const u64 , out: *mut *mut CqParams) -> c_int;
     pub fn cq_fixed_base_mul_dev(ctx: *mut CqCtx, scalars_dev: *const u64, n: usize, out_affine_dev: *mut u64) -> c_int;
@@ -334,6 +337,7 @@
     pub fn cq_pk_set_rng_fill(pk: *mut CqPk, fill: CqRngFillFn) -> c_int;
     pub fn cq_pk_destroy(pk: *mut CqPk);
     pub fn cq_pk_usable_rows(pk: *const CqPk) -> u32;
+    pub fn cq_pk_coset_quotient(pk: *const CqPk) -> c_int;
     pub fn cq_pk_b_row_bases_dev(pk: *const CqPk, which: c_int) -> *const u64;
     pub fn cq_pk_proof_size(pk: *const CqPk) -> usize;
     pub fn cq_create_proof(pk: *mut CqPk, advice_dev: *const *const u64, rng: CqRngNextU64, rng_state: *mut c_void, proof: *mut u8, proof_cap: usize, proof_len: *mut usize) -> c_int;
diff --git a/sha2_on_cq_halo2_amd/csrc/capi_cq.hip b/sha2_on_cq_halo2_amd/csrc/capi_cq.hip
--- a/sha2_on_cq_halo2_amd/csrc/capi_cq.hip
+++ b/sha2_on_cq_halo2_amd/csrc/capi_cq.hip
@@ -208,6 +208,7 @@
 }
 
 uint32_t cq_pk_usable_rows(const cq_pk* pk) { return pk ? pk->u : 0; }
+int cq_pk_coset_quotient(const cq_pk* pk) { return pk && pk->coset_quotient() ? 1 : 0; }
 const uint64_t* cq_pk_b_row_bases_dev(const cq_pk* pk, int which) {
   return pk && (which == 0 || which == 1) ? (const uint64_t*)pk->b_row_bases[which] : nullptr;
 }
diff --git a/sha2_on_cq_halo2_amd/csrc/capi_poly.hip b/sha2_on_cq_halo2_amd/csrc/capi_poly.hip
--- a/sha2_on_cq_halo2_amd/csrc/capi_poly.hip
+++ b/sha2_on_cq_halo2_amd/csrc/capi_poly.hip
@@ -75,6 +75,34 @@
   return domain_extended_to_coeff(d, (const Fr*)in_dev, (Fr*)out_dev);
 }
 
+int cq_coeff_to_cosets_dev(cq_domain* d, const uint64_t* in_dev, uint64_t* out_dev, uint32_t batch) {
+  if (!d || !in_dev || !out_dev || !batch) return CQ_ERR_ARG;
+  if ((const void*)in_dev == (const void*)out_dev) return d->ctx->fail(CQ_ERR_ARG, "coeff_to_cosets: in == out");
+  CQ_HIP(d->ctx, hipSetDevice(d->ctx->device));
+  return domain_coeff_to_cosets(d, (const Fr*)in_dev, (Fr*)out_dev, batch, d->n(), d->ext());
+}
+int cq_cosets_to_coeff_dev(cq_domain* d, const uint64_t* in_dev, uint64_t* out_dev) {
+  if (!d || !in_dev || !out_dev) return CQ_ERR_ARG;
+  CQ_HIP(d->ctx, hipSetDevice(d->ctx->device));
+  return domain_cosets_to_coeff(d, (const Fr*)in_dev, (Fr*)out_dev);
+}
+int cq_fold_columns_dev(cq_ctx* c, const uint64_t* const* cols_dev, uint32_t width, const uint64_t theta[4], size_t n, uint64_t* out_dev) {
+  if (!c || !cols_dev || !theta || !out_dev || !width || width > FOLD_MAX_WIDTH || n > 0x7fffffffull) return CQ_ERR_ARG;
+  CQ_HIP(c, hipSetDevice(c->device));
+  FoldCoeffArgs fa;
+  fa.count = 1;
+  fa.width[0] = width;
+  fa.out[0] = (Fr*)out_dev;
+  for (uint32_t j = 0; j < width; j++) {
+    if (!cols_dev[j]) return CQ_ERR_ARG;
+    fa.src[0][j] = (const Fr*)cols_dev[j];
+  }
+  const Fr th = Fr::from_limbs64(theta);
+  fa.theta_pow261[0] = Fr::one();
+  for (uint32_t j = 1; j < FOLD_MAX_WIDTH; j++) fa.theta_pow261[j] = fa.theta_pow261[j - 1] * th;
+  return poly_fold_coeff(c, fa, (uint32_t)n);
+}
+
 int cq_lagrange_to_coeff(cq_domain* d, uint64_t* a) {
   if (!d || !a) return CQ_ERR_ARG;
   cq_ctx* c = d->ctx;
diff --git a/sha2_on_cq_halo2_amd/csrc/coset_kernels.hpp b/sha2_on_cq_halo2_amd/csrc/coset_kernels.hpp
--- /dev/null
+++ b/sha2_on_cq_halo2_amd/csrc/coset_kernels.hpp
@@ -0,0 +1,62 @@
+#pragma once
+
+__global__ __launch_bounds__(256) void fold_coeff_kernel(FoldCoeffArgs args, uint32_t n) {
+  const uint32_t l = blockIdx.y, i = blockIdx.x * blockDim.x + threadIdx.x;
+  if (i >= n) return;
+  const uint32_t w = args.width[l];
+  if (!w) return;
+  Fr29 acc = Fr29::zero();
+  uint64_t col[18];
+  for (uint32_t j0 = 0; j0 < w; j0 += 6) {
+    CQ_UNROLL for (int k = 0; k < 18; k++) col[k] = 0;
+    const uint32_t j1 = min(w, j0 + 6);
+    for (uint32_t j = j0; j < j1; j++) {
+      uint32_t v[8];
+      ld8w(args.src[l][j] + i, v);
+      Fr29::mac(col, Fr29::unpack(v), Fr29::unpack(args.theta_pow261[w - 1 - j].v.l));
+    }
+    acc = acc + Fr29::redc(col);
+    acc.normalise();
+  }
+  uint32_t v[8];
+  acc.to_canonical_words(v);
+  Fr r;
+  CQ_UNROLL for (int k = 0; k < 8; k++) r.v.l[k] = v[k];
+  st(args.out[l] + i, r);
+}
+
+__global__ __launch_bounds__(256) void coset_solve_kernel(Fr* io, const Fr* tw_full, const Fr* tw_lo, const Fr* tw_hi, uint32_t tw_l,
+                                                          CosetSolveConsts k, uint32_t n) {
+  CQ_CRITICAL_WAVES();
+  const uint32_t i = blockIdx.x * blockDim.x + threadIdx.x;
+  if (i >= n) return;
+  const Fr u0 = ld(io + i);
+  Fr u1 = ld(io + n + i);
+  if (i) {
+    uint32_t v[8], t[8];
+    if (tw_full) {
+      ld8w(tw_full + i, t);
+    } else {
+      ld8w(tw_lo + (i & ((1u << tw_l) - 1)), t);
+      if (i >> tw_l) {
+        ld8w(tw_hi + (i >> tw_l), v);
+        Fr29::mul(Fr29::unpack(t), Fr29::unpack(v)).pack(t);
+        Fr::cond_sub_p(t, 0);
+      }
+    }
+    Fr29::mul(Fr29::unpack(u1.v.l), Fr29::unpack(t)).pack(v);
+    Fr::cond_sub_p(v, 0);
+    CQ_UNROLL for (int q = 0; q < 8; q++) u1.v.l[q] = v[q];
+  }
+  Fr lo, hi;
+  coset_solve(k, u0, u1, lo, hi);
+  st(io + i, lo);
+  st(io + n + i, hi);
+}
+
+__global__ void to_coset_major_kernel(const Fr* __restrict__ in, Fr* __restrict__ out, uint32_t log_n, uint32_t log_cosets) {
+  const uint32_t o = blockIdx.x * blockDim.x + threadIdx.x;
+  if (o >> (log_n + log_cosets)) return;
+  const uint32_t j = o >> log_n, m = o & ((1u << log_n) - 1);
+  st(out + o, ld(in + ((m << log_cosets) + j)));
+}
diff --git a/sha2_on_cq_halo2_amd/csrc/coset_solve.hpp b/sha2_on_cq_halo2_amd/csrc/coset_solve.hpp
--- /dev/null
+++ b/sha2_on_cq_halo2_amd/csrc/coset_solve.hpp
@@ -0,0 +1,24 @@
+#pragma once
+#include "field.hpp"
+
+namespace cq {
+
+struct CosetSolveConsts {
+  Fr c0, inv_c0_c1;
+};
+
+inline Fr coset_load_scale(const Fr& zeta, const Fr& w_ext, uint64_t j, uint64_t i) {
+  return zeta.pow_u64(i % 3) * w_ext.pow_u64(i * j);
+}
+inline CosetSolveConsts coset_solve_consts(const Fr& zeta, const Fr& w_ext, uint64_t n) {
+  CosetSolveConsts k;
+  k.c0 = zeta.pow_u64(n);
+  k.inv_c0_c1 = (k.c0 - (zeta * w_ext).pow_u64(n)).inv();
+  return k;
+}
+CQ_HD void coset_solve(const CosetSolveConsts& k, const Fr& u0, const Fr& u1, Fr& lo, Fr& hi) {
+  hi = (u0 - u1) * k.inv_c0_c1;
+  lo = u0 - k.c0 * hi;
+}
+
+}
diff --git a/sha2_on_cq_halo2_amd/csrc/cq.hpp b/sha2_on_cq_halo2_amd/csrc/cq.hpp
--- a/sha2_on_cq_halo2_amd/csrc/cq.hpp
+++ b/sha2_on_cq_halo2_amd/csrc/cq.hpp
@@ -128,6 +128,8 @@
   bool own_b0 = false;
   cq::G1Affine* b_row_bases[2] = {nullptr, nullptr};
   cq::Fr* l_active_row = nullptr;
+  cq::Fr* l_active_cosets = nullptr;
+  bool coset_quotient() const { return l_active_cosets != nullptr && !sharded(); }
   cq::Fr* fixed_values = nullptr;
   cq::Fr* fixed_polys = nullptr;
   cq::Fr* fixed_cosets = nullptr;
diff --git a/sha2_on_cq_halo2_amd/csrc/domain.hip b/sha2_on_cq_halo2_amd/csrc/domain.hip
--- a/sha2_on_cq_halo2_amd/csrc/domain.hip
+++ b/sha2_on_cq_halo2_amd/csrc/domain.hip
@@ -62,7 +62,7 @@
   const size_t n = (size_t)1 << log_n;
   const bool aux = c->aux_stream && c->stream == c->aux_stream;
   void* scr;
-  if ((rc = c->ensure_scratch(aux ? Scratch::NttAux : Scratch::Ntt, (size_t)2 * io.batch * n * sizeof(Fr), &scr)) != CQ_OK) return rc;
+  if ((rc = c->ensure_scratch(aux ? Scratch::NttAux : Scratch::Ntt, (size_t)2 * ((size_t)io.batch << io.log_cosets) * n * sizeof(Fr), &scr)) != CQ_OK) return rc;
   io.prof = c;
   io.critical = !aux;
   if (ntt_run(*tb, in, out, (Fr*)scr, io, c->stream) != 0) return c->fail(CQ_ERR_HIP, "ntt launch failed");
@@ -118,4 +118,42 @@
   return run(d->ctx, d->extended_k, d->extended_omega_inv, in, out, io);
 }
 
+int domain_coeff_to_cosets(cq_domain* d, const Fr* in, Fr* out, uint32_t batch, size_t in_stride, size_t out_stride) {
+  int rc = CQ_OK;
+  NttIo io;
+  io.batch = batch;
+  io.in_stride = in_stride;
+  io.out_stride = out_stride;
+  io.in_len = io.out_len = (uint32_t)d->n();
+  io.in_coset = true;
+  io.in_coset_mul[0] = d->g_coset;
+  io.in_coset_mul[1] = d->g_coset_inv;
+  io.log_cosets = d->extended_k - d->k;
+  if (io.log_cosets) {
+    io.coset_tb = d->ctx->tables_for(d->extended_k, d->extended_omega, &rc);
+    if (!io.coset_tb) return rc;
+  }
+  return run(d->ctx, d->k, d->omega, in, out, io);
 }
+
+int domain_cosets_to_coeff(cq_domain* d, const Fr* in, Fr* out) {
+  cq_ctx* c = d->ctx;
+  if (d->extended_k != d->k + 1 || d->quotient_poly_degree != 2) return c->fail(CQ_ERR_ARG, "cosets_to_coeff: the extended domain is not 2n");
+  int rc = CQ_OK;
+  const NttTables* inv_tb = c->tables_for(d->extended_k, d->extended_omega_inv, &rc);
+  if (!inv_tb) return rc;
+  const size_t n = d->n();
+  NttIo io;
+  io.batch = 2;
+  io.in_stride = io.out_stride = n;
+  io.in_len = io.out_len = (uint32_t)n;
+  io.out_mul = true;
+  io.out_coset = true;
+  io.out_mul_v[0] = d->ifft_divisor;
+  io.out_mul_v[1] = d->ifft_divisor * d->g_coset_inv;
+  io.out_mul_v[2] = d->ifft_divisor * d->g_coset;
+  if ((rc = run(c, d->k, d->omega_inv, in, out, io)) != CQ_OK) return rc;
+  return poly_coset_solve(c, out, *inv_tb, coset_solve_consts(d->g_coset, d->extended_omega, (uint64_t)n), (uint32_t)n);
+}
+
+}
diff --git a/sha2_on_cq_halo2_amd/csrc/ntt.hip b/sha2_on_cq_halo2_amd/csrc/ntt.hip
--- a/sha2_on_cq_halo2_amd/csrc/ntt.hip
+++ b/sha2_on_cq_halo2_amd/csrc/ntt.hip
@@ -59,6 +59,8 @@
   if (j >= count) return;
   g_store29(t + j, Fr29::mul(g_load29(t + j), const29(CONSTS29<FrP>.from256)), true);
 }
+
+#include "ntt_coset.hpp"
 
 #ifdef CQ_NTT_TRACE
 __device__ uint64_t g_ntt_trace[4 * 65536];
@@ -118,8 +120,9 @@
   const uint32_t p = 1u << a.lgp;
   const uint32_t tile = blockIdx.x;
   const uint32_t batch = blockIdx.y;
-  const Fr* in = a.in + (size_t)batch * a.in_stride;
-  Fr* out = a.out + (size_t)batch * a.out_stride;
+  const uint32_t cs = batch & ((1u << a.in_cosets) - 1u);
+  const Fr* in = a.in + (size_t)(batch >> a.in_cosets) * a.in_stride;
+  Fr* out = a.out + (size_t)(batch >> a.out_cosets) * a.out_stride + ((size_t)(batch & ((1u << a.out_cosets) - 1u)) << a.log_n);
   const uint32_t index0 = tile * T;
   const bool first = a.lgp == 0, last = a.next_deg == 0;
   constexpr bool SWZ = !DYN && LOG_T == 4;
@@ -152,6 +155,7 @@
     if (g < a.in_len) {
       x = g_load29(in + g);
       if (load_mul) x = Fr29::mul(x, lds_load29(cl29 + (g % 3) * 9, 1, 0));
+      if (cs && g) x = coset_scale29(x, a, g * cs);
     }
     lds_store29(smem29, E, at(i, c), x);
   }
@@ -319,7 +323,9 @@
       if (found) break;
     }
   }
-  Fr* sbuf[2] = {scratch, scratch + (size_t)io.batch * n};
+  if (io.log_cosets && (!io.in_coset || !io.coset_tb || io.coset_tb->log_n != log_n + io.log_cosets)) return -1;
+  const uint32_t nbatch = io.batch << io.log_cosets;
+  Fr* sbuf[2] = {scratch, scratch + (size_t)nbatch * n};
   const Fr* src = in;
   uint32_t lgp = 0;
   for (uint32_t ps = 0; ps < npass; ps++) {
@@ -354,9 +360,17 @@
         a.in_coset[0] = io.in_coset_mul[0];
         a.in_coset[1] = io.in_coset_mul[1];
       }
+      if (io.log_cosets) {
+        a.in_cosets = io.log_cosets;
+        a.ctw_lo = io.coset_tb->tw_lo;
+        a.ctw_hi = io.coset_tb->tw_hi;
+        a.ctw_full = io.coset_tb->tw_full;
+        a.ctw_l = io.coset_tb->tw_l;
+      }
     }
     if (last) {
       a.out_len = io.out_len;
+      a.out_cosets = io.log_cosets;
       const Fr fix = io.in_coset ? Fr::one() : Fr::from_u64(32);
       if (io.out_mul || !io.in_coset) {
         a.flags |= NTT_OUT_MUL;
@@ -369,7 +383,7 @@
       }
     }
     const uint32_t T = 1u << log_t;
-    dim3 grid(t / T, io.batch);
+    dim3 grid(t / T, nbatch);
     const size_t lds = ((size_t)(T << degs[ps]) + ((size_t)1 << degs[ps]) / 2 + 1) * 36 + 54 * 4;
     hipEvent_t pe = io.prof ? io.prof->prof_begin(CQ_PROF_NTT_PASS) : nullptr;
     constexpr uint32_t LT = NTT_TILE_ELEMS == 512 ? 9 : NTT_TILE_ELEMS == 2048 ? 11 : 10;
diff --git a/sha2_on_cq_halo2_amd/csrc/ntt.hpp b/sha2_on_cq_halo2_amd/csrc/ntt.hpp
--- a/sha2_on_cq_halo2_amd/csrc/ntt.hpp
+++ b/sha2_on_cq_halo2_amd/csrc/ntt.hpp
@@ -39,6 +39,11 @@
   uint32_t out_len;
   Fr in_coset[2];
   Fr out_mul[3];
+  uint32_t in_cosets = 0, out_cosets = 0;
+  const Fr* ctw_lo = nullptr;
+  const Fr* ctw_hi = nullptr;
+  const Fr* ctw_full = nullptr;
+  uint32_t ctw_l = 0;
 };
 
 struct NttTables {
@@ -64,6 +69,8 @@
   Fr in_coset_mul[2];
   bool out_mul = false, out_coset = false;
   Fr out_mul_v[3];
+  uint32_t log_cosets = 0;
+  const NttTables* coset_tb = nullptr;
   cq_ctx* prof = nullptr;
   bool critical = false;
 };
diff --git a/sha2_on_cq_halo2_amd/csrc/ntt_coset.hpp b/sha2_on_cq_halo2_amd/csrc/ntt_coset.hpp
--- /dev/null
+++ b/sha2_on_cq_halo2_amd/csrc/ntt_coset.hpp
@@ -0,0 +1,13 @@
+#pragma once
+
+static __device__ __forceinline__ Fr29 coset_scale29(const Fr29& x, const NttPassArgs& a, uint32_t ex) {
+  Fr29 w;
+  if (a.ctw_full) {
+    w = g_load29(a.ctw_full + ex);
+  } else {
+    w = g_load29(a.ctw_lo + (ex & ((1u << a.ctw_l) - 1)));
+    const uint32_t h = ex >> a.ctw_l;
+    if (h) w = canon29(Fr29::mul(w, g_load29(a.ctw_hi + h)));
+  }
+  return Fr29::mul(x, w);
+}
diff --git a/sha2_on_cq_halo2_amd/csrc/pk.hip b/sha2_on_cq_halo2_amd/csrc/pk.hip
--- a/sha2_on_cq_halo2_amd/csrc/pk.hip
+++ b/sha2_on_cq_halo2_amd/csrc/pk.hip
@@ -322,6 +322,10 @@
   if ((rc = domain_create(c, pk->cs_degree, pk->k, &pk->domain)) != CQ_OK) return rc;
   if ((rc = pk_alloc_polys(pk)) != CQ_OK) return rc;
   if ((rc = in ? pk_read_polys(pk, *in) : pk_keygen_polys(pk, cs->plonk)) != CQ_OK) return rc;
+  if (!pk->general() && !pk->lookups.empty() && pk->domain->extended_k == pk->k + 1) {
+    if ((rc = c->dev_alloc(&pk->l_active_cosets, pk->domain->ext(), "l_active_row, coset-major")) != CQ_OK) return rc;
+    if ((rc = poly_to_coset_major(c, pk->l_active_row, pk->l_active_cosets, pk->k, 1)) != CQ_OK) return rc;
+  }
   if ((rc = pk_attach_bases(pk, b0_g1_bound, b0_on_device)) != CQ_OK) return rc;
   *out = guard.release();
   return CQ_OK;
@@ -529,6 +533,7 @@
   hipStreamSynchronize(pk->ctx->stream);
   if (pk->domain) domain_destroy(pk->domain);
   if (pk->l_active_row) hipFree(pk->l_active_row);
+  if (pk->l_active_cosets) hipFree(pk->l_active_cosets);
   for (void* p : {(void*)pk->fixed_values, (void*)pk->fixed_polys, (void*)pk->fixed_cosets, (void*)pk->l0, (void*)pk->l_last,
                   (void*)pk->gate_prog, (void*)pk->constants, (void*)pk->lookup_prog, (void*)pk->legacy_prog, (void*)pk->perm_values, (void*)pk->perm_polys, (void*)pk->perm_cosets,
                   (void*)pk->omega_powers, (void*)pk->ext_pow_lo, (void*)pk->ext_pow_hi})
diff --git a/sha2_on_cq_halo2_amd/csrc/pk.hpp b/sha2_on_cq_halo2_amd/csrc/pk.hpp
--- a/sha2_on_cq_halo2_amd/csrc/pk.hpp
+++ b/sha2_on_cq_halo2_amd/csrc/pk.hpp
@@ -17,6 +17,11 @@
   std::vector<uint32_t> cols;
   std::vector<int64_t> prog;
   std::vector<cq_static_table*> tables;
+  bool plain_advice() const {
+    for (int64_t p : prog)
+      if (p >= 0) return false;
+    return true;
+  }
 };
 
 struct cq_pk_desc {
diff --git a/sha2_on_cq_halo2_amd/csrc/poly.hip b/sha2_on_cq_halo2_amd/csrc/poly.hip
--- a/sha2_on_cq_halo2_amd/csrc/poly.hip
+++ b/sha2_on_cq_halo2_amd/csrc/poly.hip
@@ -305,6 +305,7 @@
 }
 
 #include "assigned_kernels.hpp"
+#include "coset_kernels.hpp"
 
 __global__ __launch_bounds__(256) void lincomb_kernel(LincombArgs args, uint32_t n, Fr* __restrict__ out) {
   __shared__ uint32_t cf[LINCOMB_MAX][9];
@@ -385,7 +386,7 @@
     acc = Fr29::sub<2>(Fr29::redc(col), one);
   }
   acc = Fr29::mul(acc, Fr29::unpack(k.scale261.v.l));
-  if (args.t_len) acc = Fr29::mul(acc, load29(args.t_evals + (i & (args.t_len - 1))));
+  if (args.t_len) acc = Fr29::mul(acc, load29(args.t_evals + (args.coset_log_n ? i >> args.coset_log_n : (i & (args.t_len - 1)))));
   acc.pack(w8);
   Fr::cond_sub_p(w8, 0);
   Fr r;
@@ -588,6 +589,25 @@
   return hipGetLastError() == hipSuccess ? CQ_OK : c->fail(CQ_ERR_HIP, "lincomb launch failed");
 }
 
+int poly_fold_coeff(cq_ctx* c, const FoldCoeffArgs& args_in, uint32_t n) {
+  if (!n || !args_in.count) return CQ_OK;
+  FoldCoeffArgs args = args_in;
+  for (uint32_t j = 0; j < FOLD_MAX_WIDTH; j++) args.theta_pow261[j] = fr_to_r261(args_in.theta_pow261[j]);
+  fold_coeff_kernel<<<dim3(blocks_for(n), args.count), 256, 0, c->stream>>>(args, n);
+  return hipGetLastError() == hipSuccess ? CQ_OK : c->fail(CQ_ERR_HIP, "fold_coeff launch failed");
+}
+
+int poly_coset_solve(cq_ctx* c, Fr* io, const NttTables& inv_ext_tb, const CosetSolveConsts& k, uint32_t n) {
+  coset_solve_kernel<<<blocks_for(n), 256, 0, c->stream>>>(io, inv_ext_tb.tw_full, inv_ext_tb.tw_lo, inv_ext_tb.tw_hi, inv_ext_tb.tw_l, k, n);
+  return hipGetLastError() == hipSuccess ? CQ_OK : c->fail(CQ_ERR_HIP, "coset_solve launch failed");
+}
+
+int poly_to_coset_major(cq_ctx* c, const Fr* in, Fr* out, uint32_t log_n, uint32_t log_cosets) {
+  const uint32_t ext = 1u << (log_n + log_cosets);
+  to_coset_major_kernel<<<blocks_for(ext), 256, 0, c->stream>>>(in, out, log_n, log_cosets);
+  return hipGetLastError() == hipSuccess ? CQ_OK : c->fail(CQ_ERR_HIP, "to_coset_major launch failed");
+}
+
 int poly_from_u512(cq_ctx* c, const uint64_t* words_dev, uint32_t n, Fr* out) {
   if (!n) return CQ_OK;
   from_u512_kernel<<<blocks_for(n), 256, 0, c->stream>>>(words_dev, n, out);
diff --git a/sha2_on_cq_halo2_amd/csrc/poly.hpp b/sha2_on_cq_halo2_amd/csrc/poly.hpp
--- a/sha2_on_cq_halo2_amd/csrc/poly.hpp
+++ b/sha2_on_cq_halo2_amd/csrc/poly.hpp
@@ -3,6 +3,7 @@
 #include <vector>
 #include "field.hpp"
 #include "ntt.hpp"
+#include "coset_solve.hpp"
 
 struct cq_ctx;
 
@@ -47,7 +48,17 @@
   Fr y, beta;
   Fr scale;
   uint32_t has_scale = 0;
+  uint32_t coset_log_n = 0;
 };
+constexpr uint32_t FOLD_MAX_WIDTH = 8;
+struct FoldCoeffArgs {
+  const Fr* src[CQ_MAX_LOOKUPS][FOLD_MAX_WIDTH];
+  Fr* out[CQ_MAX_LOOKUPS];
+  uint32_t width[CQ_MAX_LOOKUPS];
+  uint32_t count;
+  Fr theta_pow261[FOLD_MAX_WIDTH];
+};
+
 
 int poly_eval(cq_ctx* c, const Fr* a_dev, uint32_t n, const Fr& z, Fr* out_host);
 int poly_eval_batch(cq_ctx* c, const Fr* const* p_dev, const uint32_t* len, uint32_t count, const Fr& z, Fr* out_host);
@@ -64,6 +75,9 @@
 int poly_resolve_assigned(cq_ctx* c, const Fr* const* num_dev, Fr* const* out_dev, const uint32_t* off, uint32_t ncols,
                           const uint32_t* rows_dev, const Fr* den_dev, uint32_t nrows, Fr* work_dev, const uint32_t* verdict_dev);
 int poly_lincomb(cq_ctx* c, const LincombArgs& args, uint32_t n, Fr* out_dev);
+int poly_fold_coeff(cq_ctx* c, const FoldCoeffArgs& args, uint32_t n);
+int poly_coset_solve(cq_ctx* c, Fr* io, const NttTables& inv_ext_tb, const CosetSolveConsts& k, uint32_t n);
+int poly_to_coset_major(cq_ctx* c, const Fr* in, Fr* out, uint32_t log_n, uint32_t log_cosets);
 int poly_from_u512(cq_ctx* c, const uint64_t* words_dev, uint32_t n, Fr* out_dev);
 int poly_cq_b_denominators(cq_ctx* c, const Fr* f, uint32_t n, uint32_t u, const Fr& beta, Fr* out);
 int poly_cq_quotient(cq_ctx* c, const CqQuotientArgs& args, uint32_t ext, Fr* h);
@@ -101,6 +115,8 @@
 int domain_lagrange_to_coeff(cq_domain* d, const Fr* in, Fr* out, uint32_t batch, size_t in_stride, size_t out_stride);
 int domain_coeff_to_extended(cq_domain* d, const Fr* in, Fr* out, uint32_t batch, size_t in_stride, size_t out_stride);
 int domain_extended_to_coeff(cq_domain* d, const Fr* in, Fr* out );
+int domain_coeff_to_cosets(cq_domain* d, const Fr* in, Fr* out, uint32_t batch, size_t in_stride, size_t out_stride);
+int domain_cosets_to_coeff(cq_domain* d, const Fr* in, Fr* out );
 int domain_fft(cq_ctx* c, const Fr* in, Fr* out, uint32_t log_n, const Fr& omega, uint32_t batch, size_t in_stride,
                size_t out_stride);
 }
diff --git a/sha2_on_cq_halo2_amd/csrc/prover_lookup.hip b/sha2_on_cq_halo2_amd/csrc/prover_lookup.hip
--- a/sha2_on_cq_halo2_amd/csrc/prover_lookup.hip
+++ b/sha2_on_cq_halo2_amd/csrc/prover_lookup.hip
@@ -172,6 +172,29 @@
       CQ_TRY(fork.begin(seq));
       if (resident) {
         CQ_TRY(resident_round1_transforms());
+      } else if (by_cosets) {
+        if (A && !adv_is_coeff) {
+          CQ_TRY(lagrange_to_coeff_cols(B.adv, B.adv, A));
+          adv_is_coeff = true;
+        }
+        FoldCoeffArgs fa;
+        fa.count = (uint32_t)L;
+        for (uint32_t j = 0; j < CQ_MAX_WIDTH; j++) fa.theta_pow261[j] = theta_pow[j];
+        bool any_linear = false;
+        for (size_t l = 0; l < L; l++) {
+          const cq_lookup_desc& lk = pk->lookups[l];
+          fa.width[l] = 0;
+          fa.out[l] = B.f_coeff + l * n;
+          if (!lk.plain_advice()) {
+            CQ_TRY(domain_lagrange_to_coeff(dom, B.f_lag + l * n, B.f_coeff + l * n, 1, n, n));
+            continue;
+          }
+          any_linear = true;
+          fa.width[l] = (uint32_t)lk.cols.size();
+          for (size_t j = 0; j < lk.cols.size(); j++) fa.src[l][j] = adv_poly + (size_t)lk.cols[j] * n;
+        }
+        if (any_linear) CQ_TRY(poly_fold_coeff(c, fa, (uint32_t)n));
+        CQ_TRY(domain_coeff_to_cosets(dom, B.f_coeff, B.cosets + L * ext, (uint32_t)L, n, ext));
       } else {
         if (L) {
           CQ_TRY(lagrange_to_coeff_cols(B.f_lag, B.f_coeff, L));
@@ -316,6 +339,7 @@
       CQ_TRY(fork.begin(seq));
       if (A && !adv_is_coeff) CQ_TRY(lagrange_to_coeff_cols(B.adv, B.adv, A));
       if (resident) CQ_TRY(resident_b_to_coset());
+      else if (by_cosets) CQ_TRY(domain_coeff_to_cosets(dom, B.bpoly, B.cosets, (uint32_t)L, n, ext));
       else if (L) CQ_TRY(coeff_to_extended_cols(B.bpoly, B.cosets, L));
       if (general && A) CQ_TRY(coeff_to_extended_cols(B.adv, B.adv_cosets, A));
       CQ_TRY(fork.end());
diff --git a/sha2_on_cq_halo2_amd/csrc/prover_quotient.hip b/sha2_on_cq_halo2_amd/csrc/prover_quotient.hip
--- a/sha2_on_cq_halo2_amd/csrc/prover_quotient.hip
+++ b/sha2_on_cq_halo2_amd/csrc/prover_quotient.hip
@@ -169,7 +169,8 @@
   }
   CqQuotientArgs qa;
   qa.h_in = general ? B.h_ext : nullptr;
-  qa.l_active = pk->l_active_row;
+  qa.l_active = by_cosets ? pk->l_active_cosets : pk->l_active_row;
+  qa.coset_log_n = by_cosets ? k : 0;
   qa.t_evals = dom->t_evaluations_dev;
   qa.t_len = (uint32_t)dom->t_evaluations.size();
   qa.y = y;
@@ -185,6 +186,7 @@
 
 int ProofRun::construct_h() {
   if (resident) CQ_TRY(resident_collect_h());
+  else if (by_cosets) CQ_TRY(domain_cosets_to_coeff(dom, B.h_ext, B.h_coeff));
   else CQ_TRY(domain_extended_to_coeff(dom, B.h_ext, B.h_coeff));
   for (size_t i = 0; i < pieces; i++) (void)rng.fr();
   {
diff --git a/sha2_on_cq_halo2_amd/csrc/prover_run.hpp b/sha2_on_cq_halo2_amd/csrc/prover_run.hpp
--- a/sha2_on_cq_halo2_amd/csrc/prover_run.hpp
+++ b/sha2_on_cq_halo2_amd/csrc/prover_run.hpp
@@ -242,6 +242,7 @@
   const size_t S = pk->perm_sets(), PC = pk->perm_columns.size(), chunk_len = pk->cs_degree - 2;
   const size_t PL = pk->legacy.size(), NC = pk->challenge_phase.size(), pieces = dom->quotient_poly_degree;
   const bool general = pk->general();
+  const bool by_cosets = pk->coset_quotient();
   const bool early_m = L > 0 && pk->num_phases == 1 && pk->challenge_phase.empty();
   const bool early_adv = early_advice_polys(pk);
   const bool b_by_rows = L > 0 && !pk->sharded() && pk->b_row_bases[0] != nullptr &&
diff --git a/sha2_on_cq_halo2_amd/params.py b/sha2_on_cq_halo2_amd/params.py
--- a/sha2_on_cq_halo2_amd/params.py
+++ b/sha2_on_cq_halo2_amd/params.py
@@ -288,3 +288,9 @@
 
     def extended_to_coeff_dev(self, src: DevBuf, dst: DevBuf):
         self.ctx._chk(self.ctx.lib.cq_extended_to_coeff_dev(self.h, src.ptr, dst.ptr))
+
+    def coeff_to_cosets_dev(self, src: DevBuf, dst: DevBuf, batch: int = 1):
+        self.ctx._chk(self.ctx.lib.cq_coeff_to_cosets_dev(self.h, src.ptr, dst.ptr, batch))
+
+    def cosets_to_coeff_dev(self, src: DevBuf, dst: DevBuf):
+        self.ctx._chk(self.ctx.lib.cq_cosets_to_coeff_dev(self.h, src.ptr, dst.ptr))
diff --git a/sha2_on_cq_halo2_amd/proving_key.py b/sha2_on_cq_halo2_amd/proving_key.py
--- a/sha2_on_cq_halo2_amd/proving_key.py
+++ b/sha2_on_cq_halo2_amd/proving_key.py
@@ -190,6 +190,10 @@
     def b_row_bases(self, which):
         return self.ctx.lib.cq_pk_b_row_bases_dev(self.h, which)
 
+    @property
+    def coset_quotient(self) -> bool:
+        return bool(self.ctx.lib.cq_pk_coset_quotient(self.h))
+
     def set_opener(self, name: str):
         self.ctx._chk(self.ctx.lib.cq_pk_set_opener(self.h, _OPENERS[name]))
         self.proof_size = self.ctx.lib.cq_pk_proof_size(self.h)
```

Result: slower. 1418 (-1.4%).
